# chrischoy/DeepGlobalRegistration

Measured on AMD Instinct MI355X. Metric: pair registrations/sec (FCGF x2 + 1-NN + 6-D inlier net + gate + weighted Procrustes + SE(3) refinement), higher is better.
Workload: dtype f32 results via 2 x f16 split operands (3 f16 MFMA products per MAC, f32 accumulate); k = 1 convs, kNN re-evaluation and registration in exact f32, SVD in f64

## Files before the change

deepglobalregistration_amd/_lib.py:

```python
import ctypes as C
import os
import threading

import torch

_HERE = os.path.dirname(os.path.abspath(__file__))
LIB_PATH = os.environ.get('DGR_HIP_LIB') or os.path.join(_HERE, 'lib', 'libdgr_hip.so')

DGR_OK, DGR_EINVAL, DGR_EHIP, DGR_ENOMEM, DGR_ESVD, DGR_EINTERNAL = 0, -1, -2, -3, -4, -5
STATUS_OK, STATUS_LOW_CONFIDENCE, STATUS_SVD_FAILED, STATUS_SAFEGUARD = 0, 1, 2, 3
STATUS_FLAG_ICP_SKIPPED, STATUS_MASK = 0x100, 0xff

c_i32p, c_i64p, c_f32p, c_f64p = (C.POINTER(C.c_int32), C.POINTER(C.c_int64),
                                  C.POINTER(C.c_float), C.POINTER(C.c_double))
vp = C.c_void_p


class WeightDesc(C.Structure):
    _fields_ = [('name', C.c_char_p), ('data', vp), ('numel', C.c_int64)]


class Params(C.Structure):
    _fields_ = [('clip_weight_thresh', C.c_float), ('voxel_size', C.c_float),
                ('inlier_feature_type', C.c_int), ('max_iter', C.c_int),
# ... 29 lines not shown
    'dgr_net_rerun_layer': (C.c_int, [vp, vp, C.c_int, C.c_int, c_f32p, c_f32p]),
    'dgr_maps_create': (C.c_int, [vp, vp, C.c_int64, C.c_int, C.c_int, C.POINTER(vp), vp]),
    'dgr_maps_destroy': (None, [vp]),
    'dgr_maps_get_coords': (C.c_int, [vp, C.c_int, vp, C.c_int64, c_i64p]),
    'dgr_maps_get_kernel_map': (C.c_int, [vp, C.c_int, C.c_int, vp, C.c_int64, vp, vp, C.c_int64,
                                          c_i64p, c_i64p]),
    'dgr_knn1_l2': (C.c_int, [vp, vp, C.c_int64, vp, C.c_int64, C.c_int, C.c_int, vp, vp, vp]),
    'dgr_knn1_l2_batch': (C.c_int, [vp, vp, c_i64p, vp, c_i64p, C.c_int, C.c_int, C.c_int, vp, vp, vp]),
    'dgr_knn_l2': (C.c_int, [vp, vp, C.c_int64, vp, C.c_int64, C.c_int, C.c_int, C.c_int, vp, vp, vp]),
    'dgr_knn_l2_batch': (C.c_int, [vp, vp, c_i64p, vp, c_i64p, C.c_int, C.c_int, C.c_int, C.c_int, vp, vp,
                                   vp]),
    'dgr_inlier_inputs': (C.c_int, [vp, vp, vp, C.c_int64, vp, vp, C.c_int64, vp, C.c_int, vp, vp, vp]),
    'dgr_sigmoid_clip_sum': (C.c_int, [vp, vp, C.c_int64, C.c_float, vp, c_f64p, vp]),
    'dgr_gather_rows3': (C.c_int, [vp, vp, vp, C.c_int64, vp, vp]),
    'dgr_weighted_procrustes': (C.c_int, [vp, vp, vp, vp, C.c_int64, C.c_float, c_f32p, c_f32p, vp]),
    'dgr_se3_refine': (C.c_int, [vp, vp, vp, vp, C.c_int64, C.c_float, C.c_int, C.c_int, C.c_double,
                                 c_f32p, c_f32p, c_i32p, c_f32p, c_i32p, vp]),
    'dgr_register_batch': (C.c_int, [vp, vp, vp, vp, vp, c_i64p, vp, vp, c_i64p, C.c_int,
                                     C.POINTER(Params), vp, vp, c_f32p, c_i32p, c_f32p, vp]),
    'dgr_register_pairs': (C.c_int, [vp, vp, vp, vp, vp, c_i64p, C.c_int, C.c_int, c_i32p, C.c_int,
                                     C.POINTER(Params), vp, vp, c_f32p, c_i32p, c_f32p, vp]),
    'dgr_register_batch_f64': (C.c_int, [vp, c_f64p, C.c_int64, c_i64p]),
    'dgr_register_batch_output': (C.c_int, [vp, C.c_int, vp, C.c_int64, c_i64p, vp]),
    'dgr_ctx_set_profiling': (C.c_int, [vp, C.c_int]),
    'dgr_icp_point_to_point': (C.c_int, [vp, vp, C.c_int64, vp, C.c_int64, C.c_double, c_f64p, C.c_int, C.c_double,
                                          C.c_double, c_f64p, c_f64p, vp]),
    'dgr_ransac_correspondence': (C.c_int, [vp, vp, vp, C.c_int64, C.c_double, C.c_int64, C.c_uint32, c_f64p, c_f64p, vp]),
    'dgr_ctx_stage_times': (C.c_int, [vp, c_f32p]),
    'dgr_ctx_stage_times_v2': (C.c_int, [vp, c_f32p, C.c_int, C.POINTER(C.c_int)]),
    'dgr_ctx_conv_launches': (C.c_int64, [vp]),
    'dgr_ctx_conv_launch_times': (C.c_int, [vp, c_f32p, c_f32p, C.c_int64, C.POINTER(C.c_int64)]),
    'dgr_ctx_conv_launch_kernel_us': (C.c_int, [vp, c_f32p, C.c_int64, C.POINTER(C.c_int64)]),
    'dgr_ctx_conv_launch_kinds': (C.c_int, [vp, C.c_char_p, C.c_int64, C.POINTER(C.c_int64)]),
    'dgr_radius_pairs_batch': (C.c_int, [vp, vp, c_i64p, vp, c_i64p, C.c_int, c_f64p, C.c_double, C.c_int, vp, vp,
                                         C.c_int64, c_i64p, vp]),
    'dgr_pairs_isin_batch': (C.c_int, [vp, vp, c_i64p, vp, c_i64p, C.c_int, c_i64p, vp, vp]),
    'dgr_validation_counts': (C.c_int, [vp, vp, vp, C.c_float, c_i64p, C.c_int, c_i64p, vp]),
    'dgr_score_pairs': (C.c_int, [vp, vp, c_i64p, C.c_int, c_i32p, C.c_int, c_f64p, C.c_double, c_f64p, vp]),
    'dgr_pose_graph_optimize': (C.c_int, [vp, C.c_int, c_i64p, c_i64p, c_i32p, c_f64p, c_f64p, C.POINTER(C.c_uint8), c_f64p,
                                          C.POINTER(PgParams), c_f64p, c_f64p, c_f64p, vp]),
    'dgr_voxel_mean': (C.c_int, [vp, vp, C.c_int, c_i64p, C.c_int, c_i32p, C.c_int, c_f64p, c_f64p, C.c_double, vp, vp, vp, vp,
                                 vp, c_i64p, c_i64p, vp]),
    'dgr_debug_ortho2rotation': (C.c_int, [vp, vp, C.c_int64, vp, vp, vp, vp]),
    'dgr_debug_se3_refine_from': (C.c_int, [vp, vp, vp, vp, C.c_int64, C.c_float, C.c_int, C.c_int, C.c_double,
                                            c_f64p, c_f64p, vp]),
    'dgr_debug_smooth_l1': (C.c_int, [vp, vp, vp, C.c_int64, C.c_float, vp, vp]),
    'dgr_debug_conv_layer': (C.c_int, [vp, vp, C.c_int, vp, vp, C.c_int, C.c_int64, vp, vp]),
}

_lib = None


def load():
    global _lib
    if _lib is not None:
        return _lib
    if not os.path.exists(LIB_PATH):
        raise RuntimeError(
            f'{LIB_PATH} not found: the HIP extension is not built.  Run '
            '`python -c "import __graft_entry__ as g; g.build()"` (or `make -C '
            'deepglobalregistration_amd/csrc`).  There is no CPU fallback.')
    lib = C.CDLL(LIB_PATH)
    for name, (res, args) in SIGNATURES.items():
        fn = getattr(lib, name)
        fn.restype = res
        fn.argtypes = args
# ... 74 lines not shown
```

deepglobalregistration_amd/csrc/conv.hip:

```cpp
#include <stdlib.h>

#include <map>

#include "dgr_internal.h"
#include <algorithm>
#include "hash.h"
#include "split.h"

typedef float f32x16 __attribute__((ext_vector_type(16)));
typedef float f32x4 __attribute__((ext_vector_type(4)));
typedef _Float16 f16x4 __attribute__((ext_vector_type(4)));
typedef int i32x4 __attribute__((ext_vector_type(4)));
typedef unsigned int u32x2 __attribute__((ext_vector_type(2)));
typedef unsigned int u32x4 __attribute__((ext_vector_type(4)));

struct ConvKArgs {
  const float *in;
  float *out;
  float *y;
  const float *shift;
  const float *w;
  const int32_t *pair_in, *pair_out, *tile_ptr, *rule_ptr, *n_rows_dev;
  const int4 *tile_desc;
  int in_ld, out_ld, in_relu, y_ld;
// ... 817 lines not shown
__global__ void grid_layout_kernel(DgrGridMeta *m, int pad, long long cap) {
  static_assert(GRID_MAXB == 64, "one lane per batch element");
  const int b = threadIdx.x;
  long long vol = 0;
  if (m->mx[b][0] >= m->mn[b][0]) {
    vol = 1;
    for (int d = 0; d < 3; ++d) {
      const long long e = (long long)m->mx[b][d] - m->mn[b][d] + 1 + 2 * pad;
      m->dim[b][d] = (int32_t)(e < (1ll << 30) ? e : (1ll << 30));
      vol = (vol <= cap && e <= cap) ? vol * e : cap + 1;
    }
  }
  long long incl = vol;
#pragma unroll
  for (int s = 1; s < 64; s <<= 1) {
    const long long up = __shfl_up(incl, s, 64);
    if (b >= s) incl += up;
  }
  m->base[b] = incl - vol;
  const long long total = __shfl(incl, 63, 64);
  if (b == 0) {
    m->total = total <= cap ? total : cap + 1;
    m->ok = (!m->bad && total <= cap) ? 1 : 0;
  }
}

__global__ void grid_clear_kernel(const DgrGridMeta *m, int32_t *__restrict__ cells) {
  if (!m->ok) return;
  const long long total = m->total;
  for (long long i = ((long long)blockIdx.x * blockDim.x + threadIdx.x) * 4; i < total; i += (long long)gridDim.x * blockDim.x * 4)
    *reinterpret_cast<int4 *>(cells + i) = make_int4(-1, -1, -1, -1);
}

__device__ __forceinline__ long long grid_cell(const DgrGridMeta *m, int b, int x, int y, int z, int pad) {
  const long long dx = m->dim[b][0], dy = m->dim[b][1];
  return m->base[b] + ((long long)(z - m->mn[b][2] + pad) * dy + (y - m->mn[b][1] + pad)) * dx + (x - m->mn[b][0] + pad);
}

constexpr uint32_t GRID_EMPTY = 0xffffffffu;
__global__ void grid_fill_kernel(const int32_t *__restrict__ coords, const int32_t *n_dev, const DgrGridMeta *m, int pad,
                                 int32_t *__restrict__ cells, const float *__restrict__ values, int values_ld) {
  if (!m->ok) return;
  const int64_t o = (int64_t)blockIdx.x * blockDim.x + threadIdx.x;
  if (o >= *n_dev) return;
  const int4 c = *reinterpret_cast<const int4 *>(coords + o * 4);
  cells[grid_cell(m, c.x, c.y, c.z, c.w, pad)] = values ? __builtin_bit_cast(int32_t, values[o * values_ld]) : (int32_t)o;
}

constexpr int C1_MAXK = 343;
__global__ void __launch_bounds__(256)
    conv1_grid_kernel(const int32_t *__restrict__ coords, const int32_t *n_dev, const DgrGridMeta *__restrict__ m,
                      const int32_t *__restrict__ cells, int ks, const float *__restrict__ in, int in_ld, int cin,
                      const float *__restrict__ w, const float *__restrict__ shift, float *__restrict__ out,
                      int out_ld, int32_t *pair_count, uint32_t *__restrict__ out_amax) {
  __shared__ int2 lists[256 / 64][2][C1_MAXK + 1];
  if (!m->ok) return;
  const int n = *n_dev;
  const int lane = threadIdx.x & 63, wv = threadIdx.x >> 6;
  const int half = ks >> 1, ks2 = ks * ks;
  const int ky = lane % ks, kz = lane / ks;
  const int vsel = lane >> 5, co = lane & 31;
  const unsigned long long below = (1ull << lane) - 1ull;
  const int64_t wave_id = ((int64_t)blockIdx.x * blockDim.x + threadIdx.x) >> 6;
  const int64_t n_waves = ((int64_t)gridDim.x * blockDim.x) >> 6;
  int pairs = 0;
  for (int64_t o0 = wave_id * 2; o0 < n; o0 += n_waves * 2) {
// ... 146 lines not shown
      }
      if (kz + 1 < KS) fill((kz + 1) & 1);
    }
    const int64_t o = v0 + (lane & 15);
    uint32_t mx = 0;
    if (o < n) {
#pragma unroll
      for (int jb = 0; jb < 2; ++jb) {
        f32x4 v = acc[jb];
        if (shift) v += *reinterpret_cast<const f32x4 *>(shift + 16 * jb + 4 * (lane >> 4));
        *reinterpret_cast<f32x4 *>(out + o * out_ld + 16 * jb + 4 * (lane >> 4)) = v;
        const i32x4 b = __builtin_bit_cast(i32x4, v);
        mx = max(mx, max(max((uint32_t)b.x & 0x7fffffffu, (uint32_t)b.y & 0x7fffffffu), max((uint32_t)b.z & 0x7fffffffu, (uint32_t)b.w & 0x7fffffffu)));
      }
    }
    if (out_amax) {
      mx = max(mx, (uint32_t)__shfl_xor((int)mx, 16, 64));
      mx = max(mx, (uint32_t)__shfl_xor((int)mx, 32, 64));
      if (lane < 16 && o < n) atomicMax(out_amax + o, mx);
    }
  }
  if (pair_count) {
    for (int d = 32; d > 0; d >>= 1) pairs += __shfl_down(pairs, d, 64);
    if (lane == 0 && pairs) atomicAdd(&pair_sum, pairs);
    __syncthreads();
    if (threadIdx.x == 0 && pair_sum) atomicAdd(pair_count, pair_sum);
  }
}

int dgr_conv1_probe(DgrArena &arena, const DgrCoordMap &cm, int ks, const float *in, int in_ld, int cin,
                    const float *w_tiled, const float *shift, float *out, int out_ld, int32_t *pair_count,
                    hipStream_t stream, const float *w_compact, const char **kernel_name, uint32_t *out_amax) {
  DGR_REQUIRE(cin >= 1 && cin <= 8 && ks % 2 == 1, "conv1 probe: cin=%d ks=%d", cin, ks);
  if (pair_count && ks > 7) DGR_HIP_CHECK(hipMemsetAsync(pair_count, 0, sizeof(int32_t), stream));
  const int32_t *grid_done = nullptr;
  if (ks <= 7) {
    static const long long cap = 64ll << 20;
    DgrArena::Mark mk = arena.mark();
    DgrGridMeta *meta;
    int32_t *cells;
    DGR_ALLOC(meta, arena, DgrGridMeta, 1);
    DGR_ALLOC(cells, arena, int32_t, cap + 4);
    grid_init_kernel<<<1, 64, 0, stream>>>(meta, pair_count);
    grid_bbox_kernel<<<(int)dgr_ceil_div(cm.n_cap, 256), 256, 0, stream>>>(cm.coords, cm.n_dev, meta);
    grid_layout_kernel<<<1, 64, 0, stream>>>(meta, ks >> 1, cap);
    grid_clear_kernel<<<2048, 256, 0, stream>>>(meta, cells);
    const bool mfma = cin == 1 && w_compact && (out_ld & 3) == 0 && (ks == 3 || ks == 5 || ks == 7);
    grid_fill_kernel<<<(int)dgr_ceil_div(cm.n_cap, 256), 256, 0, stream>>>(cm.coords, cm.n_dev, meta, ks >> 1, cells,
                                                                           mfma ? in : nullptr, in_ld);
    static int resident = 0;
    if (resident == 0) {
      int per_cu = 0, dev = 0, cus = 0;
      DGR_HIP_CHECK(hipOccupancyMaxActiveBlocksPerMultiprocessor(&per_cu, conv1_grid_kernel, 256, 0));
      DGR_HIP_CHECK(hipGetDevice(&dev));
      DGR_HIP_CHECK(hipDeviceGetAttribute(&cus, hipDeviceAttributeMultiprocessorCount, dev));
      resident = (per_cu < 1 ? 1 : per_cu) * (cus < 1 ? 1 : cus);
    }
    if (mfma) {
      const int wgs = (int)dgr_ceil_div(cm.n_cap, 64);
      if (ks == 7) conv1_grid_mfma<7><<<wgs, 256, 0, stream>>>(cm.coords, cm.n_dev, meta, cells, w_compact, shift, out, out_ld, pair_count, out_amax);
      else if (ks == 5) conv1_grid_mfma<5><<<wgs, 256, 0, stream>>>(cm.coords, cm.n_dev, meta, cells, w_compact, shift, out, out_ld, pair_count, out_amax);
      else conv1_grid_mfma<3><<<wgs, 256, 0, stream>>>(cm.coords, cm.n_dev, meta, cells, w_compact, shift, out, out_ld, pair_count, out_amax);
      if (kernel_name) *kernel_name = ks == 7 ? "conv1_grid_mfma<7>" : ks == 5 ? "conv1_grid_mfma<5>" : "conv1_grid_mfma<3>";
    } else {
    int64_t blocks = dgr_ceil_div(cm.n_cap, 8);
    if (blocks > resident) blocks = (int64_t)resident * std::min<int64_t>(4, blocks / resident);
    conv1_grid_kernel<<<(int)blocks, 256, 0, stream>>>(cm.coords, cm.n_dev, meta, cells, ks, in, in_ld, cin, w_tiled, shift,
                                                       out, out_ld, pair_count, out_amax);
    if (kernel_name) *kernel_name = "conv1_grid_kernel";
    }
    DGR_LAUNCH_CHECK();
    grid_done = &meta->ok;
    arena.rewind(mk);
  }
  {
    int64_t blocks = dgr_ceil_div(cm.n_cap, 4);
    if (blocks > 4096) blocks = 4096;
    conv1_probe_kernel<<<(int)blocks, 256, 0, stream>>>(cm.coords, cm.n_dev, cm.table, cm.table_mask, ks, in, in_ld, cin,
                                                        w_tiled, shift, out, out_ld, pair_count, grid_done, out_amax);
  }
  DGR_LAUNCH_CHECK();
  return DGR_OK;
}

__global__ void l2_normalize_kernel(const float *__restrict__ in, int in_ld, float *__restrict__ out,
                                    int out_ld, int c, int relu, const int32_t *n_dev) {
  const int64_t n = *n_dev;
  for (int64_t r = (int64_t)blockIdx.x * blockDim.x + threadIdx.x; r < n;
       r += (int64_t)gridDim.x * blockDim.x) {
    float s = 0.f;
    for (int j = 0; j < c; ++j) {
      float v = in[r * in_ld + j];
      if (relu) v = fmaxf(v, 0.f);
      s += v * v;
    }
    const float den = sqrtf(s) + 1e-8f;
    for (int j = 0; j < c; ++j) {
      float v = in[r * in_ld + j];
      if (relu) v = fmaxf(v, 0.f);
      out[r * out_ld + j] = v / den;
    }
  }
}

// ... 10 lines not shown
```

deepglobalregistration_amd/csrc/coordmap.hip:

```cpp
#include <algorithm>

#include "dgr_internal.h"
#include "hash.h"

constexpr int SCAN_THREADS = 256;
constexpr int SCAN_ITEMS = 8;
constexpr int SCAN_BLOCK = SCAN_THREADS * SCAN_ITEMS;

__device__ __forceinline__ int block_exclusive_scan_256(int v, int *lds , int *total) {
  const int lane = threadIdx.x & 63, wave = threadIdx.x >> 6;
  int x = v;
#pragma unroll
  for (int d = 1; d < 64; d <<= 1) {
    int y = __shfl_up(x, d, 64);
    if (lane >= d) x += y;
  }
  if (lane == 63) lds[wave] = x;
  __syncthreads();
  int base = 0, tot = 0;
#pragma unroll
  for (int w = 0; w < SCAN_THREADS / 64; ++w) {
    int s = lds[w];
    if (w < wave) base += s;
    tot += s;
  }
  __syncthreads();
  *total = tot;
  return base + x - v;
}

__global__ void __launch_bounds__(1024) scan_single_block(const int32_t *__restrict__ in, int64_t n,
                                                          int32_t *__restrict__ out, int32_t *total_out) {
  __shared__ int wsum[16];
  __shared__ int carry_s;
  const int lane = threadIdx.x & 63, wave = threadIdx.x >> 6;
  if (threadIdx.x == 0) carry_s = 0;
  __syncthreads();
  for (int64_t base = 0; base < n; base += 4096) {
    const int64_t i0 = base + (int64_t)threadIdx.x * 4;
    int v[4], s = 0;
#pragma unroll
    for (int j = 0; j < 4; ++j) { v[j] = (i0 + j < n) ? in[i0 + j] : 0; s += v[j]; }
    int x = s;
#pragma unroll
    for (int d = 1; d < 64; d <<= 1) { int y = __shfl_up(x, d, 64); if (lane >= d) x += y; }
    if (lane == 63) wsum[wave] = x;
    __syncthreads();
    int wbase = 0, tot = 0;
#pragma unroll
    for (int w = 0; w < 16; ++w) { const int t = wsum[w]; if (w < wave) wbase += t; tot += t; }
    int ex = carry_s + wbase + x - s;
#pragma unroll
    for (int j = 0; j < 4; ++j) { if (i0 + j < n) out[i0 + j] = ex; ex += v[j]; }
    __syncthreads();
    if (threadIdx.x == 0) carry_s += tot;
    __syncthreads();
  }
  if (threadIdx.x == 0 && total_out) *total_out = carry_s;
}

struct ScanJobs {
  const int32_t *in[DGR_SCAN_MAX];
  int32_t *out[DGR_SCAN_MAX], *sums[DGR_SCAN_MAX], *total[DGR_SCAN_MAX];
  long long n[DGR_SCAN_MAX];
  int nblocks[DGR_SCAN_MAX];
};

__global__ void __launch_bounds__(SCAN_THREADS) scan_block_sums_multi(ScanJobs j) {
  __shared__ int lds[4];
  const int a = blockIdx.y;
  if ((int)blockIdx.x >= j.nblocks[a]) return;
  const int32_t *in = j.in[a];
  const long long n = j.n[a];
  long long base = (long long)blockIdx.x * SCAN_BLOCK + (long long)threadIdx.x * SCAN_ITEMS;
  int s = 0;
#pragma unroll
  for (int i = 0; i < SCAN_ITEMS; ++i)
    if (base + i < n) s += in[base + i];
  int tot;
  block_exclusive_scan_256(s, lds, &tot);
  if (threadIdx.x == 0) j.sums[a][blockIdx.x] = tot;
}

__global__ void __launch_bounds__(SCAN_THREADS) scan_sums_serial_multi(ScanJobs j) {
  __shared__ int lds[4];
  const int a = blockIdx.x;
  int32_t *sums = j.sums[a];
  const int nblocks = j.nblocks[a];
  int carry = 0;
  for (int b0 = 0; b0 < nblocks; b0 += SCAN_THREADS) {
    int i = b0 + threadIdx.x;
    int v = i < nblocks ? sums[i] : 0;
    int tot;
    int ex = block_exclusive_scan_256(v, lds, &tot);
    if (i < nblocks) sums[i] = carry + ex;
    carry += tot;
  }
  if (threadIdx.x == 0 && j.total[a]) *j.total[a] = carry;
}

__global__ void __launch_bounds__(SCAN_THREADS) scan_final_multi(ScanJobs j) {
  __shared__ int lds[4];
  const int a = blockIdx.y;
  if ((int)blockIdx.x >= j.nblocks[a]) return;
  const int32_t *in = j.in[a];
  int32_t *out = j.out[a];
  const long long n = j.n[a];
  long long base = (long long)blockIdx.x * SCAN_BLOCK + (long long)threadIdx.x * SCAN_ITEMS;
  int v[SCAN_ITEMS];
  int s = 0;
#pragma unroll
  for (int i = 0; i < SCAN_ITEMS; ++i) {
    v[i] = (base + i < n) ? in[base + i] : 0;
    s += v[i];
  }
  int tot;
  int ex = block_exclusive_scan_256(s, lds, &tot) + j.sums[a][blockIdx.x];
#pragma unroll
  for (int i = 0; i < SCAN_ITEMS; ++i) {
    if (base + i < n) out[base + i] = ex;
    ex += v[i];
  }
}

int dgr_exclusive_scan_multi(DgrArena &arena, int count, const int32_t *const *in, int32_t *const *out, const int64_t *n,
                             int32_t *const *total_out, hipStream_t stream) {
  DGR_REQUIRE(count >= 1 && count <= DGR_SCAN_MAX, "scan: %d arrays", count);
  ScanJobs j;
  int maxb = 0;
  for (int a = 0; a < count; ++a) {
    DGR_REQUIRE(n[a] > 0, "scan: empty array");
    j.in[a] = in[a]; j.out[a] = out[a]; j.total[a] = total_out ? total_out[a] : nullptr; j.n[a] = n[a];
    j.nblocks[a] = (int)dgr_ceil_div(n[a], SCAN_BLOCK);
    DGR_ALLOC(j.sums[a], arena, int32_t, j.nblocks[a]);
    maxb = j.nblocks[a] > maxb ? j.nblocks[a] : maxb;
  }
  for (int a = count; a < DGR_SCAN_MAX; ++a) { j.in[a] = nullptr; j.out[a] = j.sums[a] = j.total[a] = nullptr; j.n[a] = 0; j.nblocks[a] = 0; }
  scan_block_sums_multi<<<dim3(maxb, count), SCAN_THREADS, 0, stream>>>(j);
  scan_sums_serial_multi<<<count, SCAN_THREADS, 0, stream>>>(j);
  scan_final_multi<<<dim3(maxb, count), SCAN_THREADS, 0, stream>>>(j);
  DGR_LAUNCH_CHECK();
  return DGR_OK;
}

int dgr_exclusive_scan_i32(DgrArena &arena, const int32_t *in, int32_t *out, int64_t n,
                           int32_t *total_out, hipStream_t stream) {
  if (n <= 0) {
    if (total_out) DGR_HIP_CHECK(hipMemsetAsync(total_out, 0, sizeof(int32_t), stream));
    return DGR_OK;
  }
  if (n <= (1 << 14)) {
    scan_single_block<<<1, 1024, 0, stream>>>(in, n, out, total_out);
    DGR_LAUNCH_CHECK();
    return DGR_OK;
  }
  const int32_t *ins[1] = {in};
  int32_t *outs[1] = {out}, *tots[1] = {total_out};
  const int64_t ns[1] = {n};
  return dgr_exclusive_scan_multi(arena, 1, ins, outs, ns, tots, stream);
}

template <int NC>
__global__ void unique_insert(const int32_t *__restrict__ keys, const int32_t *n_dev, int64_t n_cap,
                              int32_t *table, uint32_t mask) {
  int64_t r = (int64_t)blockIdx.x * blockDim.x + threadIdx.x;
  int64_t n = n_dev ? *n_dev : n_cap;
  if (r >= n) return;
  int32_t me[NC];
#pragma unroll
  for (int d = 0; d < NC; ++d) me[d] = keys[r * NC + d];
  uint32_t slot = dgr_hash_row<NC>(me) & mask;
  while (true) {
    int cur = __hip_atomic_load(&table[slot], __ATOMIC_RELAXED, __HIP_MEMORY_SCOPE_AGENT);
    if (cur == DGR_EMPTY) {
      int old = atomicCAS(&table[slot], DGR_EMPTY, (int)r);
      if (old == DGR_EMPTY) return;
      cur = old;
    }
    if (dgr_rows_equal<NC>(keys + (int64_t)cur * NC, me)) {
      atomicMin(&table[slot], (int)r);
      return;
// ... 33 lines not shown
  int64_t o = rank[r];
#pragma unroll
  for (int d = 0; d < NC; ++d) out_coords[o * NC + d] = keys[r * NC + d];
  if (sel_out) sel_out[o] = r;
}

__global__ void table_relabel(int32_t *table, uint32_t cap, const int32_t *__restrict__ rank) {
  uint32_t s = blockIdx.x * blockDim.x + threadIdx.x;
  if (s >= cap) return;
  int v = table[s];
  if (v >= 0) table[s] = rank[v];
}

template <int NC>
__global__ void stride_keys(const int32_t *__restrict__ coords, const int32_t *n_dev, int ts_new,
                            int32_t *__restrict__ keys) {
  int64_t r = (int64_t)blockIdx.x * blockDim.x + threadIdx.x;
  if (r >= *n_dev) return;
  const int32_t m = ~(ts_new - 1);
  keys[r * NC] = coords[r * NC];
#pragma unroll
  for (int d = 1; d < NC; ++d) keys[r * NC + d] = coords[r * NC + d] & m;
}

static inline int grid_for(int64_t n, int threads = 256) { return (int)dgr_ceil_div(n > 0 ? n : 1, threads); }

template <int NC>
static int unique_rows_t(DgrArena &arena, const int32_t *keys, const int32_t *n_dev, int64_t n_cap,
                         int32_t *first_flag, int32_t *rank, int32_t *n_unique_dev,
                         int32_t **table_out, uint32_t *mask_out, hipStream_t stream) {
  uint32_t cap = dgr_next_pow2((uint64_t)(2 * n_cap > 64 ? 2 * n_cap : 64));
  int32_t *table;
  DGR_ALLOC(table, arena, int32_t, cap);
  DGR_HIP_CHECK(hipMemsetAsync(table, 0xff, (size_t)cap * sizeof(int32_t), stream));
  unique_insert<NC><<<grid_for(n_cap), 256, 0, stream>>>(keys, n_dev, n_cap, table, cap - 1);
  unique_flag<NC><<<grid_for(n_cap), 256, 0, stream>>>(keys, n_dev, n_cap, table, cap - 1, first_flag,
                                                      nullptr);
  DGR_LAUNCH_CHECK();
  DGR_CHECK(dgr_exclusive_scan_i32(arena, first_flag, rank, n_cap, n_unique_dev, stream));
  *table_out = table;
  *mask_out = cap - 1;
  return DGR_OK;
}

int dgr_unique_rows(DgrArena &arena, const int32_t *keys, int64_t n, int nc, int32_t *first_flag,
                    int32_t *rank, int32_t *n_unique_dev, int32_t **table_out, uint32_t *mask_out,
                    hipStream_t stream) {
  if (nc == 4)
    return unique_rows_t<4>(arena, keys, nullptr, n, first_flag, rank, n_unique_dev, table_out,
                            mask_out, stream);
  if (nc == 7)
    return unique_rows_t<7>(arena, keys, nullptr, n, first_flag, rank, n_unique_dev, table_out,
                            mask_out, stream);
  dgr_set_error("unsupported coordinate width %d", nc);
  return DGR_EINVAL;
}

template <int NC>
static int build_coord_maps_t(DgrArena &arena, const int32_t *coords, int64_t N, DgrMapSet *ms,
                              hipStream_t stream) {
  DgrCoordMap &c1 = ms->cm[0];
  c1.coords = const_cast<int32_t *>(coords);
  c1.n_cap = N;
  c1.ts = 1;
  DGR_ALLOC(c1.n_dev, arena, int32_t, 1);
  int32_t n32 = (int32_t)N;
  DGR_HIP_CHECK(hipMemcpyAsync(c1.n_dev, &n32, sizeof(int32_t), hipMemcpyHostToDevice, stream));
  {
    uint32_t cap = dgr_next_pow2((uint64_t)(2 * N > 64 ? 2 * N : 64));
    DGR_ALLOC(c1.table, arena, int32_t, cap);
    c1.table_mask = cap - 1;
    DGR_HIP_CHECK(hipMemsetAsync(c1.table, 0xff, (size_t)cap * sizeof(int32_t), stream));
    unique_insert<NC><<<grid_for(N), 256, 0, stream>>>(coords, nullptr, N, c1.table, cap - 1);
    unique_flag<NC><<<grid_for(N), 256, 0, stream>>>(coords, nullptr, N, c1.table, cap - 1, nullptr,
                                                    ms->overflow);
    DGR_LAUNCH_CHECK();
  }
  for (int l = 1; l < 4; ++l) {
    DgrCoordMap &p = ms->cm[l - 1];
    DgrCoordMap &c = ms->cm[l];
    c.ts = p.ts * 2;
    c.n_cap = p.n_cap;
    int32_t *keys, *flag, *rank;
    DGR_ALLOC(keys, arena, int32_t, p.n_cap * NC);
    DGR_ALLOC(flag, arena, int32_t, p.n_cap);
    DGR_ALLOC(rank, arena, int32_t, p.n_cap);
    DGR_ALLOC(c.coords, arena, int32_t, c.n_cap * NC);
    DGR_ALLOC(c.n_dev, arena, int32_t, 1);
    stride_keys<NC><<<grid_for(p.n_cap), 256, 0, stream>>>(p.coords, p.n_dev, c.ts, keys);
    DGR_CHECK(unique_rows_t<NC>(arena, keys, p.n_dev, p.n_cap, flag, rank, c.n_dev, &c.table,
                                &c.table_mask, stream));
    unique_compact<NC><<<grid_for(p.n_cap), 256, 0, stream>>>(keys, p.n_dev, p.n_cap, flag, rank,
                                                             c.coords, nullptr);
    table_relabel<<<grid_for((int64_t)c.table_mask + 1), 256, 0, stream>>>(c.table, c.table_mask + 1,
                                                                           rank);
    DGR_LAUNCH_CHECK();
  }
  return DGR_OK;
}

__global__ void half_keys_kernel(const int32_t *__restrict__ coords7, const int32_t *n_dev,
                                 int32_t *__restrict__ keys4) {
  int64_t r = (int64_t)blockIdx.x * blockDim.x + threadIdx.x;
  if (r >= *n_dev) return;
#pragma unroll
  for (int d = 0; d < 4; ++d) keys4[r * 4 + d] = coords7[r * 7 + d];
}

__global__ void bucket_count_kernel(const int32_t *__restrict__ keys4, const int32_t *n_dev,
                                    const int32_t *__restrict__ table, uint32_t mask,
                                    const int32_t *__restrict__ bkeys, int32_t *__restrict__ row_bucket,
                                    int32_t *counts) {
  int64_t r = (int64_t)blockIdx.x * blockDim.x + threadIdx.x;
  if (r >= *n_dev) return;
  int32_t q[4] = {keys4[r * 4], keys4[r * 4 + 1], keys4[r * 4 + 2], keys4[r * 4 + 3]};
  const int b = dgr_lookup<4>(table, mask, bkeys, q);
  row_bucket[r] = b;
  atomicAdd(&counts[b], 1);
}

__global__ void bucket_members_kernel(const int32_t *__restrict__ row_bucket, const int32_t *n_dev,
                                      const int32_t *__restrict__ start, int32_t *cursor, int32_t *__restrict__ members) {
  int64_t r = (int64_t)blockIdx.x * blockDim.x + threadIdx.x;
  if (r >= *n_dev) return;
  const int b = row_bucket[r];
  members[start[b] + atomicAdd(&cursor[b], 1)] = (int32_t)r;
}

__global__ void bucket_fill_kernel(const int32_t *__restrict__ row_bucket, const int32_t *n_dev,
// ... 7 lines not shown
  const int32_t *c = coords7 + r * 7;
  int p;
  if (members) {
    int rank = 0;
    for (int e = start[b], end = start[b + 1]; e < end; ++e) rank += members[e] < (int32_t)r;
    p = start[b] + rank;
  } else {
    p = start[b] + atomicAdd(&cursor[b], 1);
  }
  if (coords_new) {
#pragma unroll
    for (int d = 0; d < 7; ++d) coords_new[(int64_t)p * 7 + d] = c[d];
    canon[p] = (int32_t)r;
    inv[r] = p;
    second[p] = make_int4(c[4], c[5], c[6], p);
  } else {
    second[p] = make_int4(c[4], c[5], c[6], (int32_t)r);
  }
}

struct RenumberJobs {
  const int32_t *inv[4];
  int32_t *table[4];
  uint32_t cap[4];
};
__global__ void renumber_table_kernel(RenumberJobs j) {
  const int l = blockIdx.y;
  const uint32_t s = blockIdx.x * blockDim.x + threadIdx.x;
  if (s >= j.cap[l]) return;
  const int v = j.table[l][s];
  if (v >= 0) j.table[l][s] = j.inv[l][v];
}

int dgr_build_half_buckets(DgrArena &arena, DgrCoordMap *cm, DgrHalfBuckets *hb, int levels, int renumber_from,
                           hipStream_t stream) {
  DGR_REQUIRE(levels >= 1 && levels <= 4 && renumber_from >= 1, "half buckets: %d levels", levels);
  int32_t *keys[4], *flag[4], *rank[4], *nb_dev[4], *row_bucket[4], *counts[4], *cursor[4];
  uint32_t cap[4];
  size_t table_words = 0, count_words = 0;
  for (int l = 0; l < levels; ++l) {
    const int64_t n = cm[l].n_cap;
    cap[l] = dgr_next_pow2((uint64_t)(2 * n > 64 ? 2 * n : 64));
    table_words += cap[l];
    count_words += 2 * (size_t)(n + 1);
  }
  int32_t *tables, *cnts;
  DGR_ALLOC(tables, arena, int32_t, table_words);
  DGR_ALLOC(cnts, arena, int32_t, count_words);
  DGR_HIP_CHECK(hipMemsetAsync(tables, 0xff, table_words * sizeof(int32_t), stream));
  DGR_HIP_CHECK(hipMemsetAsync(cnts, 0, count_words * sizeof(int32_t), stream));
  for (int l = 0; l < levels; ++l) {
    const int64_t n = cm[l].n_cap;
    hb[l].table = tables; tables += cap[l];
    hb[l].mask = cap[l] - 1;
    counts[l] = cnts; cursor[l] = cnts + (n + 1); cnts += 2 * (n + 1);
    DGR_ALLOC(keys[l], arena, int32_t, n * 4);
    DGR_ALLOC(flag[l], arena, int32_t, n);
    DGR_ALLOC(rank[l], arena, int32_t, n);
    DGR_ALLOC(nb_dev[l], arena, int32_t, 1);
    DGR_ALLOC(row_bucket[l], arena, int32_t, n);
    DGR_ALLOC(hb[l].bkeys, arena, int32_t, n * 4);
    DGR_ALLOC(hb[l].start, arena, int32_t, n + 1);
    DGR_ALLOC(hb[l].second, arena, int4, n);
  }
  for (int l = 0; l < levels; ++l) {
    const int64_t n = cm[l].n_cap;
    half_keys_kernel<<<grid_for(n), 256, 0, stream>>>(cm[l].coords, cm[l].n_dev, keys[l]);
    unique_insert<4><<<grid_for(n), 256, 0, stream>>>(keys[l], cm[l].n_dev, n, hb[l].table, hb[l].mask);
    unique_flag<4><<<grid_for(n), 256, 0, stream>>>(keys[l], cm[l].n_dev, n, hb[l].table, hb[l].mask, flag[l], nullptr);
  }
  DGR_LAUNCH_CHECK();
  {
    const int32_t *ins[4];
    int32_t *outs[4], *tots[4];
    int64_t ns[4];
    for (int l = 0; l < levels; ++l) { ins[l] = flag[l]; outs[l] = rank[l]; tots[l] = nb_dev[l]; ns[l] = cm[l].n_cap; }
    DGR_CHECK(dgr_exclusive_scan_multi(arena, levels, ins, outs, ns, tots, stream));
  }
  for (int l = 0; l < levels; ++l) {
    const int64_t n = cm[l].n_cap;
    unique_compact<4><<<grid_for(n), 256, 0, stream>>>(keys[l], cm[l].n_dev, n, flag[l], rank[l], hb[l].bkeys, nullptr);
    table_relabel<<<grid_for((int64_t)hb[l].mask + 1), 256, 0, stream>>>(hb[l].table, hb[l].mask + 1, rank[l]);
    bucket_count_kernel<<<grid_for(n), 256, 0, stream>>>(keys[l], cm[l].n_dev, hb[l].table, hb[l].mask, hb[l].bkeys, row_bucket[l],
                                                         counts[l]);
  }
  DGR_LAUNCH_CHECK();
  {
    const int32_t *ins[4];
    int32_t *outs[4], *tots[4];
    int64_t ns[4];
    for (int l = 0; l < levels; ++l) { ins[l] = counts[l]; outs[l] = hb[l].start; tots[l] = nullptr; ns[l] = cm[l].n_cap + 1; }
    DGR_CHECK(dgr_exclusive_scan_multi(arena, levels, ins, outs, ns, tots, stream));
  }
  RenumberJobs rj = {};
  int nrj = 0;
  int64_t max_cap = 0;
  for (int l = 0; l < levels; ++l) {
    const int64_t n = cm[l].n_cap;
    int32_t *coords_new = nullptr, *canon = nullptr, *inv = nullptr;
    if (l >= renumber_from) {
      DGR_ALLOC(coords_new, arena, int32_t, n * 7);
      DGR_ALLOC(canon, arena, int32_t, n);
      DGR_ALLOC(inv, arena, int32_t, n);
      rj.inv[nrj] = inv; rj.table[nrj] = cm[l].table; rj.cap[nrj] = cm[l].table_mask + 1;
      max_cap = std::max<int64_t>(max_cap, rj.cap[nrj]);
      ++nrj;
    }
    const int32_t *members = nullptr;
    if (coords_new) {
      bucket_members_kernel<<<grid_for(n), 256, 0, stream>>>(row_bucket[l], cm[l].n_dev, hb[l].start, cursor[l], rank[l]);
      members = rank[l];
    }
    bucket_fill_kernel<<<grid_for(n), 256, 0, stream>>>(row_bucket[l], cm[l].n_dev, hb[l].start, cursor[l], members,
                                                        cm[l].coords, hb[l].second, coords_new, canon, inv);
    if (coords_new) { cm[l].coords = coords_new; cm[l].canon = canon; }
    hb[l].built = true;
  }
  if (nrj) renumber_table_kernel<<<dim3((unsigned)grid_for(max_cap), nrj), 256, 0, stream>>>(rj);
  DGR_LAUNCH_CHECK();
  return DGR_OK;
}

int dgr_build_coord_maps(DgrArena &arena, const int32_t *coords, int64_t N, DgrMapSet *ms,
                         hipStream_t stream) {
  if (ms->nc == 4) return build_coord_maps_t<4>(arena, coords, N, ms, stream);
  if (ms->nc == 7) return build_coord_maps_t<7>(arena, coords, N, ms, stream);
  dgr_set_error("unsupported dimension D=%d (3 and 6 are on the DGR path)", ms->D);
  return DGR_EINVAL;
}

template <typename T>
__global__ void voxel_keys(const T *__restrict__ xyz, int64_t M, T inv_unused, T voxel, int32_t batch,
                           int32_t *__restrict__ keys) {
  int64_t r = (int64_t)blockIdx.x * blockDim.x + threadIdx.x;
  if (r >= M) return;
  keys[r * 4] = batch;
#pragma unroll
  for (int d = 0; d < 3; ++d) keys[r * 4 + 1 + d] = (int32_t)floor(xyz[r * 3 + d] / voxel);
}

template <typename T>
__global__ void voxel_gather_xyz(const T *__restrict__ xyz, const int64_t *__restrict__ sel,
                                 const int32_t *n_dev, float *__restrict__ out) {
  int64_t r = (int64_t)blockIdx.x * blockDim.x + threadIdx.x;
  if (r >= *n_dev) return;
  int64_t s = sel[r];
#pragma unroll
  for (int d = 0; d < 3; ++d) out[r * 3 + d] = (float)xyz[s * 3 + d];
}

extern "C" int dgr_voxelize(dgr_ctx *ctx, const void *xyz, int is_f64, int64_t M, double voxel_size,
                            int32_t batch_index, int64_t *sel_out, int32_t *coords_out,
                            float *xyz_out, int64_t *n_out, dgr_stream stream_) {
  DGR_REQUIRE(ctx && xyz && sel_out && coords_out && n_out, "dgr_voxelize: NULL argument");
  DGR_REQUIRE(M > 0 && M < (1ll << 30), "dgr_voxelize: M=%lld out of range", (long long)M);
  DGR_REQUIRE(voxel_size > 0, "dgr_voxelize: voxel_size must be positive");
  hipStream_t stream = (hipStream_t)stream_;
  DGR_HIP_CHECK(hipSetDevice(ctx->device));
  DGR_CHECK(ctx->arena.reset());
  DgrArena &A = ctx->arena;
  int32_t *keys, *flag, *rank, *n_dev, *table;
  uint32_t mask;
  DGR_ALLOC(keys, A, int32_t, M * 4);
  DGR_ALLOC(flag, A, int32_t, M);
  DGR_ALLOC(rank, A, int32_t, M);
  DGR_ALLOC(n_dev, A, int32_t, 1);
  if (is_f64)
    voxel_keys<double><<<grid_for(M), 256, 0, stream>>>((const double *)xyz, M, 0.0, voxel_size,
                                                       batch_index, keys);
  else
    voxel_keys<float><<<grid_for(M), 256, 0, stream>>>((const float *)xyz, M, 0.f, (float)voxel_size,
                                                      batch_index, keys);
  DGR_CHECK(unique_rows_t<4>(A, keys, nullptr, M, flag, rank, n_dev, &table, &mask, stream));
  unique_compact<4><<<grid_for(M), 256, 0, stream>>>(keys, nullptr, M, flag, rank, coords_out, sel_out);
  if (xyz_out) {
    if (is_f64)
      voxel_gather_xyz<double><<<grid_for(M), 256, 0, stream>>>((const double *)xyz, sel_out, n_dev,
                                                               xyz_out);
    else
      voxel_gather_xyz<float><<<grid_for(M), 256, 0, stream>>>((const float *)xyz, sel_out, n_dev,
                                                              xyz_out);
  }
  DGR_LAUNCH_CHECK();
  int32_t n32 = 0;
  DGR_HIP_CHECK(hipMemcpyAsync(&n32, n_dev, sizeof(int32_t), hipMemcpyDeviceToHost, stream));
  DGR_HIP_CHECK(hipStreamSynchronize(stream));
  *n_out = n32;
  return DGR_OK;
}
```

deepglobalregistration_amd/csrc/ctx.hip:

```cpp
#include <stdarg.h>
#include <time.h>
#include <string.h>

#include "dgr_internal.h"

static thread_local char g_err[1024] = "";

void dgr_set_error(const char *fmt, ...) {
  va_list ap;
  va_start(ap, fmt);
  vsnprintf(g_err, sizeof(g_err), fmt, ap);
  va_end(ap);
}

extern "C" const char *dgr_last_error(void) { return g_err; }
extern "C" const char *dgr_version(void) { return "dgr_hip 0.4 (gfx950)"; }

static constexpr size_t kAlign = 256;
static constexpr size_t kMinChunk = (size_t)256 << 20;

void *DgrArena::alloc(size_t bytes) {
  bytes = (bytes + kAlign - 1) / kAlign * kAlign;
  if (bytes == 0) bytes = kAlign;
  while (cur < chunks.size()) {
// ... 203 lines not shown

extern "C" int dgr_ctx_stage_times_v2(dgr_ctx *ctx, float *times_ms, int capacity, int *n) {
  DGR_REQUIRE(ctx != nullptr && times_ms != nullptr && capacity >= 0, "bad argument");
  static_assert(sizeof(ctx->stage_ms) == DGR_NUM_STAGE_TIMES * sizeof(float), "stage list and header disagree");
  const int m = capacity < DGR_NUM_STAGE_TIMES ? capacity : DGR_NUM_STAGE_TIMES;
  memcpy(times_ms, ctx->stage_ms, (size_t)m * sizeof(float));
  if (n) *n = m;
  return DGR_OK;
}

extern "C" int64_t dgr_ctx_conv_launches(dgr_ctx *ctx) { return ctx ? ctx->conv_launches : 0; }

extern "C" int dgr_ctx_conv_launch_times(dgr_ctx *ctx, float *times_ms, float *gemm_ms, int64_t capacity, int64_t *n) {
  DGR_REQUIRE(ctx != nullptr && times_ms != nullptr && n != nullptr, "bad argument");
  int64_t m = (int64_t)ctx->conv_span_ms.size();
  if (m > capacity) m = capacity;
  for (int64_t i = 0; i < m; ++i) {
    times_ms[i] = ctx->conv_span_ms[i];
    if (gemm_ms) gemm_ms[i] = i < (int64_t)ctx->gemm_span_ms.size() ? ctx->gemm_span_ms[i] : 0.f;
  }
  *n = m;
  return DGR_OK;
}

extern "C" int dgr_ctx_conv_launch_kernel_us(dgr_ctx *ctx, float *us, int64_t capacity, int64_t *n) {
  DGR_REQUIRE(ctx != nullptr && us != nullptr && n != nullptr, "bad argument");
  int64_t m = (int64_t)ctx->conv_clk_us.size();
  if (m > capacity) m = capacity;
  for (int64_t i = 0; i < m; ++i) us[i] = ctx->conv_clk_us[i];
  *n = m;
  return DGR_OK;
}

extern "C" int dgr_ctx_conv_launch_kinds(dgr_ctx *ctx, char *buf, int64_t capacity, int64_t *n) {
  DGR_REQUIRE(ctx != nullptr && buf != nullptr && n != nullptr && capacity > 0, "bad argument");
  std::string all;
  int64_t m = 0;
  for (const char *k : ctx->conv_kinds) {
    if ((int64_t)(all.size() + strlen(k) + 2) > capacity) break;
    all += k;
    all += '\n';
    ++m;
  }
  memcpy(buf, all.c_str(), all.size() + 1);
  *n = m;
  return DGR_OK;
}
```

deepglobalregistration_amd/csrc/dgr_internal.h:

```cpp
#pragma once
#include <hip/hip_runtime.h>
#include <stdint.h>
#include <stdio.h>
#include <stdlib.h>
#include <string>
#include <vector>

#include "../../include/dgr_hip.h"

void dgr_set_error(const char *fmt, ...);

#define DGR_HIP_CHECK(expr)                                                                  \
  do {                                                                                       \
    hipError_t _e = (expr);                                                                  \
    if (_e != hipSuccess) {                                                                  \
      dgr_set_error("%s:%d: %s failed: %s", __FILE__, __LINE__, #expr, hipGetErrorString(_e)); \
      return DGR_EHIP;                                                                       \
    }                                                                                        \
  } while (0)

#define DGR_CHECK(expr)          \
  do {                           \
    int _r = (expr);             \
    if (_r != DGR_OK) return _r; \
  } while (0)

#define DGR_REQUIRE(cond, ...)     \
  do {                             \
    if (!(cond)) {                 \
      dgr_set_error(__VA_ARGS__);  \
      return DGR_EINVAL;           \
    }                              \
  } while (0)

#define DGR_LAUNCH_CHECK() DGR_HIP_CHECK(hipGetLastError())

inline bool dgr_exact_f32() {
  static const bool on = getenv("DGR_EXACT_F32") != nullptr;
  return on;
}

struct DgrArena {
  struct Chunk {
    char *base;
    size_t size;
  };
  std::vector<Chunk> chunks;
  size_t cur = 0;
  size_t offset = 0;
  size_t high_water = 0, used_total = 0;
  uint64_t generation = 0;

  struct Mark {
    size_t cur, offset, used_total;
  };
  Mark mark() const { return {cur, offset, used_total}; }
  void rewind(const Mark &m) { cur = m.cur; offset = m.offset; used_total = m.used_total; }
  void *alloc(size_t bytes);
  int reset();
  void release();
  size_t reserved() const;
  template <typename T>
  T *get(size_t n) {
    return static_cast<T *>(alloc(n * sizeof(T)));
  }
};

#define DGR_ALLOC(ptr, arena, T, n)                       \
// ... 151 lines not shown
};

struct DgrEventPool {
  std::vector<hipEvent_t> ev;
  size_t used = 0;
  hipEvent_t next();
  void release();
};

struct dgr_ctx {
  int device = 0;
  int num_cus = 256;
  DgrArena arena;
  bool profiling = false;
  float stage_ms[9] = {0, 0, 0, 0, 0, 0, 0, 0, 0};
  int64_t conv_launches = 0;
  DgrBatchOutputs last;
  std::vector<double> last_T64;
  DgrEventPool events;
  std::vector<std::pair<hipEvent_t, hipEvent_t>> conv_spans, gemm_spans, map3_spans, map6_spans;
  std::vector<float> conv_span_ms, gemm_span_ms;
  std::vector<unsigned long long *> conv_clks;
  std::vector<float> conv_clk_us;
  std::vector<const char *> conv_kinds;
  int32_t *flag_dev = nullptr;
  hipEvent_t wait_ev = nullptr;
  long last_wait_ns = 0;
  double batch_ns_per_row = 0;
  double pairs_ns_per_row = 0;
  unsigned char *pin = nullptr;
  size_t pin_bytes = 0;
  hipStream_t part_stream = nullptr;
  int all_cus = 256;
};

int dgr_ctx_pinned(dgr_ctx *ctx, size_t bytes, unsigned char **out);
int dgr_flag_error(int32_t flag);

int dgr_ctx_wait(dgr_ctx *ctx, hipStream_t stream, long predicted_ns = 0);

int dgr_resunet_forward_impl(dgr_ctx *ctx, dgr_net *net, const int32_t *coords, const float *feats,
                             int64_t N, float *out, hipStream_t stream);
int dgr_ctx_collect_profile(dgr_ctx *ctx);
void dgr_ctx_begin_profile(dgr_ctx *ctx);

int dgr_knn1_batch_impl(dgr_ctx *ctx, const float *F0, const int64_t *off0, const float *F1, const int64_t *off1,
                        int npairs, int C, int squared, int64_t *idx_out, float *dist_out, hipStream_t stream);
int dgr_knn1_impl(dgr_ctx *ctx, const float *F0, int64_t N0, const float *F1, int64_t N1, int C,
                  int squared, int64_t *idx_out, float *dist_out, hipStream_t stream);
int dgr_inlier_inputs_impl(const int32_t *coords0, const float *xyz0, int64_t N0,
                           const int32_t *coords1, const float *xyz1, const int64_t *idx1,
                           int feature_type, int32_t *coords6, float *feats, hipStream_t stream);
int dgr_icp_impl(dgr_ctx *ctx, const float *src, int64_t N0, const float *dst, int64_t N1, double max_dist,
                 const double *T_init, int max_iter, double rel_fitness, double rel_rmse, double *T_out,
                 double *stats_out, hipStream_t stream);
int dgr_ransac_impl(dgr_ctx *ctx, const float *X, const float *Y, int64_t N, double max_dist, int64_t num_hypotheses,
                    uint32_t seed, double *T_out, double *stats_out, hipStream_t stream);
struct DgrIcpJob {
  const float *src = nullptr, *dst = nullptr;
  int64_t N0 = 0, N1 = 0;
  double max_dist = 0;
  int nblocks = 0;
  void *st = nullptr;
  double *P = nullptr, *sorted = nullptr, *partial = nullptr;
  int32_t ncell = 0;
  double host_state[64];
// ... 25 lines not shown
```

deepglobalregistration_amd/csrc/kmap.hip:

```cpp
#include <string.h>

#include <algorithm>

#include "dgr_internal.h"
#include "hash.h"

constexpr int KM_THREADS = 256;

template <int D>
__device__ __forceinline__ void offset_of(int k, int ks, int ts, int32_t *delta) {
  const int half = ks >> 1;
#pragma unroll
  for (int d = 0; d < D; ++d) {
    delta[d] = ((k % ks) - half) * ts;
    k /= ks;
  }
}

template <int D>
__device__ __forceinline__ int probe(const int32_t *__restrict__ out_coords, int64_t o,
                                     const int32_t *delta, const int32_t *__restrict__ in_coords,
                                     const int32_t *__restrict__ in_table, uint32_t in_mask) {
  constexpr int NC = D + 1;
  int32_t q[NC];
// ... 442 lines not shown
  if (need_in_csr) {
    DGR_ALLOC(km->in_ptr, arena, int32_t, n_in_cap + 1);
    DGR_ALLOC(km->in_pos, arena, int32_t, km->pair_cap);
  }
  return DGR_OK;
}

static void finalize_job(FinalizeJobs &fj, int m, const int32_t *base, const int32_t *total, int K, int RB, DgrKernelMap *km) {
  fj.base[m] = base; fj.total[m] = total; fj.K[m] = K; fj.RB[m] = RB;
  fj.rule_ptr[m] = km->rule_ptr; fj.tile_ptr[m] = km->tile_ptr;
  fj.desc[m] = km->tile_desc; fj.tile_cap[m] = km->tile_cap;
}

static int build_kernel_map3(DgrArena &arena, const DgrCoordMap &in, const DgrCoordMap &out, int ks, int max_pairs_per_row,
                             bool need_in_csr, bool want_pair_out, bool want_pair_k, DgrKernelMap *km,
                             int32_t *overflow, hipStream_t stream) {
  constexpr int D = 3;
  const int K = ks * ks * ks;
  const int64_t n_cap = out.n_cap, n_in_cap = in.n_cap;
  const int RB = (int)dgr_ceil_div(n_cap, KM_THREADS);
  DGR_CHECK(alloc_kernel_map(arena, K, n_cap, n_in_cap, max_pairs_per_row, need_in_csr, want_pair_out, want_pair_k, km));
  const int KW = (K + 31) / 32;
  DgrArena::Mark mk = arena.mark();
  int32_t *counts, *base, *total;
  DGR_ALLOC(counts, arena, int32_t, (int64_t)K * RB);
  DGR_ALLOC(base, arena, int32_t, (int64_t)K * RB);
  DGR_ALLOC(total, arena, int32_t, 1);
  uint32_t *mask_out, *mask_in = nullptr;
  int32_t *cnt_out, *cnt_in = nullptr;
  {
    const size_t w_out = (size_t)(n_cap + 1) * KW, w_in = need_in_csr ? (size_t)(n_in_cap + 1) * KW : 0;
    DGR_ALLOC(mask_out, arena, uint32_t, w_out + w_in);
    if (need_in_csr) mask_in = mask_out + w_out;
    DGR_HIP_CHECK(hipMemsetAsync(mask_out, 0, (w_out + w_in) * sizeof(uint32_t), stream));
  }
  DGR_ALLOC(cnt_out, arena, int32_t, n_cap + 1);
  if (need_in_csr) DGR_ALLOC(cnt_in, arena, int32_t, n_in_cap + 1);
  int32_t *hits;
  DGR_ALLOC(hits, arena, int32_t, (int64_t)K * n_cap);
  kmap_search<D><<<dim3(RB, K), KM_THREADS, 0, stream>>>(out.coords, out.n_dev, in.coords, in.table, in.table_mask, ks,
                                                         in.ts, RB, n_cap, hits, counts, KW, mask_out, mask_in);
  DGR_LAUNCH_CHECK();
  mask_count_kernel<<<(int)dgr_ceil_div(n_cap + 1, 256), 256, 0, stream>>>(mask_out, KW, out.n_dev, n_cap + 1, cnt_out);
  if (need_in_csr)
    mask_count_kernel<<<(int)dgr_ceil_div(n_in_cap + 1, 256), 256, 0, stream>>>(mask_in, KW, in.n_dev, n_in_cap + 1, cnt_in);
  {
    const int32_t *ins[3] = {cnt_out, counts, cnt_in};
    int32_t *outs[3] = {km->out_ptr, base, km->in_ptr}, *tots[3] = {nullptr, total, nullptr};
    const int64_t ns[3] = {n_cap + 1, (int64_t)K * RB, n_in_cap + 1};
    DGR_CHECK(dgr_exclusive_scan_multi(arena, need_in_csr ? 3 : 2, ins, outs, ns, tots, stream));
  }
  FinalizeJobs fj = {};
  finalize_job(fj, 0, base, total, K, RB, km);
  kmap_finalize<<<1, 1024, 0, stream>>>(fj);
  tile_desc_kernel<<<dim3((unsigned)dgr_ceil_div(km->tile_cap, 256), 1), 256, 0, stream>>>(fj);
  kmap_fill<<<dim3(RB, (K + KM_KGROUP - 1) / KM_KGROUP), KM_THREADS, 0, stream>>>(
      out.n_dev, RB, K, n_cap, hits, counts, base, km->pair_in, km->pair_out, km->pair_cap, overflow, KW, mask_out,
      km->out_ptr, km->out_pos, mask_in, km->in_ptr, km->in_pos, km->pair_k);
  DGR_LAUNCH_CHECK();
  arena.rewind(mk);
  km->built = true;
  return DGR_OK;
}

struct Kmap6Job {
  const DgrCoordMap *in, *out;
  const DgrHalfBuckets *hb;
  const DgrHalfBuckets *hb_out;
  bool need_in_csr, want_pair_out, want_pair_k;
  DgrKernelMap *km;
};
static int build_kernel_maps6(DgrArena &arena, const Kmap6Job *jobs, int nj, int max_pairs_per_row, int32_t *overflow,
                              hipStream_t stream) {
  constexpr int K = 729, KW = (K + 31) / 32;
  DGR_REQUIRE(nj >= 1 && nj <= KM_MAXJOBS, "6-D kernel maps: %d jobs", nj);
  struct Tr {
    int RB, symmetric;
    int64_t n_cap, n_in_cap, hit_waves;
    int32_t *counts, *base, *total, *cnt_out, *cnt_in;
    uint32_t *mask_out, *mask_in;
    int4 *cell;
    HitList hl;
    unsigned short *wpre_out, *wpre_in;
  } t[KM_MAXJOBS];
  for (int m = 0; m < nj; ++m) {
    const Kmap6Job &J = jobs[m];
    t[m].n_cap = J.out->n_cap; t[m].n_in_cap = J.in->n_cap;
    DGR_REQUIRE(t[m].n_cap < (1ll << 27) && t[m].n_in_cap < (1ll << 27), "6-D kernel maps: more than 2^27 rows");
    DGR_CHECK(alloc_kernel_map(arena, K, t[m].n_cap, t[m].n_in_cap, max_pairs_per_row, J.need_in_csr, J.want_pair_out,
                               J.want_pair_k, J.km));
  }
  DgrArena::Mark mk = arena.mark();
  {
    size_t words = 0;
    for (int m = 0; m < nj; ++m)
      words += (size_t)(t[m].n_cap + 1) * KW + (jobs[m].need_in_csr ? (size_t)(t[m].n_in_cap + 1) * KW : 0) + (size_t)(t[m].n_cap + 1);
    uint32_t *pool;
    DGR_ALLOC(pool, arena, uint32_t, words);
    DGR_HIP_CHECK(hipMemsetAsync(pool, 0, words * sizeof(uint32_t), stream));
    for (int m = 0; m < nj; ++m) {
      t[m].mask_out = pool; pool += (size_t)(t[m].n_cap + 1) * KW;
      t[m].mask_in = nullptr;
      if (jobs[m].need_in_csr) { t[m].mask_in = pool; pool += (size_t)(t[m].n_in_cap + 1) * KW; }
      t[m].cnt_out = reinterpret_cast<int32_t *>(pool); pool += (size_t)(t[m].n_cap + 1);
    }
  }
  for (int m = 0; m < nj; ++m) {
    const Kmap6Job &J = jobs[m];
    Tr &r = t[m];
    r.RB = (int)dgr_ceil_div(r.n_cap, KM_THREADS);
    r.symmetric = (J.in->coords == J.out->coords && !J.need_in_csr) ? 1 : 0;
    DGR_REQUIRE(J.hb && J.hb->built && J.hb_out && J.hb_out->built, "6-D kernel map: first-half buckets missing");
    DGR_ALLOC(r.counts, arena, int32_t, (int64_t)K * r.RB);
    DGR_ALLOC(r.base, arena, int32_t, (int64_t)K * r.RB);
    DGR_ALLOC(r.total, arena, int32_t, 1);
    r.cnt_in = nullptr;
    if (J.need_in_csr) DGR_ALLOC(r.cnt_in, arena, int32_t, r.n_in_cap + 1);
    DGR_ALLOC(r.cell, arena, int4, (int64_t)r.RB * (KM_THREADS / 64) * K);
    const int64_t search_blocks = dgr_ceil_div(r.n_cap * (r.symmetric ? 14 : 27), KM_THREADS);
    r.hit_waves = search_blocks * (KM_THREADS / 64);
    r.hl.region = (J.in->ts >= 8 && r.symmetric) ? 2 * KM_REGION : KM_REGION / 2;
    DGR_REQUIRE(r.hit_waves < (1ll << 31), "6-D kernel map: too many search waves");
    DGR_ALLOC(r.hl.recs, arena, unsigned long long, r.hit_waves * r.hl.region);
    DGR_ALLOC(r.hl.wave_count, arena, int32_t, r.hit_waves);
    DGR_ALLOC(r.wpre_out, arena, unsigned short, (r.n_cap + 1) * KW);
    r.wpre_in = nullptr;
    if (J.need_in_csr) DGR_ALLOC(r.wpre_in, arena, unsigned short, (r.n_in_cap + 1) * KW);
  }
  static_assert(KM_JOBS6 >= KM_MAXJOBS, "multi-job launch tables");
  {
    Bits6Jobs bj = {};
    Colmask6Jobs cj = {};
    int max_sb = 0, max_rb = 0;
    for (int m = 0; m < nj; ++m) {
      const Kmap6Job &J = jobs[m];
      Tr &r = t[m];
      bj.pa[m] = PrunedArgs{J.out->coords, J.out->n_dev, J.hb_out->second, r.n_cap, *J.hb, J.in->ts, r.symmetric};
      bj.mask_out[m] = r.mask_out; bj.mask_in[m] = r.mask_in; bj.hl[m] = r.hl;
      bj.blocks[m] = (int)(r.hit_waves / (KM_THREADS / 64));
      max_sb = std::max(max_sb, bj.blocks[m]);
      cj.mask_out[m] = r.mask_out; cj.n_out_dev[m] = J.out->n_dev; cj.RB[m] = r.RB; cj.cell[m] = r.cell;
      cj.counts[m] = r.counts; cj.row_cnt[m] = r.cnt_out; cj.wpre[m] = r.wpre_out;
      max_rb = std::max(max_rb, r.RB);
    }
    kmap_bits_pruned6<<<dim3((unsigned)max_sb, (unsigned)nj), KM_THREADS, 0, stream>>>(bj, KW);
    kmap_colmask<<<dim3((unsigned)max_rb, (unsigned)nj), KM_THREADS, 0, stream>>>(cj, K, KW);
    {
      MaskCountJobs mj = {};
      int nm = 0;
      long long max_rows = 0;
      for (int m = 0; m < nj; ++m)
        if (jobs[m].need_in_csr) {
          mj.mask[nm] = t[m].mask_in; mj.n_dev[nm] = jobs[m].in->n_dev; mj.n_cap[nm] = t[m].n_in_cap + 1;
          mj.cnt[nm] = t[m].cnt_in; mj.wpre[nm] = t[m].wpre_in;
          max_rows = std::max(max_rows, mj.n_cap[nm]);
          ++nm;
        }
      static_assert(KM_MC_JOBS >= KM_MAXJOBS, "mask-count job table");
      if (nm) mask_count_multi<KW><<<dim3((unsigned)dgr_ceil_div(max_rows, 256), (unsigned)nm), 256, 0, stream>>>(mj);
    }
  }
  DGR_LAUNCH_CHECK();
  {
    const int32_t *ins[DGR_SCAN_MAX];
    int32_t *outs[DGR_SCAN_MAX], *tots[DGR_SCAN_MAX];
    int64_t ns[DGR_SCAN_MAX];
    int c = 0;
    for (int m = 0; m < nj; ++m) {
      ins[c] = t[m].cnt_out; outs[c] = jobs[m].km->out_ptr; tots[c] = nullptr; ns[c++] = t[m].n_cap + 1;
      ins[c] = t[m].counts; outs[c] = t[m].base; tots[c] = t[m].total; ns[c++] = (int64_t)K * t[m].RB;
      if (jobs[m].need_in_csr) { ins[c] = t[m].cnt_in; outs[c] = jobs[m].km->in_ptr; tots[c] = nullptr; ns[c++] = t[m].n_in_cap + 1; }
    }
    DGR_CHECK(dgr_exclusive_scan_multi(arena, c, ins, outs, ns, tots, stream));
  }
  FinalizeJobs fj = {};
  int64_t max_tiles = 0;
  for (int m = 0; m < nj; ++m) {
    finalize_job(fj, m, t[m].base, t[m].total, K, t[m].RB, jobs[m].km);
    max_tiles = std::max<int64_t>(max_tiles, jobs[m].km->tile_cap);
  }
  kmap_finalize<<<nj, 1024, 0, stream>>>(fj);
  tile_desc_kernel<<<dim3((unsigned)dgr_ceil_div(max_tiles, 256), nj), 256, 0, stream>>>(fj);
  {
    Place6Jobs pj = {};
    int max_pb = 0;
    for (int m = 0; m < nj; ++m) {
      const Kmap6Job &J = jobs[m];
      Tr &r = t[m];
      DgrKernelMap *km = J.km;
      pj.p[m] = PlaceArgs{K, KW, r.RB, r.mask_out, km->out_ptr, r.cell, r.base, km->pair_in, km->pair_out, km->pair_k, km->out_pos,
                          km->pair_cap, overflow, r.mask_in, km->in_ptr, km->in_pos, r.wpre_out, r.wpre_in};
      pj.replay[m] = PrunedArgs{J.out->coords, J.out->n_dev, J.hb_out->second, r.n_cap, *J.hb, J.in->ts, r.symmetric};
      pj.h[m] = r.hl;
      pj.n_waves[m] = (int)r.hit_waves;
      pj.blocks[m] = (int)std::min<int64_t>(dgr_ceil_div(r.hit_waves, KM_THREADS / 64), 16384);
      max_pb = std::max(max_pb, pj.blocks[m]);
      km->built = true;
    }
    kmap_place_hits<<<dim3((unsigned)max_pb, (unsigned)nj), KM_THREADS, 0, stream>>>(pj);
  }
  DGR_LAUNCH_CHECK();
  arena.rewind(mk);
  return DGR_OK;
}

constexpr int NBR_JOBS = 10;
struct NbrJobs {
  const int32_t *out_coords[NBR_JOBS], *n_out_dev[NBR_JOBS], *in_coords[NBR_JOBS], *in_table[NBR_JOBS];
  uint32_t in_mask[NBR_JOBS];
  int ts[NBR_JOBS];
  long long n_pad[NBR_JOBS];
  int32_t *nbr[NBR_JOBS];
};
__global__ void __launch_bounds__(KM_THREADS) nbr_search3(NbrJobs J) {
  const int jm = blockIdx.z;
  const int64_t n_pad = J.n_pad[jm];
  const int64_t o = (int64_t)blockIdx.x * KM_THREADS + threadIdx.x;
  if (o >= n_pad) return;
  int32_t *__restrict__ nbr = J.nbr[jm];
  const int kz = blockIdx.y;
  if (o >= *J.n_out_dev[jm]) {
#pragma unroll
    for (int u = 0; u < 9; ++u) nbr[(int64_t)(9 * kz + u) * n_pad + o] = -1;
    return;
  }
  const int sts = J.ts[jm];
  const int4 c = *reinterpret_cast<const int4 *>(J.out_coords[jm] + o * 4);
  int32_t q[9][4];
#pragma unroll
  for (int u = 0; u < 9; ++u) {
    q[u][0] = c.x;
    q[u][1] = c.y + ((u % 3) - 1) * sts;
    q[u][2] = c.z + ((u / 3) - 1) * sts;
    q[u][3] = c.w + (kz - 1) * sts;
// ... 112 lines not shown
  for (int64_t o = (int64_t)blockIdx.x * blockDim.x + threadIdx.x; o < n; o += (int64_t)gridDim.x * blockDim.x)
    c += nbr[(int64_t)k * n_pad + o] >= 0;
  for (int d = 32; d > 0; d >>= 1) c += __shfl_down(c, d, 64);
  if ((threadIdx.x & 63) == 0 && c) atomicAdd(&counts[k], (unsigned long long)c);
}

int dgr_nbr_counts(const DgrNbrTable &t, const int32_t *n_out_dev, int64_t counts[27]) {
  unsigned long long *dev;
  DGR_HIP_CHECK(hipMalloc((void **)&dev, 27 * sizeof(unsigned long long)));
  DGR_HIP_CHECK(hipMemset(dev, 0, 27 * sizeof(unsigned long long)));
  nbr_count_kernel<<<dim3(64, 27), 256>>>(t.nbr, t.n_pad, n_out_dev, dev);
  unsigned long long host[27];
  hipError_t e = hipMemcpy(host, dev, sizeof(host), hipMemcpyDeviceToHost);
  (void)hipFree(dev);
  DGR_HIP_CHECK(e);
  for (int k = 0; k < 27; ++k) counts[k] = (int64_t)host[k];
  return DGR_OK;
}

int dgr_build_coord_maps(DgrArena &arena, const int32_t *coords, int64_t N, DgrMapSet *ms,
                         hipStream_t stream);
int dgr_build_half_buckets(DgrArena &arena, DgrCoordMap *cm, DgrHalfBuckets *hb, int levels, int renumber_from, hipStream_t stream);

int dgr_build_maps(DgrArena &arena, const int32_t *coords, int64_t N, int D, int conv1_ks,
                   DgrMapSet *ms, hipStream_t stream, bool skip_conv1_map, bool lean, bool nbr_tables) {
  DGR_REQUIRE(D == 3 || D == 6, "D=%d not supported (the DGR path uses D=3 and D=6)", D);
  DGR_REQUIRE(conv1_ks % 2 == 1 && conv1_ks >= 1, "conv1 kernel size must be odd");
  DGR_REQUIRE(N > 0 && N < (1ll << 30), "N=%lld out of range", (long long)N);
  ms->D = D;
  ms->nc = D + 1;
  ms->conv1_ks = conv1_ks;
  if (!ms->overflow) {
    DGR_ALLOC(ms->overflow, arena, int32_t, 1);
    DGR_HIP_CHECK(hipMemsetAsync(ms->overflow, 0, sizeof(int32_t), stream));
  }
  DGR_CHECK(dgr_build_coord_maps(arena, coords, N, ms, stream));
  if (nbr_tables) {
    DGR_REQUIRE(D == 3, "neighbour tables are a D = 3 structure");
    ms->use_nbr = true;
    NbrJobs nbj = {};
    int n_nbj = 0;
    int32_t *cls;
    DGR_ALLOC(cls, arena, int32_t, 3 * 8);
    for (int l = 0; l < 4; ++l) DGR_CHECK(build_nbr_table(arena, ms->cm[l], ms->cm[l], ms->cm[l].ts, +1, &ms->nsame[l], &nbj, &n_nbj));
    for (int l = 0; l < 3; ++l) {
      DGR_CHECK(build_nbr_table(arena, ms->cm[l], ms->cm[l + 1], ms->cm[l].ts, +1, &ms->ndown[l], &nbj, &n_nbj));
      DGR_CHECK(build_nbr_table(arena, ms->cm[l + 1], ms->cm[l], ms->cm[l].ts, -1, &ms->nup[l], &nbj, &n_nbj, cls + 8 * l));
    }
    DGR_CHECK(nbr_tables_launch(nbj, n_nbj, stream));
    {
      ClsJobs cj = {};
      int max_nb = 0;
      for (int l = 0; l < 3; ++l) {
        cj.coords[l] = ms->cm[l].coords; cj.n_dev[l] = ms->cm[l].n_dev; cj.ts[l] = ms->cm[l].ts;
        cj.nb[l] = (int)dgr_ceil_div(ms->cm[l].n_cap, KM_THREADS);
        DGR_ALLOC(cj.blk_cnt[l], arena, int32_t, (int64_t)cj.nb[l] * 8);
        cj.perm[l] = ms->nup[l].perm; cj.cls_count[l] = ms->nup[l].cls_count; cj.cls_cap[l] = ms->nup[l].cls_cap;
        max_nb = std::max(max_nb, cj.nb[l]);
      }
      cls_count_kernel<<<dim3((unsigned)max_nb, 3), KM_THREADS, 0, stream>>>(cj);
      cls_fill_kernel<<<dim3((unsigned)max_nb, 3), KM_THREADS, 0, stream>>>(cj);
      DGR_LAUNCH_CHECK();
    }
    if (lean) {
      if (conv1_ks != 3 && !skip_conv1_map)
        DGR_CHECK(build_kernel_map3(arena, ms->cm[0], ms->cm[0], conv1_ks, 1024, false, false, true, &ms->conv1, ms->overflow,
                                    stream));
      return DGR_OK;
    }
  }
  const int cap_row = (D == 3) ? 1024 : 160;
  if (D == 6) {
    DGR_REQUIRE(conv1_ks == 3, "6-D kernel maps support kernel size 3 only (got %d)", conv1_ks);
    DGR_CHECK(dgr_build_half_buckets(arena, ms->cm, ms->hb, 4, 1, stream));
    Kmap6Job jobs[7];
    for (int l = 0; l < 4; ++l) jobs[l] = {&ms->cm[l], &ms->cm[l], &ms->hb[l], &ms->hb[l], false, !lean, !lean || l == 0, &ms->same[l]};
    for (int l = 0; l < 3; ++l) jobs[4 + l] = {&ms->cm[l], &ms->cm[l + 1], &ms->hb[l], &ms->hb[l + 1], true, true, !lean, &ms->down[l]};
    DGR_CHECK(build_kernel_maps6(arena, jobs, 7, cap_row, ms->overflow, stream));
    ms->conv1 = ms->same[0];
    return DGR_OK;
  }
  auto build = [&](const DgrCoordMap &in, const DgrCoordMap &out, int ks, bool rev, bool want_k, DgrKernelMap *km) -> int {
    const bool want_out = !lean || rev, want_pk = !lean || want_k;
    return build_kernel_map3(arena, in, out, ks, cap_row, rev, want_out, want_pk, km, ms->overflow, stream);
  };
  for (int l = 0; l < 4; ++l) DGR_CHECK(build(ms->cm[l], ms->cm[l], 3, false, l == 0, &ms->same[l]));
  if (conv1_ks == 3)
    ms->conv1 = ms->same[0];
  else if (!skip_conv1_map)
    DGR_CHECK(build(ms->cm[0], ms->cm[0], conv1_ks, false, true, &ms->conv1));
  for (int l = 0; l < 3; ++l) DGR_CHECK(build(ms->cm[l], ms->cm[l + 1], 3, true, false, &ms->down[l]));
  return DGR_OK;
}

struct dgr_maps {
  dgr_ctx *ctx;
  DgrArena arena;
  DgrMapSet ms;
  int32_t *coords_copy = nullptr;
  hipStream_t stream;
};

extern "C" int dgr_maps_create(dgr_ctx *ctx, const int32_t *coords, int64_t N, int D,
                               int conv1_kernel_size, dgr_maps **out, dgr_stream stream_) {
  DGR_REQUIRE(ctx && coords && out, "dgr_maps_create: NULL argument");
  hipStream_t stream = (hipStream_t)stream_;
  DGR_HIP_CHECK(hipSetDevice(ctx->device));
  dgr_maps *m = new dgr_maps();
  m->ctx = ctx;
  m->stream = stream;
  int rc = DGR_OK;
  do {
    m->coords_copy = m->arena.get<int32_t>((size_t)N * (D + 1));
    if (!m->coords_copy) { rc = DGR_ENOMEM; break; }
    if (hipMemcpyAsync(m->coords_copy, coords, (size_t)N * (D + 1) * sizeof(int32_t),
                       hipMemcpyDeviceToDevice, stream) != hipSuccess) { rc = DGR_EHIP; break; }
    rc = dgr_build_maps(m->arena, m->coords_copy, N, D, conv1_kernel_size, &m->ms, stream, false, false, D == 3);
    if (rc != DGR_OK) break;
    int32_t flag = 0;
    if (hipMemcpyAsync(&flag, m->ms.overflow, sizeof(int32_t), hipMemcpyDeviceToHost, stream) != hipSuccess ||
        hipStreamSynchronize(stream) != hipSuccess) { rc = DGR_EHIP; dgr_set_error("maps sync failed"); break; }
    if (flag == 1) { dgr_set_error("duplicate coordinates in the sparse tensor input"); rc = DGR_EINVAL; break; }
    if (flag == 2) { dgr_set_error("kernel-map capacity exceeded"); rc = DGR_ENOMEM; break; }
  } while (0);
  if (rc != DGR_OK) {
    m->arena.release();
    delete m;
    return rc;
  }
  *out = m;
  return DGR_OK;
}

extern "C" void dgr_maps_destroy(dgr_maps *m) {
  if (!m) return;
  (void)hipDeviceSynchronize();
  m->arena.release();
  delete m;
// ... 110 lines not shown
```

deepglobalregistration_amd/csrc/knn.hip:

```cpp
#include "knn_prefilter.h"

template <int C, int QPT>
__global__ void __launch_bounds__(KNN_THREADS)
    knn1_kernel(const float *__restrict__ F0, const float *__restrict__ F1, KnnBatch B, int splits,
                u64 *__restrict__ best, const int32_t *run_flag, const int32_t *__restrict__ qlist,
                const int32_t *qcount, int64_t q_begin) {
  __shared__ __attribute__((aligned(16))) float tile[KNN_TB * C];
  const KnnPair d = B.p[blockIdx.z];
  if (run_flag && run_flag[blockIdx.z] == 0) return;
  F0 += d.q0 * C;
  F1 += d.r0 * C;
  best += d.q0;
  const int64_t N0 = d.n0, N1 = d.n1;
  if (qlist) qlist += d.q0 - q_begin;
  const int64_t n_q = qlist ? (int64_t)qcount[blockIdx.z] : N0;
  if ((int64_t)blockIdx.x * KNN_THREADS * QPT >= n_q) return;
  const int64_t q0 = ((int64_t)blockIdx.x * KNN_THREADS + threadIdx.x) * QPT;
  const int rows_per_split = (int)(((N1 + splits - 1) / splits + KNN_TB - 1) / KNN_TB) * KNN_TB;
  const int64_t j_begin = (int64_t)blockIdx.y * rows_per_split;
  const int64_t j_end = min(N1, j_begin + rows_per_split);
  if (j_begin >= j_end) return;
  float q[QPT][C];
  int64_t qrow[QPT];
#pragma unroll
// ... 139 lines not shown
    }
#pragma unroll
    for (int s2 = 32; s2 > 0; s2 >>= 1) {
      const u64 o = __shfl_xor(key, s2, 64);
      key = o < key ? o : key;
    }
    if ((threadIdx.x & 63) == 0) wkey[threadIdx.x >> 6] = key;
    __syncthreads();
    if (threadIdx.x == 0) {
      u64 k3 = wkey[0];
      for (int w = 1; w < 4; ++w) k3 = wkey[w] < k3 ? wkey[w] : k3;
      if (k3 != KNN_KEY_NONE) atomicMin(best + q, k3);
    }
    __syncthreads();
  }
}

__global__ void knn_long_list_flags(const int32_t *__restrict__ qcount, int np, int32_t *__restrict__ flags) {
  if ((int)threadIdx.x < np) flags[threadIdx.x] = qcount[threadIdx.x] > KNN_SCAN_MAX;
}

static int knn_prefiltered(dgr_ctx *ctx, const float *F0, const float *F1, KnnBatch B, u64 *best, hipStream_t stream) {
  KnnPlan P;
  DGR_CHECK(knn_prefilter_setup<false>(ctx, F0, F1, B, KNN_SLOTS, stream, &P));
  DGR_CHECK((knn_mfma_launch<false, false>(ctx, B, P, KNN_SUB, KNN_SLOTS, stream)));
  DGR_CHECK((knn_mfma_launch<true, false>(ctx, B, P, 1, KNN_SLOTS, stream)));
  knn_exact_kernel<<<(int)dgr_ceil_div(P.span, 256), 256, 0, stream>>>(F0, F1, P.cand, P.cand_cnt, P.q_begin,
                                                                      P.q_begin + P.span, best);
  DGR_LAUNCH_CHECK();
  DGR_CHECK(knn_list_overflows(B, P, KNN_SLOTS, stream));
  dim3 grid(KNN_SCAN_SPLITS, B.np);
  knn_query_scan_kernel<<<grid, 256, 0, stream>>>(F0, F1, B, P.q_begin, P.qlist, P.qcount, best);
  knn_long_list_flags<<<1, 64, 0, stream>>>(P.qcount, B.np, P.flags);
  DGR_LAUNCH_CHECK();
  DGR_CHECK(knn_launch<32>(ctx, F0, F1, B, best, P.flags, stream, P.qlist, P.qcount, P.q_begin));
  return knn_launch<32>(ctx, F0, F1, B, best, P.fallback, stream);
}

int dgr_knn1_batch_impl(dgr_ctx *ctx, const float *F0, const int64_t *off0, const float *F1, const int64_t *off1,
                        int npairs, int C, int squared, int64_t *idx_out, float *dist_out, hipStream_t stream) {
  return knn_for_each_table(ctx, off0, off1, npairs, 1, true, stream, [&](const KnnBatch &B, u64 *best) -> int {
    DGR_CHECK(knn_dispatch(
        B, C,
        [&](auto width, const KnnBatch &pairs) {
          return knn_launch<decltype(width)::value>(ctx, F0, F1, pairs, best, nullptr, stream);
        },
        [&](const KnnBatch &pairs) { return knn_prefiltered(ctx, F0, F1, pairs, best, stream); }));
    dim3 grid((unsigned)dgr_ceil_div(knn_n0_max(B), 256), B.np);
    knn1_finish<<<grid, 256, 0, stream>>>(best, B, squared, idx_out, dist_out);
    DGR_LAUNCH_CHECK();
    return DGR_OK;
  });
}

int dgr_knn1_impl(dgr_ctx *ctx, const float *F0, int64_t N0, const float *F1, int64_t N1, int C,
                  int squared, int64_t *idx_out, float *dist_out, hipStream_t stream) {
  const int64_t off0[2] = {0, N0}, off1[2] = {0, N1};
  return dgr_knn1_batch_impl(ctx, F0, off0, F1, off1, 1, C, squared, idx_out, dist_out, stream);
}

extern "C" int dgr_knn1_l2(dgr_ctx *ctx, const float *F0, int64_t N0, const float *F1, int64_t N1, int C,
                           int squared, int64_t *idx_out, float *dist_out, dgr_stream stream) {
  const int64_t off0[2] = {0, N0}, off1[2] = {0, N1};
  DGR_CHECK(knn_enter("dgr_knn1_l2", ctx, F0, F1, idx_out, off0, off1, 1));
  return dgr_knn1_impl(ctx, F0, N0, F1, N1, C, squared, idx_out, dist_out, (hipStream_t)stream);
}

// ... 7 lines not shown
```

deepglobalregistration_amd/csrc/knn_common.h:

```cpp
#pragma once
#include <type_traits>
#include "dgr_internal.h"

constexpr int KNN_THREADS = 256;
constexpr int KNN_TB = 64;
constexpr int KNN_MAXP = 32;
constexpr int KNN_MIN_REFS = 1024;

struct KnnPair {
  int64_t q0, r0;
  int32_t n0, n1;
  int32_t qb0, rt0;
};
struct KnnBatch {
  KnnPair p[KNN_MAXP];
  int np;
};

typedef unsigned long long u64;
constexpr u64 KNN_KEY_NONE = ~0ull;
__device__ __forceinline__ u64 knn_key(float d2, int64_t row) {
  return ((u64)__float_as_uint(d2) << 32) | (unsigned int)row;
}

// ... 34 lines not shown
    *q_begin = std::min(*q_begin, B.p[p].q0);
    q_end = std::max(q_end, B.p[p].q0 + B.p[p].n0);
  }
  return q_end - *q_begin;
}

inline dim3 knn_brute_grid(const dgr_ctx *ctx, const KnnBatch &B, int qpt, int64_t max_splits) {
  int64_t n1_max = 0, qblocks_all = 0;
  for (int p = 0; p < B.np; ++p) {
    n1_max = std::max<int64_t>(n1_max, B.p[p].n1);
    qblocks_all += dgr_ceil_div(B.p[p].n0, (int64_t)KNN_THREADS * qpt);
  }
  int64_t splits = dgr_ceil_div((int64_t)ctx->num_cus * 4, qblocks_all);
  splits = std::max<int64_t>(1, std::min(splits, std::min(max_splits, dgr_ceil_div(n1_max, KNN_TB))));
  return dim3((unsigned)dgr_ceil_div(knn_n0_max(B), (int64_t)KNN_THREADS * qpt), (unsigned)splits, B.np);
}

inline int knn_enter(const char *entry, dgr_ctx *ctx, const void *F0, const void *F1, const void *idx_out,
                     const int64_t *off0, const int64_t *off1, int npairs) {
  DGR_REQUIRE(ctx && F0 && F1 && off0 && off1 && idx_out, "%s: NULL argument", entry);
  DGR_REQUIRE(npairs >= 1, "%s: npairs=%d", entry, npairs);
  DGR_HIP_CHECK(hipSetDevice(ctx->device));
  return ctx->arena.reset();
}

template <class Fn>
inline int knn_for_each_table(dgr_ctx *ctx, const int64_t *off0, const int64_t *off1, int npairs, int k, bool clear,
                              hipStream_t stream, Fn &&fn) {
  const int64_t n0 = off0[npairs];
  DGR_REQUIRE(off0[0] == 0 && off1[0] == 0, "find_knn: the row offsets start at 0");
  DGR_REQUIRE(off1[npairs] < (1ll << 31) && n0 < (1ll << 31), "find_knn: N0 / N1 too large");
  u64 *keys;
  DGR_ALLOC(keys, ctx->arena, u64, n0 * k);
  if (clear) DGR_HIP_CHECK(hipMemsetAsync(keys, 0xff, (size_t)(n0 * k) * sizeof(u64), stream));
  for (int p0 = 0; p0 < npairs; p0 += KNN_MAXP) {
    KnnBatch B;
    B.np = std::min(KNN_MAXP, npairs - p0);
    for (int p = 0; p < B.np; ++p) {
      KnnPair &d = B.p[p];
      d.q0 = off0[p0 + p]; d.r0 = off1[p0 + p];
      d.n0 = (int32_t)(off0[p0 + p + 1] - off0[p0 + p]); d.n1 = (int32_t)(off1[p0 + p + 1] - off1[p0 + p]);
      d.qb0 = d.rt0 = 0;
      DGR_REQUIRE(d.n0 > 0 && d.n1 > 0, "find_knn: pair %d has an empty feature matrix (N0=%d, N1=%d)", p0 + p, d.n0,
                  d.n1);
    }
    const DgrArena::Mark mk = ctx->arena.mark();
    DGR_CHECK(fn(B, keys));
    ctx->arena.rewind(mk);
  }
  return DGR_OK;
}

inline bool knn_force_brute() {
  static const bool brute = getenv("DGR_KNN_BRUTE") != nullptr;
  return brute;
}
template <class Brute, class Prefiltered>
inline int knn_dispatch(const KnnBatch &B, int C, Brute &&brute, Prefiltered &&prefiltered) {
  switch (C) {
    case 16: return brute(std::integral_constant<int, 16>{}, B);
    case 64: return brute(std::integral_constant<int, 64>{}, B);
    case 32: {
      KnnBatch big, small;
      big.np = small.np = 0;
      for (int p = 0; p < B.np; ++p) {
        if (knn_force_brute() || B.p[p].n1 < KNN_MIN_REFS) small.p[small.np++] = B.p[p];
        else big.p[big.np++] = B.p[p];
// ... 11 lines not shown
```

deepglobalregistration_amd/csrc/knn_prefilter.h:

```cpp
#pragma once
#include "knn_common.h"

typedef __attribute__((ext_vector_type(8))) short bf16x8;
typedef __attribute__((ext_vector_type(16))) float f32x16_t;
constexpr float KNN_TAU_C = 8e-5f;
constexpr int KNN_ST = 4;
constexpr int KNN_SLOTS = 32;
#ifndef DGR_KNN_SUB
#define DGR_KNN_SUB 2
#endif
constexpr int KNN_SUB = DGR_KNN_SUB;

__device__ __forceinline__ unsigned short knn_f2bf(float x) {
  uint32_t u = __float_as_uint(x);
  if ((u & 0x7f800000u) == 0x7f800000u) return (unsigned short)((u >> 16) | ((u & 0xffffu) ? 0x40u : 0u));
  u += 0x7fffu + ((u >> 16) & 1u);
  return (unsigned short)(u >> 16);
}
__device__ __forceinline__ float knn_bf2f(unsigned short h) { return __uint_as_float((uint32_t)h << 16); }
__device__ __forceinline__ uint32_t knn_ord(float f) {
  const uint32_t u = __float_as_uint(f);
  return u ^ ((u >> 31) ? 0xffffffffu : 0x80000000u);
}
__device__ __forceinline__ float knn_unord(uint32_t k) {
// ... 224 lines not shown
  KnnPlan &P = *plan;
  DgrArena &arena = ctx->arena;
  int n_qb = 0, n_rt = 0;
  P.qb_max = P.rt_max = P.qgroups_all = 0;
  for (int p = 0; p < B.np; ++p) {
    KnnPair &d = B.p[p];
    d.qb0 = n_qb;
    d.rt0 = n_rt;
    const int qb = (d.n0 + 31) / 32, rt = (d.n1 + 31) / 32;
    n_qb += qb;
    n_rt += rt;
    P.qb_max = std::max(P.qb_max, qb);
    P.rt_max = std::max(P.rt_max, rt);
    P.qgroups_all += (int)dgr_ceil_div(qb, 16);
  }
  P.n0_max = knn_n0_max(B);
  P.span = knn_query_span(B, &P.q_begin);
  const int64_t n_mt = (TOPK ? 32 : 1) * P.span;
  DGR_ALLOC(P.Qp, arena, bf16x8, (int64_t)n_qb * 256);
  DGR_ALLOC(P.Rp, arena, bf16x8, (int64_t)n_rt * 256);
  DGR_ALLOC(P.na, arena, float, (int64_t)n_qb * 32);
  DGR_ALLOC(P.nb, arena, float, (int64_t)n_rt * 32);
  DGR_ALLOC(P.mt, arena, uint32_t, n_mt);
  P.thr = nullptr;
  if (TOPK) DGR_ALLOC(P.thr, arena, float, P.span);
  DGR_ALLOC(P.qlist, arena, int32_t, P.span);
  DGR_ALLOC(P.cand_cnt, arena, int32_t, P.span + 4 * KNN_MAXP);
  DGR_ALLOC(P.cand, arena, int32_t, P.span * slots);
  int32_t *pair_words = P.cand_cnt + P.span;
  P.nb_max = reinterpret_cast<uint32_t *>(pair_words);
  P.fallback = pair_words + KNN_MAXP;
  P.qcount = pair_words + 2 * KNN_MAXP;
  P.flags = pair_words + 3 * KNN_MAXP;
  DGR_HIP_CHECK(hipMemsetAsync(P.cand_cnt, 0, (size_t)(P.span + 4 * KNN_MAXP) * sizeof(int32_t), stream));
  DGR_HIP_CHECK(hipMemsetAsync(P.mt, 0xff, (size_t)n_mt * sizeof(uint32_t), stream));
  dim3 grid((unsigned)dgr_ceil_div((int64_t)std::max(P.qb_max, P.rt_max) * 32 * 4, 256), 2 * B.np);
  knn_pack_kernel<TOPK><<<grid, 256, 0, stream>>>(F0, F1, B, P.Qp, P.Rp, P.na, P.nb, P.nb_max, P.fallback);
  DGR_LAUNCH_CHECK();
  return DGR_OK;
}

template <bool PASS2, bool TOPK>
inline int knn_mfma_launch(dgr_ctx *ctx, const KnnBatch &B, const KnnPlan &P, int sub, int slots, hipStream_t stream) {
  const auto kernel = knn_mfma_kernel<PASS2, TOPK>;
  static int per_cu = 0;
  if (per_cu == 0) {
    int n = 0;
    DGR_HIP_CHECK(hipOccupancyMaxActiveBlocksPerMultiprocessor(&n, kernel, 256, 0));
    per_cu = n < 1 ? 1 : n;
  }
  const int capacity = ctx->num_cus * per_cu;
  const int stages = (int)dgr_ceil_div(P.rt_max, KNN_ST);
  int splits = 1;
  double best_fill = 0.;
  for (int sp = 1; sp <= std::min(16, std::max(1, stages / sub)); ++sp) {
    const int64_t blocks = (int64_t)P.qgroups_all * sp;
    const double fill = (double)blocks / (double)(dgr_ceil_div(blocks, (int64_t)capacity) * capacity);
    if (fill >= best_fill) { best_fill = fill; splits = sp; }
  }
  dim3 grid((unsigned)dgr_ceil_div(P.qb_max, 16), splits, B.np);
  kernel<<<grid, 256, 0, stream>>>(P.Qp, P.Rp, P.nb, B, splits, sub, P.q_begin, P.span, P.mt, P.na, P.nb_max, P.thr,
                                   P.cand, P.cand_cnt, slots);
  DGR_LAUNCH_CHECK();
  return DGR_OK;
}

int knn_list_overflows(const KnnBatch &B, const KnnPlan &P, int slots, hipStream_t stream);
```

deepglobalregistration_amd/csrc/net.hip:

```cpp
#include <math.h>
#include <stdlib.h>
#include <string.h>

#include <algorithm>
#include <map>
#include <memory>
#include <string>

#include "dgr_internal.h"

static const int CH[5] = {0, 32, 64, 128, 256};
static const int TR[5] = {0, 64, 64, 64, 128};
static constexpr float BN_EPS = 1e-5f;

struct DgrLayer {
  std::string name;
  int K, cin, cout, cin_pad, cout_pad;
  float *w = nullptr;
  float *w16 = nullptr;
  void *w16b = nullptr;
  void *w16d = nullptr;
  int64_t w16b_piece = 0;
  float *wc = nullptr;
  float *wq = nullptr;
// ... 140 lines not shown
                          *v = find_desc(descs, nd, p + "running_var");
    DGR_REQUIRE(g && b && m && v, "state_dict is missing batch-norm tensors '%s*'", p.c_str());
    DGR_REQUIRE(g->numel == cout && b->numel == cout && m->numel == cout && v->numel == cout,
                "batch-norm '%s' has the wrong width", p.c_str());
    const float *gd = host_of(g), *bd2 = host_of(b), *md = host_of(m), *vd = host_of(v);
    DGR_REQUIRE(gd && bd2 && md && vd, "batch-norm '%s': device tensors could not be read", p.c_str());
    for (int c = 0; c < cout; ++c) {
      float s = gd[c] / sqrtf(vd[c] + BN_EPS);
      scale[c] = s;
      shift[c] = bd2[c] - md[c] * s;
    }
    has_shift = true;
  }
  if (bias) {
    const dgr_weight_desc *bd = find_desc(descs, nd, name + ".bias");
    DGR_REQUIRE(bd && bd->numel == cout, "state_dict is missing '%s.bias' [1,%d]", name.c_str(), cout);
    const float *bh = host_of(bd);
    DGR_REQUIRE(bh, "'%s.bias': device tensor could not be read", name.c_str());
    for (int c = 0; c < cout; ++c) shift[c] += bh[c];
    has_shift = true;
  }
  DgrWeights &W = *net->W;
  hipStream_t s = P.s;
  const float *src = kd->data;
  if (!P.dev) {
    const size_t n = (size_t)kd->numel;
    if (n > P.staging_n) {
      DGR_HIP_CHECK(hipStreamSynchronize(s));
      DGR_HIP_CHECK(hipFree(P.staging));
      P.staging = nullptr;
      DGR_HIP_CHECK(hipMalloc((void **)&P.staging, n * sizeof(float)));
      P.staging_n = n;
    }
    DGR_HIP_CHECK(hipMemcpyAsync(P.staging, kd->data, n * sizeof(float), hipMemcpyHostToDevice, s));
    src = P.staging;
  }
  const float *sc = P.sc;
  DGR_HIP_CHECK(hipMemcpyAsync(P.sc, scale.data(), (size_t)cout * sizeof(float), hipMemcpyHostToDevice, s));
  if (has_shift) {
    DGR_CHECK(W.alloc(&L.shift, cout));
    DGR_HIP_CHECK(hipMemcpyAsync(L.shift, shift.data(), (size_t)cout * sizeof(float), hipMemcpyHostToDevice, s));
  }
  const int64_t nw = (int64_t)K * cin * cout;
  DGR_HIP_CHECK(hipMemsetAsync(P.mxb, 0, sizeof(uint32_t), s));
  dgr_absmax_scaled_kernel<<<(int)std::min<int64_t>((nw + 255) / 256, 4096), 256, 0, s>>>(src, sc, nw, cout, P.mxb);
  DGR_LAUNCH_CHECK();
  uint32_t bits = 0;
  DGR_HIP_CHECK(hipMemcpyAsync(&bits, P.mxb, sizeof(bits), hipMemcpyDeviceToHost, s));
  DGR_HIP_CHECK(hipStreamSynchronize(s));
  float mx;
  memcpy(&mx, &bits, 4);
  int ex = 0;
  if (mx > 0.f && std::isfinite(mx)) (void)frexpf(mx, &ex);
  ex = std::min(std::max(ex, -100), 100);
  const float w_scale = ldexpf(1.f, 15 - ex);
  L.w_unscale = ldexpf(1.f, ex - 15);
  const bool use_wide = K > 1 && !dgr_exact_f32() && dgr_conv_wide_supported(L.cin_pad, cin, cout) && !(net->D == 3 && K == 27);
  if (use_wide) {
    const int S16 = cin / 16, NB32 = cout / 32;
    L.wb_piece = (int64_t)K * S16 * NB32 * 64;
    const int64_t ne = L.wb_piece * 8;
    uint16_t *dst;
    DGR_CHECK(W.alloc(&dst, (size_t)2 * ne));
    L.wb = dst;
    DGR_CHECK(dgr_fill(s, ne, [=] __device__(int64_t o) {
      const int e = (int)(o & 7), lane = (int)((o >> 3) & 63);
      const int64_t r = o >> 9;
      const int nb = (int)(r % NB32), s2 = (int)((r / NB32) % S16), k = (int)(r / ((int64_t)NB32 * S16));
      const int col = 32 * nb + (lane & 31), row = 16 * s2 + 8 * (lane >> 5) + e;
      const float xs = __fmul_rn(__fmul_rn(src[((size_t)k * cin + row) * cout + col], sc[col]), w_scale);
      dst[o] = dgr_f16_bits_dev(xs);
      dst[ne + o] = dgr_f16_bits_dev(xs - dgr_f16_val_dev(xs));
    }));
    W.param_bytes += (size_t)2 * ne * sizeof(uint16_t);
  } else {
    const int S = L.cin_pad / 8, NBLK = L.cout_pad / 32;
    const int64_t ne = (int64_t)K * S * NBLK * 256;
    DGR_CHECK(W.alloc(&L.w, ne));
    float *const dst = L.w;
    DGR_CHECK(dgr_fill(s, ne, [=] __device__(int64_t o) {
      const int c = (int)(o & 3), lane = (int)((o >> 2) & 63);
// ... 273 lines not shown
        o.in_dsplit = in.dsplit;
        o.out_dsplit = out.dsplit;
        if (out.dsplit_only) o.out = nullptr;
      }
      const char *kname = "sparse_conv_os";
      DGR_CHECK(dgr_conv_os_launch(o, stream, &kname));
      if (prof) {
        DGR_HIP_CHECK(hipEventRecord(e1, stream));
        ctx->conv_spans.push_back({e0, e1});
        ctx->gemm_spans.push_back({e0, e1});
        ctx->conv_kinds.push_back(kname);
      }
      LayerRun &r = net->runs[li];
      r = LayerRun();
      r.os = true;
      r.os_launch = o;
      r.nbr = *t;
      r.os_launch.nbr = &r.nbr;
      r.n_in = cin_map.n_dev; r.n_out = cout_map.n_dev; r.K = L.K;
      r.n_out_cap = cout_map.n_cap;
      return DGR_OK;
    }
    const bool small_cin = km && !swapped && !res && L.cin <= 8 && L.cout == 32 && L.cin_pad == 8;
    const char *kname = (L.cin == 6 && L.wq) ? "conv_cin6_quad_kernel" : L.cin == 1 ? "conv_small_cin_row_kernel" : "conv_small_cin_kernel";
    unsigned long long *clk = nullptr;
    const bool wide = L.wb && km;
    if (small_cin)
      DGR_CHECK(dgr_conv_small_cin(in.ptr, in.ld, in.relu, L.cin, L.w, L.wq, L.shift, *km, cout_map.n_dev, cout_map.n_cap,
                                   out.ptr, out.ld, stream));
    else if (wide) {
      DGR_REQUIRE(in.split.planes, "layer %s: the wide-layer kernel needs its input as split rows", L.name.c_str());
      if (prof) {
        DGR_ALLOC(a.clk, ctx->arena, unsigned long long, 2);
        DGR_HIP_CHECK(hipMemsetAsync(a.clk, 0xff, sizeof(unsigned long long), stream));
        DGR_HIP_CHECK(hipMemsetAsync(a.clk + 1, 0, sizeof(unsigned long long), stream));
        clk = a.clk;
      }
      DGR_CHECK(dgr_conv_wide_launch(a, in.split, L.wb, L.wb_piece, L.w_unscale, ctx->num_cus, stream, &kname));
    } else
      DGR_CHECK(dgr_conv_launch(a, ctx->num_cus, stream, &kname));
    if (prof) DGR_HIP_CHECK(hipEventRecord(em, stream));
    DGR_REQUIRE(!out.split.planes || (km && !small_cin), "layer %s: only a reduction can write split rows", L.name.c_str());
    if (km && !small_cin)
      DGR_CHECK(dgr_reduce_rows(ybuf, L.cout, swapped ? km->in_ptr : km->out_ptr, swapped ? km->in_pos : km->out_pos,
                                cout_map.n_dev, cout_map.n_cap, out.split_only ? nullptr : out.ptr, out.ld, L.shift, res ? res->ptr : nullptr,
                                res ? res->ld : 0, res ? res->relu : 0, stream, out.split.planes ? &out.split : nullptr,
                                out.relu));
    if (prof) {
      DGR_HIP_CHECK(hipEventRecord(e1, stream));
      ctx->conv_spans.push_back({e0, e1});
      ctx->gemm_spans.push_back({e0, em});
      ctx->conv_kinds.push_back(kname);
      ctx->conv_clks.resize(ctx->conv_spans.size(), nullptr);
      ctx->conv_clks.back() = clk;
    }
    LayerRun &r = net->runs[li];
    a.clk = nullptr;
    r.launch = a;
    r.split_in = wide ? in.split : DgrSplitRows();
    r.split_out = out.split;
    r.out_relu = out.relu;
    r.split_only = out.split_only;
    r.has_reduce = km != nullptr;
    r.small_cin = small_cin;
    if (km) r.km = *km;
    if (km) {
      r.red_ptr = swapped ? km->in_ptr : km->out_ptr;
      r.red_pos = swapped ? km->in_pos : km->out_pos;
// ... 52 lines not shown
  const Tensor X{const_cast<float *>(feats), net->cin, 0};
  Tensor T1{t1, 32, 0}, Y1{y1, 32, 1}, S1{cat1 + 64, 96, 1};
  Tensor T2{t2, 64, 0}, Y2{y2, 64, 1};
  Tensor S2{cat2 + 64, 128, 1};
  Tensor T4{t4, 128, 0}, Y4{y4, 128, 1}, S4{cat4 + 128, 256, 1};
  Tensor T8{t8, 256, 0}, Y8{y8, 256, 1}, S8{s8, 256, 1};
  Tensor U4{u4, 128, 0}, V4{v4, 128, 1};
  Tensor U2{u2, 64, 0}, V2{v2, 64, 1};
  Tensor U1{u1, 64, 0}, V1{v1, 64, 1};
  Tensor S4T{cat4, 256, 1};
  {
    struct { Tensor *t; int consumer, channels; int64_t rows; bool middle; } sp[] = {
        {&T2, 4, 64, n2, false}, {&Y2, 5, 64, n2, true},
        {&S2, 6, 64, n2, false}, {&T4, 7, 128, n4, false}, {&Y4, 8, 128, n4, true}, {&S4, 9, 128, n4, false},
        {&T8, 10, 256, n8, false}, {&Y8, 11, 256, n8, true}, {&S8, 12, 256, n8, false}, {&U4, 13, 128, n4, false},
        {&V4, 14, 128, n4, true}, {&U2, 16, 64, n2, false}, {&V2, 17, 64, n2, true}, {&U1, 19, 64, n1, false},
        {&V1, 20, 64, n1, true}};
    for (auto &e : sp) {
      if (!net->W->layers[e.consumer].wb) continue;
      e.t->split.channels = e.channels;
      e.t->split_only = e.middle;
      DGR_ALLOC(e.t->split.planes, A, unsigned char, (size_t)e.rows * 4 * e.channels);
      DGR_ALLOC(e.t->split.scale, A, float, e.rows);
    }
  }
  Tensor S2T{cat2, 128, 1};
  const Tensor S1T{cat1, 96, 1};
  const Tensor H{h, 64, 1}, FIN{fin, net->cout, 0};
  Tensor CAT4{cat4, 256, 1}, CAT2{cat2, 128, 1};
  if (use_nbr) {
    const int64_t words = 5 * n1 + 6 * n2 + 6 * n4 + 3 * n8;
    uint32_t *pool;
    DGR_ALLOC(pool, A, uint32_t, words);
    DGR_HIP_CHECK(hipMemsetAsync(pool, 0, (size_t)words * sizeof(uint32_t), stream));
    auto take = [&](int64_t n) { uint32_t *p = pool; pool += n; return p; };
    for (Tensor *t : {&T1, &Y1, &S1, &U1, &V1}) t->amax = take(n1);
    for (Tensor *t : {&T2, &Y2, &S2, &CAT2, &U2, &V2}) t->amax = take(n2);
    for (Tensor *t : {&T4, &Y4, &S4, &CAT4, &U4, &V4}) t->amax = take(n4);
    for (Tensor *t : {&T8, &Y8, &S8}) t->amax = take(n8);
    S2.amax2 = CAT2.amax; S2T.amax2 = CAT2.amax;
    S4.amax2 = CAT4.amax; S4T.amax2 = CAT4.amax;
  }

  if (use_nbr && !getenv("DGR_NO_DSPLIT")) {
    static const bool os_lists = getenv("DGR_OS_LISTS") != nullptr;
    auto dense_layer = [&](int l, int64_t rows) {
      const DgrLayer &L = net->W->layers[l];
      return L.w16b && L.w16d && !dgr_exact_f32() && !os_lists && dgr_conv_dense_supported(L.cin, L.cin_pad, L.cout) &&
             rows * (int64_t)L.cin * 4 < (1ll << 31);
    };
    struct { Tensor *t; int producer; int64_t rows; } mid[] = {{&Y1, 1, n1}, {&Y2, 4, n2}, {&V2, 16, n2}, {&V1, 19, n1}};
    for (auto &e : mid)
      if (dense_layer(e.producer, e.rows) && dense_layer(e.producer + 1, e.rows) && e.t->ld == net->W->layers[e.producer].cout) {
        e.t->dsplit = reinterpret_cast<unsigned char *>(e.t->ptr);
        e.t->dsplit_only = true;
      }
  }

  int li = 0;
  if (conv1_fused) {
    const DgrLayer &L0 = net->W->layers[0];
    int32_t *pc;
    DGR_ALLOC(pc, A, int32_t, 1);
    hipEvent_t e0 = nullptr, e1 = nullptr;
    if (f.prof) {
      e0 = ctx->events.next(); e1 = ctx->events.next();
      DGR_HIP_CHECK(hipEventRecord(e0, stream));
// ... 89 lines not shown
    DGR_HIP_CHECK(hipEventElapsedTime(&t, sp.first, sp.second));
    ctx->conv_span_ms.push_back(t);
  }
  for (auto &sp : ctx->gemm_spans) {
    float t = 0.f;
    DGR_HIP_CHECK(hipEventElapsedTime(&t, sp.first, sp.second));
    ctx->gemm_span_ms.push_back(t);
  }
  ctx->conv_clk_us.assign(ctx->conv_spans.size(), 0.f);
  for (size_t i = 0; i < ctx->conv_clks.size() && i < ctx->conv_clk_us.size(); ++i)
    if (ctx->conv_clks[i]) {
      unsigned long long c[2] = {0, 0};
      DGR_HIP_CHECK(hipMemcpy(c, ctx->conv_clks[i], sizeof(c), hipMemcpyDeviceToHost));
      if (c[1] > c[0]) ctx->conv_clk_us[i] = (float)((double)(c[1] - c[0]) * 0.01);
    }
  return DGR_OK;
}

int dgr_flag_error(int32_t flag) {
  if (flag == 1) {
    dgr_set_error("duplicate coordinates in the sparse tensor input");
    return DGR_EINVAL;
  }
  if (flag == 2) {
    dgr_set_error("kernel-map capacity exceeded (more than the reserved pairs per output row)");
    return DGR_ENOMEM;
  }
  return DGR_OK;
}

static int check_flag(dgr_ctx *ctx, const int32_t *flag_dev, hipStream_t stream) {
  unsigned char *pin;
  DGR_CHECK(dgr_ctx_pinned(ctx, 64, &pin));
  DGR_HIP_CHECK(hipMemcpyAsync(pin, flag_dev, sizeof(int32_t), hipMemcpyDeviceToHost, stream));
  DGR_CHECK(dgr_ctx_wait(ctx, stream));
  return dgr_flag_error(*reinterpret_cast<volatile int32_t *>(pin));
}

int dgr_ctx_new_flag(dgr_ctx *ctx, hipStream_t stream) {
  DGR_ALLOC(ctx->flag_dev, ctx->arena, int32_t, 1);
  DGR_HIP_CHECK(hipMemsetAsync(ctx->flag_dev, 0, sizeof(int32_t), stream));
  return DGR_OK;
}

int dgr_ctx_check_flag(dgr_ctx *ctx, hipStream_t stream) {
  if (!ctx->flag_dev) return DGR_OK;
  return check_flag(ctx, ctx->flag_dev, stream);
}

void dgr_net_invalidate_runs(dgr_net *net) { net->run_generation = ~0ull; }
int dgr_net_out_channels(const dgr_net *net) { return net->cout; }
int dgr_net_in_channels(const dgr_net *net) { return net->cin; }
int dgr_net_dim(const dgr_net *net) { return net->D; }
const dgr_ctx *dgr_net_ctx(const dgr_net *net) { return net->ctx; }

extern "C" int dgr_resunet_forward(dgr_ctx *ctx, dgr_net *net, const int32_t *coords, const float *feats,
                                   int64_t N, float *out, dgr_stream stream_) {
  DGR_REQUIRE(ctx && net && coords && feats && out, "dgr_resunet_forward: NULL argument");
  DGR_REQUIRE(net->ctx == ctx, "dgr_resunet_forward: the net object belongs to another context (one dgr_net per context: "
                               "dgr_net_share gives a second context its own over the same weights)");
  DGR_REQUIRE(N > 0, "dgr_resunet_forward: empty sparse tensor (N=%lld)", (long long)N);
  hipStream_t stream = (hipStream_t)stream_;
  DGR_HIP_CHECK(hipSetDevice(ctx->device));
  DGR_CHECK(ctx->arena.reset());
  DGR_CHECK(dgr_ctx_new_flag(ctx, stream));
  dgr_ctx_begin_profile(ctx);
  DGR_CHECK(dgr_resunet_forward_impl(ctx, net, coords, feats, N, out, stream));
  DGR_CHECK(dgr_ctx_check_flag(ctx, stream));
  if (ctx->profiling) {
    memset(ctx->stage_ms, 0, sizeof(ctx->stage_ms));
    DGR_CHECK(dgr_ctx_collect_profile(ctx));
  }
  return DGR_OK;
}

extern "C" int dgr_debug_conv_layer(dgr_ctx *ctx, dgr_net *net, int layer, const int32_t *coords, const float *in,
                                    int in_relu, int64_t N, float *out, dgr_stream stream_) {
  DGR_REQUIRE(ctx && net && coords && in && out && N > 0, "dgr_debug_conv_layer: bad argument");
  DGR_REQUIRE(layer >= 0 && layer < (int)net->W->layers.size(), "layer %d out of range", layer);
  const DgrLayer &L = net->W->layers[layer];
  int k3 = 1;
  for (int d = 0; d < net->D; ++d) k3 *= 3;
  DGR_REQUIRE(L.K == k3 && L.cin >= 32, "dgr_debug_conv_layer: layer %s is not a 3^D conv with >= 32 input channels", L.name.c_str());
  hipStream_t stream = (hipStream_t)stream_;
  DGR_HIP_CHECK(hipSetDevice(ctx->device));
  DGR_CHECK(ctx->arena.reset());
  DGR_CHECK(dgr_ctx_new_flag(ctx, stream));
  dgr_ctx_begin_profile(ctx);
  DgrArena &A = ctx->arena;
  Fwd f;
  f.ctx = ctx; f.net = net; f.stream = stream; f.prof = false;
  f.ms.overflow = ctx->flag_dev;
  DGR_CHECK(dgr_build_maps(A, coords, N, net->D, 3, &f.ms, stream, false, true, net->D == 3));
  const int64_t n_cap = f.ms.cm[0].n_cap;
// ... 123 lines not shown
```

deepglobalregistration_amd/csrc/pipeline.hip:

```cpp
#include <string.h>

#include "dgr_internal.h"

int dgr_registration_launch_ctx(dgr_ctx *ctx, const float *xyz0, const float *xyz1, const int64_t *idx1,
                                const float *lw, int is_logit, float clip, const int64_t *off0_dev,
                                const int64_t *off0_host, int npairs, int64_t total_rows, float q, int max_iter, int max_break,
                                double ratio, int skip_refine, int gate, float eps, float *weights_out,
                                DgrRegResult *results_dev, hipStream_t stream);
int dgr_ctx_new_flag(dgr_ctx *ctx, hipStream_t stream);
int dgr_ctx_check_flag(dgr_ctx *ctx, hipStream_t stream);
int dgr_net_out_channels(const dgr_net *net);
void dgr_net_invalidate_runs(dgr_net *net);
int dgr_net_in_channels(const dgr_net *net);
int dgr_net_dim(const dgr_net *net);
const dgr_ctx *dgr_net_ctx(const dgr_net *net);

__global__ void inlier_inputs_kernel(const int32_t *__restrict__ coords0, const float *__restrict__ xyz0,
                                     int64_t N0, const int32_t *__restrict__ coords1,
                                     const float *__restrict__ xyz1, const int64_t *__restrict__ idx1,
                                     int feature_type, int32_t *__restrict__ coords6,
                                     float *__restrict__ feats) {
  const int64_t i = (int64_t)blockIdx.x * blockDim.x + threadIdx.x;
  if (i >= N0) return;
  const int64_t j = idx1[i];
// ... 31 lines not shown
              "inlier_feature_type must be 'ones' (0) or 'coords' (1); 'feats' is inconsistent with the "
              "network input width in the reference (deep_global_registration.py:119)");
  DGR_REQUIRE(N0 > 0 && N1 > 0, "dgr_inlier_inputs: empty input");
  DGR_HIP_CHECK(hipSetDevice(ctx->device));
  return dgr_inlier_inputs_impl(coords0, xyz0, N0, coords1, xyz1, idx1, feature_type, coords6_out, feats_out,
                                (hipStream_t)stream);
}

__global__ void sigmoid_clip_sum_kernel(const float *__restrict__ logit, int64_t N, float clip,
                                        float *__restrict__ w_out, double *__restrict__ sum) {
  __shared__ double part[4];
  double s = 0.0;
  for (int64_t i = (int64_t)blockIdx.x * blockDim.x + threadIdx.x; i < N; i += (int64_t)gridDim.x * blockDim.x) {
    float w = 1.f / (1.f + expf(-logit[i]));
    if (clip > 0.f && w < clip) w = 0.f;
    w_out[i] = w;
    s += (double)w;
  }
  for (int d = 32; d > 0; d >>= 1) s += __shfl_down(s, d, 64);
  if ((threadIdx.x & 63) == 0) part[threadIdx.x >> 6] = s;
  __syncthreads();
  if (threadIdx.x == 0) atomicAdd(sum, part[0] + part[1] + part[2] + part[3]);
}

extern "C" int dgr_sigmoid_clip_sum(dgr_ctx *ctx, const float *logit, int64_t N, float clip,
                                    float *weights_out, double *wsum, dgr_stream stream_) {
  DGR_REQUIRE(ctx && logit && weights_out && wsum, "dgr_sigmoid_clip_sum: NULL argument");
  DGR_REQUIRE(N > 0, "dgr_sigmoid_clip_sum: empty input");
  hipStream_t stream = (hipStream_t)stream_;
  DGR_HIP_CHECK(hipSetDevice(ctx->device));
  DGR_CHECK(ctx->arena.reset());
  double *sum;
  DGR_ALLOC(sum, ctx->arena, double, 1);
  DGR_HIP_CHECK(hipMemsetAsync(sum, 0, sizeof(double), stream));
  int blocks = (int)dgr_ceil_div(N, 256);
  if (blocks > 1024) blocks = 1024;
  sigmoid_clip_sum_kernel<<<blocks, 256, 0, stream>>>(logit, N, clip, weights_out, sum);
  DGR_LAUNCH_CHECK();
  DGR_HIP_CHECK(hipMemcpyAsync(wsum, sum, sizeof(double), hipMemcpyDeviceToHost, stream));
  DGR_HIP_CHECK(hipStreamSynchronize(stream));
  return DGR_OK;
}

__global__ void gather_rows3_kernel(const float *__restrict__ src, const int64_t *__restrict__ idx, int64_t N,
                                    float *__restrict__ dst) {
  const int64_t i = (int64_t)blockIdx.x * blockDim.x + threadIdx.x;
  if (i >= N) return;
  const int64_t j = idx[i];
  dst[i * 3] = src[j * 3]; dst[i * 3 + 1] = src[j * 3 + 1]; dst[i * 3 + 2] = src[j * 3 + 2];
}

extern "C" int dgr_gather_rows3(dgr_ctx *ctx, const float *src, const int64_t *idx, int64_t N, float *dst,
                                dgr_stream stream) {
  DGR_REQUIRE(ctx && src && idx && dst && N > 0, "dgr_gather_rows3: bad argument");
  DGR_HIP_CHECK(hipSetDevice(ctx->device));
  gather_rows3_kernel<<<(int)dgr_ceil_div(N, 256), 256, 0, (hipStream_t)stream>>>(src, idx, N, dst);
  DGR_LAUNCH_CHECK();
  return DGR_OK;
}

__global__ void fill_kernel(float *p, int64_t n, float v) {
  for (int64_t i = (int64_t)blockIdx.x * blockDim.x + threadIdx.x; i < n; i += (int64_t)gridDim.x * blockDim.x) p[i] = v;
}

__global__ void override_idx_kernel(int64_t *idx, const int64_t *__restrict__ ovr, int64_t n) {
  const int64_t i = (int64_t)blockIdx.x * blockDim.x + threadIdx.x;
  if (i < n && ovr[i] >= 0) idx[i] = ovr[i];
}

__global__ void concat_coords_kernel(const int32_t *__restrict__ c0, int64_t n0, const int32_t *__restrict__ c1,
                                     int64_t n1, int32_t *__restrict__ out) {
  const int64_t i = (int64_t)blockIdx.x * blockDim.x + threadIdx.x;
  if (i >= n0 + n1) return;
  const int32_t *src = i < n0 ? c0 + i * 4 : c1 + (i - n0) * 4;
  out[i * 4] = src[0] * 2 + (i < n0 ? 0 : 1);
  out[i * 4 + 1] = src[1]; out[i * 4 + 2] = src[2]; out[i * 4 + 3] = src[3];
}

struct StageTimer {
  dgr_ctx *ctx;
  hipStream_t stream;
  hipEvent_t e[9][2];
  bool on;
  int rec(int stage, int which) {
    if (!on) return DGR_OK;
    e[stage][which] = ctx->events.next();
    if (!e[stage][which]) return DGR_EHIP;
    DGR_HIP_CHECK(hipEventRecord(e[stage][which], stream));
    return DGR_OK;
  }
};

struct BatchBuffers {
  int64_t *idx1, *off0_dev;
  int32_t *coords6;
  float *feats6, *logit, *weights;
  DgrRegResult *res_dev;
};

static int alloc_batch_buffers(DgrArena &A, int64_t n0, int npairs, const int64_t *off0, hipStream_t stream,
                               BatchBuffers *B) {
  DGR_ALLOC(B->idx1, A, int64_t, n0);
  DGR_ALLOC(B->coords6, A, int32_t, n0 * 7);
  DGR_ALLOC(B->feats6, A, float, n0 * 6);
  DGR_ALLOC(B->logit, A, float, n0);
  DGR_ALLOC(B->weights, A, float, n0);
  DGR_ALLOC(B->off0_dev, A, int64_t, npairs + 1);
  DGR_ALLOC(B->res_dev, A, DgrRegResult, npairs);
  DGR_HIP_CHECK(hipMemcpyAsync(B->off0_dev, off0, (size_t)(npairs + 1) * sizeof(int64_t), hipMemcpyHostToDevice, stream));
  return DGR_OK;
}

static int register_from_features(dgr_ctx *ctx, dgr_net *inlier, const int32_t *coords0, const float *xyz0,
                                  const int64_t *off0, const int32_t *coords1, const float *xyz1, const int64_t *off1,
                                  const float *F0, const float *F1, int C, int npairs, const dgr_params *prm,
                                  const int64_t *override_idx1, const float *forced_logit, const BatchBuffers &B,
                                  StageTimer &tm, double *ns_per_row, float *T_out, int32_t *status_out,
                                  float *stats_out, hipStream_t stream);

extern "C" int dgr_register_batch(dgr_ctx *ctx, dgr_net *fcgf, dgr_net *inlier, const int32_t *coords0,
                                  const float *xyz0, const int64_t *off0, const int32_t *coords1,
                                  const float *xyz1, const int64_t *off1, int npairs, const dgr_params *prm,
                                  const int64_t *override_idx1, const float *forced_logit, float *T_out,
                                  int32_t *status_out,
                                  float *stats_out, dgr_stream stream_) {
  DGR_REQUIRE(ctx && fcgf && inlier && coords0 && xyz0 && off0 && coords1 && xyz1 && off1 && prm && T_out &&
                  status_out,
              "dgr_register_batch: NULL argument");
  DGR_REQUIRE(npairs >= 1 && npairs <= 65535, "dgr_register_batch: npairs=%d out of range", npairs);
  DGR_REQUIRE(dgr_net_dim(fcgf) == 3 && dgr_net_dim(inlier) == 6 && dgr_net_in_channels(fcgf) == 1,
              "dgr_register_batch: expects the 3-D FCGF net (1 input channel) and the 6-D inlier net");
  const int ftype = prm->inlier_feature_type;
  DGR_REQUIRE((ftype == 0 && dgr_net_in_channels(inlier) == 1) || (ftype == 1 && dgr_net_in_channels(inlier) == 6),
              "inlier_feature_type %d does not match the inlier network input width %d", ftype,
              dgr_net_in_channels(inlier));
  for (int p = 0; p < npairs; ++p)
    DGR_REQUIRE(off0[p + 1] > off0[p] && off1[p + 1] > off1[p], "pair %d is empty", p);
  DGR_REQUIRE(dgr_net_ctx(fcgf) == ctx && dgr_net_ctx(inlier) == ctx,
              "dgr_register_batch: a net object belongs to another context (one dgr_net per context: dgr_net_share)");
  hipStream_t stream = (hipStream_t)stream_;
  DGR_HIP_CHECK(hipSetDevice(ctx->device));
  ctx->last_T64.clear();
  DGR_CHECK(ctx->arena.reset());
  dgr_ctx_begin_profile(ctx);
  DGR_CHECK(dgr_ctx_new_flag(ctx, stream));
  DgrArena &A = ctx->arena;
  const int64_t n0 = off0[npairs], n1 = off1[npairs];
  const int C = dgr_net_out_channels(fcgf);
  StageTimer tm{ctx, stream, {}, ctx->profiling};

  float *F0, *F1, *ones;
  BatchBuffers B;
  DGR_ALLOC(F0, A, float, (n0 + n1) * C);
  F1 = F0 + n0 * C;
  DGR_ALLOC(ones, A, float, n0 + n1);
  DGR_CHECK(alloc_batch_buffers(A, n0, npairs, off0, stream, &B));
  fill_kernel<<<256, 256, 0, stream>>>(ones, n0 + n1, 1.f);

  DGR_CHECK(tm.rec(0, 0));
  {
    DgrArena::Mark mk = A.mark();
    int32_t *coords01;
    DGR_ALLOC(coords01, A, int32_t, (n0 + n1) * 4);
    concat_coords_kernel<<<(int)dgr_ceil_div(n0 + n1, 256), 256, 0, stream>>>(coords0, n0, coords1, n1, coords01);
    DGR_CHECK(dgr_resunet_forward_impl(ctx, fcgf, coords01, ones, n0 + n1, F0, stream));
    A.rewind(mk);
    dgr_net_invalidate_runs(fcgf);
  }
  DGR_CHECK(tm.rec(0, 1));
  return register_from_features(ctx, inlier, coords0, xyz0, off0, coords1, xyz1, off1, F0, F1, C, npairs, prm,
                                override_idx1, forced_logit, B, tm, &ctx->batch_ns_per_row, T_out, status_out, stats_out,
                                stream);
}

static int register_from_features(dgr_ctx *ctx, dgr_net *inlier, const int32_t *coords0, const float *xyz0,
                                  const int64_t *off0, const int32_t *coords1, const float *xyz1, const int64_t *off1,
                                  const float *F0, const float *F1, int C, int npairs, const dgr_params *prm,
                                  const int64_t *override_idx1, const float *forced_logit, const BatchBuffers &B,
                                  StageTimer &tm, double *ns_per_row, float *T_out, int32_t *status_out,
                                  float *stats_out, hipStream_t stream) {
  DgrArena &A = ctx->arena;
  const int64_t n0 = off0[npairs], n1 = off1[npairs];
  const int ftype = prm->inlier_feature_type;
  int64_t *const idx1 = B.idx1, *const off0_dev = B.off0_dev;
  int32_t *const coords6 = B.coords6;
  float *const feats6 = B.feats6, *const logit = B.logit, *const weights = B.weights;
  DgrRegResult *const res_dev = B.res_dev;
  DGR_CHECK(tm.rec(1, 0));
  DGR_CHECK(dgr_knn1_batch_impl(ctx, F0, off0, F1, off1, npairs, C, 0, idx1, nullptr, stream));
  if (override_idx1)
    override_idx_kernel<<<(int)dgr_ceil_div(n0, 256), 256, 0, stream>>>(idx1, override_idx1, n0);
  DGR_CHECK(tm.rec(1, 1));
  DGR_CHECK(tm.rec(2, 0));
  DGR_CHECK(dgr_inlier_inputs_impl(coords0, xyz0, n0, coords1, xyz1, idx1, ftype, coords6, feats6, stream));
  DGR_CHECK(tm.rec(2, 1));
  DGR_CHECK(tm.rec(3, 0));
  {
    DgrArena::Mark mk = A.mark();
    DGR_CHECK(dgr_resunet_forward_impl(ctx, inlier, coords6, feats6, n0, logit, stream));
    A.rewind(mk);
    dgr_net_invalidate_runs(inlier);
  }
  DGR_CHECK(tm.rec(3, 1));
  DGR_CHECK(tm.rec(4, 0));
  const float eps = 1.1920928955078125e-07f;
  DGR_CHECK(dgr_registration_launch_ctx(ctx, xyz0, xyz1, idx1, forced_logit ? forced_logit : logit, 1,
                                        prm->clip_weight_thresh, off0_dev, off0, npairs, n0, 2.f * prm->voxel_size,
                                        prm->max_iter, prm->max_break_count, prm->break_threshold_ratio,
                                        prm->skip_refinement, 1, eps, weights, res_dev, stream));
  DGR_CHECK(tm.rec(4, 1));

  unsigned char *pin;
  DGR_CHECK(dgr_ctx_pinned(ctx, 64 + (size_t)npairs * sizeof(DgrRegResult), &pin));
  const DgrRegResult *res = reinterpret_cast<const DgrRegResult *>(pin + 64);
  DGR_HIP_CHECK(hipMemcpyAsync(pin + 64, res_dev, (size_t)npairs * sizeof(DgrRegResult), hipMemcpyDeviceToHost, stream));
  DGR_HIP_CHECK(hipMemcpyAsync(pin, ctx->flag_dev, sizeof(int32_t), hipMemcpyDeviceToHost, stream));
  DGR_CHECK(dgr_ctx_wait(ctx, stream, (long)(*ns_per_row * (double)(n0 + n1))));
  *ns_per_row = (double)ctx->last_wait_ns / (double)(n0 + n1);
  DGR_CHECK(dgr_flag_error(*reinterpret_cast<volatile int32_t *>(pin)));
  for (int p = 0; p < npairs; ++p)
    if (res[p].status == DGR_STATUS_EXCHANGE_TIMEOUT) {
      dgr_set_error("registration of pair %d: the workgroups sharing the pair lost each other (exchange timed out)", p);
      return DGR_EINTERNAL;
    }
  for (int p = 0; p < npairs; ++p) {
    float *T = T_out + p * 16;
    const DgrRegResult &r = res[p];
    for (int i = 0; i < 16; ++i) T[i] = (i % 5 == 0) ? 1.f : 0.f;
    if (r.status == DGR_STATUS_OK) {
      for (int i = 0; i < 3; ++i) {
        for (int j = 0; j < 3; ++j) T[i * 4 + j] = r.R[i * 3 + j];
        T[i * 4 + 3] = r.t[i];
      }
    }
    status_out[p] = r.status;
    if (stats_out) {
      stats_out[p * 4 + 0] = (float)r.iterations;
      stats_out[p * 4 + 1] = r.loss;
      stats_out[p * 4 + 2] = (float)r.break_count;
      stats_out[p * 4 + 3] = r.wsum;
    }
  }
  ctx->last_T64.assign((size_t)npairs * 16, 0.0);
  for (int i = 0; i < npairs * 16; ++i) ctx->last_T64[i] = (double)T_out[i];
  ctx->last.ptr[0] = idx1;    ctx->last.numel[0] = n0;
  ctx->last.ptr[1] = logit;   ctx->last.numel[1] = n0;
  ctx->last.ptr[2] = weights; ctx->last.numel[2] = n0;
  ctx->last.ptr[3] = F0;      ctx->last.numel[3] = n0 * C;
  ctx->last.ptr[4] = F1;      ctx->last.numel[4] = n1 * C;
  ctx->last.generation = ctx->arena.generation;
  DGR_CHECK(tm.rec(8, 0));
  if (prm->safeguard || prm->use_icp) {
    const DgrArena::Mark mk = A.mark();
    std::vector<double *> rs(npairs, nullptr);
    std::vector<double> Th((size_t)npairs * 16), rsh((size_t)npairs * DGR_RANSAC_RESULT_DOUBLES);
    std::vector<DgrIcpJob> jobs(prm->use_icp ? npairs : 0);
    auto tail = [&]() -> int {
      if (prm->safeguard)
        for (int p = 0; p < npairs; ++p) {
          if (res[p].status != DGR_STATUS_LOW_CONFIDENCE) continue;
          const int64_t m0 = off0[p + 1] - off0[p];
          float *Y;
          DGR_ALLOC(Y, A, float, m0 * 3);
          gather_rows3_kernel<<<(int)dgr_ceil_div(m0, 256), 256, 0, stream>>>(xyz1, idx1 + off0[p], m0, Y);
          DGR_CHECK(dgr_ransac_begin(ctx, xyz0 + off0[p] * 3, Y, m0, 2.0 * prm->voxel_size,
                                     prm->ransac_hypotheses > 0 ? prm->ransac_hypotheses : 4000000, prm->ransac_seed, &rs[p],
                                     stream));
          DGR_HIP_CHECK(hipMemcpyAsync(&rsh[(size_t)p * DGR_RANSAC_RESULT_DOUBLES], rs[p],
                                       DGR_RANSAC_RESULT_DOUBLES * sizeof(double), hipMemcpyDeviceToHost, stream));
          status_out[p] = DGR_STATUS_SAFEGUARD;
        }
      if (prm->use_icp) {
        double *Tinit;
        DGR_ALLOC(Tinit, A, double, (int64_t)npairs * 16);
        for (int i = 0; i < npairs * 16; ++i) Th[i] = T_out[i];
        DGR_HIP_CHECK(hipMemcpyAsync(Tinit, Th.data(), Th.size() * sizeof(double), hipMemcpyHostToDevice, stream));
        for (int p = 0; p < npairs; ++p)
          DGR_CHECK(dgr_icp_begin(ctx, xyz0 + off0[p] * 3, off0[p + 1] - off0[p], xyz1 + off1[p] * 3, off1[p + 1] - off1[p],
                                  2.0 * prm->voxel_size, rs[p] ? rs[p] : Tinit + (int64_t)p * 16, &jobs[p], stream));
      }
      DGR_HIP_CHECK(hipStreamSynchronize(stream));
      for (int p = 0; p < npairs; ++p)
        if (rs[p])
          for (int i = 0; i < 16; ++i) {
            ctx->last_T64[(size_t)p * 16 + i] = rsh[(size_t)p * DGR_RANSAC_RESULT_DOUBLES + i];
            T_out[p * 16 + i] = (float)rsh[(size_t)p * DGR_RANSAC_RESULT_DOUBLES + i];
          }
      if (prm->use_icp) {
        std::vector<char> ran(npairs, 0);
        for (int p = 0; p < npairs; ++p) {
          if (jobs[p].ncell < 1 || jobs[p].ncell > (4 << 20)) {
            status_out[p] |= DGR_STATUS_FLAG_ICP_SKIPPED;
            continue;
          }
          DGR_CHECK(dgr_icp_run(ctx, &jobs[p], 30, 1e-6, 1e-6, stream));
          ran[p] = 1;
        }
        DGR_HIP_CHECK(hipStreamSynchronize(stream));
        for (int p = 0; p < npairs; ++p) {
          if (!ran[p]) continue;
          double Td[16];
          dgr_icp_finish(&jobs[p], Td, nullptr);
          for (int i = 0; i < 16; ++i) {
            ctx->last_T64[(size_t)p * 16 + i] = Td[i];
            T_out[p * 16 + i] = (float)Td[i];
          }
        }
      }
      return DGR_OK;
// ... 67 lines not shown
                                  const int32_t *pair_ids, int npairs, const dgr_params *prm,
                                  const int64_t *override_idx1, const float *forced_logit, float *T_out,
                                  int32_t *status_out, float *stats_out, dgr_stream stream_) {
  DGR_REQUIRE(ctx && inlier && bank_coords && bank_xyz && bank_F && bank_off && pair_ids && prm && T_out && status_out,
              "dgr_register_pairs: NULL argument");
  DGR_REQUIRE(npairs >= 1 && npairs <= 65535, "dgr_register_pairs: npairs=%d out of range", npairs);
  DGR_REQUIRE(nfrag >= 1, "dgr_register_pairs: nfrag=%d", nfrag);
  DGR_REQUIRE(C == 16 || C == 32 || C == 64, "dgr_register_pairs: feature width %d not supported (16, 32, 64)", C);
  DGR_REQUIRE(((uintptr_t)bank_coords & 15) == 0 && ((uintptr_t)bank_F & 15) == 0,
              "dgr_register_pairs: bank_coords and bank_F must be 16-byte aligned");
  DGR_REQUIRE(dgr_net_dim(inlier) == 6, "dgr_register_pairs: expects the 6-D inlier net");
  const int ftype = prm->inlier_feature_type;
  DGR_REQUIRE((ftype == 0 && dgr_net_in_channels(inlier) == 1) || (ftype == 1 && dgr_net_in_channels(inlier) == 6),
              "inlier_feature_type %d does not match the inlier network input width %d", ftype,
              dgr_net_in_channels(inlier));
  DGR_REQUIRE(dgr_net_ctx(inlier) == ctx,
              "dgr_register_pairs: the net object belongs to another context (one dgr_net per context: dgr_net_share)");
  DGR_REQUIRE(bank_off[0] >= 0, "dgr_register_pairs: bank_off[0] = %lld", (long long)bank_off[0]);
  for (int f = 0; f < nfrag; ++f)
    DGR_REQUIRE(bank_off[f + 1] > bank_off[f], "fragment %d of the bank is empty", f);
  std::vector<BankSegment> segs((size_t)2 * npairs);
  std::vector<int64_t> off0(npairs + 1, 0), off1(npairs + 1, 0);
  for (int s = 0; s < 2; ++s) {
    std::vector<int64_t> &off = s ? off1 : off0;
    for (int p = 0; p < npairs; ++p) {
      const int32_t f = pair_ids[2 * p + s];
      DGR_REQUIRE(f >= 0 && f < nfrag, "pair %d: fragment id %d outside [0, %d)", p, f, nfrag);
      off[p + 1] = off[p] + (bank_off[f + 1] - bank_off[f]);
      segs[(size_t)s * npairs + p] = {bank_off[f], off[p], bank_off[f + 1] - bank_off[f], p, s};
    }
  }
  const int64_t n0 = off0[npairs], n1 = off1[npairs];
  for (int p = 0; p < npairs; ++p) segs[(size_t)npairs + p].dst += n0;
  hipStream_t stream = (hipStream_t)stream_;
  DGR_HIP_CHECK(hipSetDevice(ctx->device));
  ctx->last_T64.clear();
  DGR_CHECK(ctx->arena.reset());
  dgr_ctx_begin_profile(ctx);
  DGR_CHECK(dgr_ctx_new_flag(ctx, stream));
  DgrArena &A = ctx->arena;
  StageTimer tm{ctx, stream, {}, ctx->profiling};

  int32_t *coords;
  float *xyz, *F0;
  BankSegment *segs_dev;
  BatchBuffers B;
  DGR_ALLOC(F0, A, float, (n0 + n1) * C);
  DGR_ALLOC(coords, A, int32_t, (n0 + n1) * 4);
  DGR_ALLOC(xyz, A, float, (n0 + n1) * 3);
  DGR_ALLOC(segs_dev, A, BankSegment, segs.size());
  auto run = [&]() -> int {
    DGR_CHECK(alloc_batch_buffers(A, n0, npairs, off0.data(), stream, &B));
    DGR_CHECK(tm.rec(0, 0));
    DGR_HIP_CHECK(hipMemcpyAsync(segs_dev, segs.data(), segs.size() * sizeof(BankSegment), hipMemcpyHostToDevice, stream));
    bank_gather_kernel<<<(int)dgr_ceil_div(n0 + n1, BANK_GATHER_ROWS), BANK_GATHER_ROWS, 0, stream>>>(
        reinterpret_cast<const int4 *>(bank_coords), bank_xyz, reinterpret_cast<const float4 *>(bank_F), segs_dev,
        2 * npairs, n0 + n1, C == 16 ? 2 : C == 32 ? 3 : 4, reinterpret_cast<int4 *>(coords), xyz,
        reinterpret_cast<float4 *>(F0));
    DGR_LAUNCH_CHECK();
    DGR_CHECK(tm.rec(0, 1));
    return register_from_features(ctx, inlier, coords, xyz, off0.data(), coords + n0 * 4, xyz + n0 * 3, off1.data(), F0,
                                  F0 + n0 * C, C, npairs, prm, override_idx1, forced_logit, B, tm, &ctx->pairs_ns_per_row,
                                  T_out, status_out, stats_out, stream);
  };
  const int rc = run();
  if (rc != DGR_OK) (void)hipStreamSynchronize(stream);
  return rc;
}

extern "C" int dgr_register_batch_f64(dgr_ctx *ctx, double *T_out, int64_t capacity_pairs, int64_t *npairs) {
  DGR_REQUIRE(ctx && npairs, "dgr_register_batch_f64: NULL argument");
  const int64_t n = (int64_t)(ctx->last_T64.size() / 16);
  DGR_REQUIRE(n > 0, "no dgr_register_batch has run on this ctx");
  *npairs = n;
  if (T_out) {
    DGR_REQUIRE(capacity_pairs >= n, "destination buffer too small");
    memcpy(T_out, ctx->last_T64.data(), (size_t)n * 16 * sizeof(double));
  }
  return DGR_OK;
}

extern "C" int dgr_register_batch_output(dgr_ctx *ctx, int which, void *dst_dev, int64_t capacity_bytes,
                                         int64_t *numel, dgr_stream stream) {
  DGR_REQUIRE(ctx && numel && which >= 0 && which < 5, "dgr_register_batch_output: bad argument");
  DGR_REQUIRE(ctx->last.ptr[which] != nullptr, "no dgr_register_batch has run on this ctx");
  DGR_REQUIRE(ctx->last.generation == ctx->arena.generation,
              "the outputs of the last dgr_register_batch are gone: a later call on this context reused its workspace "
              "(fetch them before the next library call)");
  *numel = ctx->last.numel[which];
  if (dst_dev) {
    const int64_t bytes = ctx->last.numel[which] * (which == 0 ? 8 : 4);
    DGR_REQUIRE(capacity_bytes >= bytes, "destination buffer too small");
    DGR_HIP_CHECK(hipMemcpyAsync(dst_dev, ctx->last.ptr[which], (size_t)bytes, hipMemcpyDeviceToDevice,
                                 (hipStream_t)stream));
  }
  return DGR_OK;
}
```

deepglobalregistration_amd/csrc/reg.hip:

```cpp
#include "dgr_internal.h"
#include "svd3.h"

#ifndef DGR_REG_THREADS
#define DGR_REG_THREADS 256
#endif
constexpr int REG_THREADS = DGR_REG_THREADS;
constexpr int REG_WAVES = REG_THREADS / 64;

constexpr int REG_CLMAX = 8;
constexpr int REG_XG = 64;
constexpr int REG_SPIN_LIMIT = 4000000;
#ifndef DGR_REG_CLUSTER_MAX
#define DGR_REG_CLUSTER_MAX REG_CLMAX
#endif
__host__ __device__ inline int reg_cluster_size(int n) {
  const int cl = n >= 16384 ? 8 : n >= 8192 ? 4 : n >= 4096 ? 2 : 1;
  return cl < DGR_REG_CLUSTER_MAX ? cl : DGR_REG_CLUSTER_MAX;
}

struct RegArgs {
  unsigned long long *xbuf;
  int pair_base;
  const float *xyz0, *xyz1;
  const int64_t *idx1;
// ... 453 lines not shown
  }
  if (it >= a.max_iter) it = a.max_iter - 1;
  if (tid == 0 && cj == 0) {
    Ortho o;
    ortho_forward(prm, o);
    res->R[0] = o.x[0]; res->R[1] = o.y[0]; res->R[2] = o.z[0];
    res->R[3] = o.x[1]; res->R[4] = o.y[1]; res->R[5] = o.z[1];
    res->R[6] = o.x[2]; res->R[7] = o.y[2]; res->R[8] = o.z[2];
    res->t[0] = prm[6]; res->t[1] = prm[7]; res->t[2] = prm[8];
    res->iterations = it;
    res->break_count = breaks;
    res->loss = loss;
#ifdef DGR_REG_TIMING
    printf("reg timing: m=%d iters=%d cycles/iter: points %lld reduce %lld update %lld\n", m, it + 1,
           tsum[0] / (it + 1), tsum[1] / (it + 1), tsum[2] / (it + 1));
#endif
  }
}

constexpr int REG_MAX_SPINNERS = 64;
static int launch_registration(dgr_ctx *ctx, const float *xyz0, const float *xyz1, const int64_t *idx1,
                               const float *lw, int is_logit, float clip, const int64_t *off0_dev, const int64_t *off0_host,
                               int npairs, int64_t total_rows, float q, int max_iter, int max_break,
                               double ratio, int skip_refine, int gate, float eps, float *weights_out,
                               DgrRegResult *results_dev, hipStream_t stream, const double *state_in = nullptr,
                               double *state_out = nullptr) {
  RegArgs a;
  a.xyz0 = xyz0; a.xyz1 = xyz1; a.idx1 = idx1; a.lw = lw; a.off0 = off0_dev;
  a.weights_out = weights_out; a.res = results_dev;
  const int64_t crows = total_rows + (int64_t)npairs * REG_CLMAX * REG_THREADS;
  DGR_ALLOC(a.cA, ctx->arena, float4, crows);
  DGR_ALLOC(a.cB, ctx->arena, float4, crows);
  DGR_ALLOC(a.xbuf, ctx->arena, unsigned long long, (int64_t)npairs * 2 * REG_CLMAX * REG_XG);
  DGR_HIP_CHECK(hipMemsetAsync(a.xbuf, 0, (size_t)npairs * 2 * REG_CLMAX * REG_XG * sizeof(unsigned long long), stream));
  a.clip = clip; a.q = q; a.eps = eps;
  a.is_logit = is_logit; a.gate = gate; a.skip_refine = skip_refine;
  a.max_iter = max_iter; a.max_break = max_break; a.ratio = ratio;
  a.state_in = state_in; a.state_out = state_out;
  for (int p0 = 0; p0 < npairs;) {
    int p1 = p0, spinners = 0;
    while (p1 < npairs && p1 - p0 < 4096) {
      const int cl = off0_host ? reg_cluster_size((int)(off0_host[p1 + 1] - off0_host[p1])) : REG_CLMAX;
      const int add = cl > 1 ? cl : 0;
      if (p1 > p0 && spinners + add > REG_MAX_SPINNERS) break;
      spinners += add;
      ++p1;
    }
    a.pair_base = p0;
    registration_kernel<<<(p1 - p0) * REG_CLMAX, REG_THREADS, 0, stream>>>(a);
    DGR_LAUNCH_CHECK();
    p0 = p1;
  }
  return DGR_OK;
}

int dgr_registration_launch_ctx(dgr_ctx *ctx, const float *xyz0, const float *xyz1, const int64_t *idx1,
                                const float *lw, int is_logit, float clip, const int64_t *off0_dev,
                                const int64_t *off0_host, int npairs, int64_t total_rows, float q, int max_iter, int max_break,
                                double ratio, int skip_refine, int gate, float eps, float *weights_out,
                                DgrRegResult *results_dev, hipStream_t stream) {
  return launch_registration(ctx, xyz0, xyz1, idx1, lw, is_logit, clip, off0_dev, off0_host, npairs, total_rows, q,
                             max_iter, max_break, ratio, skip_refine, gate, eps, weights_out, results_dev,
                             stream);
}

static int run_single(dgr_ctx *ctx, const float *X, const float *Y, const float *w, int64_t N, float q,
                      int max_iter, int max_break, double ratio, int skip_refine, float eps,
                      DgrRegResult *host_res, hipStream_t stream, const double *state_in_host = nullptr,
                      double *state_out_host = nullptr) {
  DGR_REQUIRE(ctx && X && Y && w, "registration: NULL argument");
  DGR_REQUIRE(N > 0 && N < (1ll << 31), "registration: N=%lld out of range", (long long)N);
  DGR_REQUIRE(skip_refine || max_iter >= 1, "GlobalRegistration: max_iter must be >= 1");
  DGR_HIP_CHECK(hipSetDevice(ctx->device));
  DGR_CHECK(ctx->arena.reset());
  int64_t *off;
  DgrRegResult *res;
  DGR_ALLOC(off, ctx->arena, int64_t, 2);
  DGR_ALLOC(res, ctx->arena, DgrRegResult, 1);
  const int64_t h_off[2] = {0, N};
  DGR_HIP_CHECK(hipMemcpyAsync(off, h_off, sizeof(h_off), hipMemcpyHostToDevice, stream));
  double *st_in = nullptr, *st_out = nullptr;
  if (state_in_host) {
    DGR_ALLOC(st_in, ctx->arena, double, 30);
    DGR_HIP_CHECK(hipMemcpyAsync(st_in, state_in_host, 30 * sizeof(double), hipMemcpyHostToDevice, stream));
  }
  if (state_out_host) {
    DGR_ALLOC(st_out, ctx->arena, double, 30);
    DGR_HIP_CHECK(hipMemsetAsync(st_out, 0, 30 * sizeof(double), stream));
  }
  DGR_CHECK(launch_registration(ctx, X, Y, nullptr, w, 0, 0.f, off, h_off, 1, N, q, max_iter, max_break, ratio,
                                skip_refine, 0, eps, nullptr, res, stream, st_in, st_out));
  DGR_HIP_CHECK(hipMemcpyAsync(host_res, res, sizeof(DgrRegResult), hipMemcpyDeviceToHost, stream));
  if (state_out_host) DGR_HIP_CHECK(hipMemcpyAsync(state_out_host, st_out, 30 * sizeof(double), hipMemcpyDeviceToHost, stream));
  DGR_HIP_CHECK(hipStreamSynchronize(stream));
  if (host_res->status == DGR_STATUS_EXCHANGE_TIMEOUT) {
    dgr_set_error("registration: the workgroups sharing a pair lost each other (exchange timed out)");
    return DGR_EINTERNAL;
  }
  if (host_res->status == DGR_STATUS_SVD_FAILED) {
    dgr_set_error("weighted Procrustes: non-finite covariance, SVD failed");
    return DGR_ESVD;
  }
  return DGR_OK;
}

extern "C" int dgr_weighted_procrustes(dgr_ctx *ctx, const float *X, const float *Y, const float *w,
                                       int64_t N, float eps, float *R9, float *t3, dgr_stream stream) {
  DGR_REQUIRE(R9 && t3, "dgr_weighted_procrustes: NULL output");
  DgrRegResult r;
  DGR_CHECK(run_single(ctx, X, Y, w, N, 1.f, 1, 1, 0.0, 1, eps, &r, (hipStream_t)stream));
  for (int i = 0; i < 9; ++i) R9[i] = r.R[i];
  for (int i = 0; i < 3; ++i) t3[i] = r.t[i];
  return DGR_OK;
}

extern "C" int dgr_se3_refine(dgr_ctx *ctx, const float *X, const float *Y, const float *w, int64_t N,
                              float quantization_size, int max_iter, int max_break_count,
                              double break_threshold_ratio, float *R9, float *t3, int32_t *iterations,
                              float *loss, int32_t *break_count, dgr_stream stream) {
  DGR_REQUIRE(R9 && t3, "dgr_se3_refine: NULL output");
  DgrRegResult r;
  const float eps = 1.1920928955078125e-07f;
  DGR_CHECK(run_single(ctx, X, Y, w, N, quantization_size, max_iter, max_break_count, break_threshold_ratio, 0,
                       eps, &r, (hipStream_t)stream));
  for (int i = 0; i < 9; ++i) R9[i] = r.R[i];
  for (int i = 0; i < 3; ++i) t3[i] = r.t[i];
// ... 69 lines not shown
```

deepglobalregistration_amd/ops.py:

```python
import ctypes as C

import numpy as np
import torch

from . import _lib
from ._lib import check, get_ctx, ptr, stream_ptr, vp

F32_EPS = float(np.finfo(np.float32).eps)


def _dev(t):
    if not (torch.is_tensor(t) and t.is_cuda):
        raise ValueError('expected a CUDA(ROCm) tensor')
    return t.device


def _as(t, dtype, device):
    if not torch.is_tensor(t):
        t = torch.as_tensor(np.asarray(t))
    return t.to(device=device, dtype=dtype).contiguous()


def voxelize(xyz, voxel_size, batch_index=0, device='cuda'):
    lib = _lib.load()
# ... 838 lines not shown
    n = C.c_int(0)
    check(_lib.load().dgr_ctx_stage_times_v2(get_ctx(device), t, 16, C.byref(n)))
    names = ['fcgf', 'knn', 'inlier_inputs', 'inlier_net', 'registration', 'maps_3d', 'maps_6d', 'conv_kernels', 'o3d_steps']
    out = dict(zip(names, [float(v) for v in t[:n.value]]))
    out['conv_launches'] = int(_lib.load().dgr_ctx_conv_launches(get_ctx(device)))
    return out


def conv_launch_times(device):
    cap = 4096
    t, g = (C.c_float * cap)(), (C.c_float * cap)()
    n = C.c_int64(0)
    check(_lib.load().dgr_ctx_conv_launch_times(get_ctx(device), t, g, cap, C.byref(n)))
    return [float(t[i]) for i in range(n.value)], [float(g[i]) for i in range(n.value)]


def conv_launch_kernel_us(device):
    cap = 4096
    t = (C.c_float * cap)()
    n = C.c_int64(0)
    check(_lib.load().dgr_ctx_conv_launch_kernel_us(get_ctx(device), t, cap, C.byref(n)))
    return [float(t[i]) for i in range(n.value)]


def conv_launch_kinds(device):
    cap = 1 << 16
    buf = C.create_string_buffer(cap)
    n = C.c_int64(0)
    check(_lib.load().dgr_ctx_conv_launch_kinds(get_ctx(device), buf, cap, C.byref(n)))
    names = buf.value.decode().split('\n')
    return names[:n.value]


def debug_ortho2rotation(p6, grad_R=None):
    dev = _dev(p6)
    p6 = _as(p6, torch.float32, dev).reshape(-1, 6)
    n = p6.shape[0]
    R = torch.empty((n, 3, 3), dtype=torch.float32, device=dev)
    g = dp = None
    if grad_R is not None:
        g = _as(grad_R, torch.float32, dev).reshape(n, 9)
        dp = torch.empty((n, 6), dtype=torch.float32, device=dev)
    check(_lib.load().dgr_debug_ortho2rotation(get_ctx(dev), ptr(p6), n, ptr(g), ptr(R), ptr(dp), stream_ptr(dev.index)))
    return (R, dp) if grad_R is not None else R


def debug_smooth_l1(X, Y, quantization_size):
    dev = _dev(X)
    X, Y = _as(X, torch.float32, dev), _as(Y, torch.float32, dev)
    out = torch.empty(X.shape[0], dtype=torch.float32, device=dev)
    check(_lib.load().dgr_debug_smooth_l1(get_ctx(dev), ptr(X), ptr(Y), X.shape[0], float(quantization_size), ptr(out),
                                          stream_ptr(dev.index)))
    return out
```

include/dgr_hip.h:

```cpp
#ifndef DGR_HIP_H
#define DGR_HIP_H

#include <stdint.h>

#ifdef __cplusplus
extern "C" {
#endif

typedef struct dgr_ctx dgr_ctx;
typedef struct dgr_net dgr_net;
typedef struct dgr_maps dgr_maps;
typedef void *dgr_stream;

enum {
  DGR_OK = 0,
  DGR_EINVAL = -1,
  DGR_EHIP = -2,
  DGR_ENOMEM = -3,
  DGR_ESVD = -4,
  DGR_EINTERNAL = -5
};

enum { DGR_STATUS_OK = 0, DGR_STATUS_LOW_CONFIDENCE = 1, DGR_STATUS_SVD_FAILED = 2,
       DGR_STATUS_SAFEGUARD = 3 ,
// ... 94 lines not shown
  int max_iter;
  int max_break_count;
  double break_threshold_ratio;
  int skip_refinement;
  int safeguard;
  int64_t ransac_hypotheses;
  uint32_t ransac_seed;
  int use_icp;
} dgr_params;

int dgr_register_batch(dgr_ctx *ctx, dgr_net *fcgf, dgr_net *inlier, const int32_t *coords0,
                       const float *xyz0, const int64_t *off0, const int32_t *coords1,
                       const float *xyz1, const int64_t *off1, int npairs, const dgr_params *params,
                       const int64_t *override_idx1, const float *forced_logit, float *T_out,
                       int32_t *status_out,
                       float *stats_out, dgr_stream stream);
int dgr_register_pairs(dgr_ctx *ctx, dgr_net *inlier, const int32_t *bank_coords, const float *bank_xyz,
                       const float *bank_F, const int64_t *bank_off, int nfrag, int C, const int32_t *pair_ids,
                       int npairs, const dgr_params *params, const int64_t *override_idx1,
                       const float *forced_logit, float *T_out, int32_t *status_out, float *stats_out,
                       dgr_stream stream);
int dgr_register_batch_output(dgr_ctx *ctx, int which, void *dst_dev, int64_t capacity_bytes,
                              int64_t *numel, dgr_stream stream);
int dgr_register_batch_f64(dgr_ctx *ctx, double *T_out, int64_t capacity_pairs, int64_t *npairs);

int dgr_ctx_set_profiling(dgr_ctx *ctx, int enable);
#define DGR_NUM_STAGE_TIMES 9
int dgr_ctx_stage_times_v2(dgr_ctx *ctx, float *times_ms, int capacity, int *n);
int dgr_ctx_stage_times(dgr_ctx *ctx, float *times_ms);
int64_t dgr_ctx_conv_launches(dgr_ctx *ctx);
int dgr_ctx_conv_launch_times(dgr_ctx *ctx, float *times_ms, float *gemm_ms, int64_t capacity, int64_t *n);
int dgr_ctx_conv_launch_kernel_us(dgr_ctx *ctx, float *us, int64_t capacity, int64_t *n);
int dgr_ctx_conv_launch_kinds(dgr_ctx *ctx, char *buf, int64_t capacity, int64_t *n);

int dgr_radius_pairs_batch(dgr_ctx *ctx, const float *xyz0, const int64_t *off0, const float *xyz1,
                           const int64_t *off1, int npairs, const double *T, double radius, int K,
                           int32_t *counts_out, int64_t *pairs_out, int64_t capacity, int64_t *total_out,
                           dgr_stream stream);
int dgr_pairs_isin_batch(dgr_ctx *ctx, const int64_t *pos, const int64_t *pos_off, const int64_t *pred,
                         const int64_t *pred_off, int npairs, const int64_t *M_per_pair, uint8_t *out,
                         dgr_stream stream);
int dgr_validation_counts(dgr_ctx *ctx, const uint8_t *label, const float *weights, float threshold,
                          const int64_t *off, int npairs, int64_t *counts_out, dgr_stream stream);

#define DGR_SCORE_WIDTH 11
int dgr_score_pairs(dgr_ctx *ctx, const float *bank_xyz, const int64_t *bank_off, int nfrag, const int32_t *pair_ids,
                    int npairs, const double *T, double radius, double *sums_out, dgr_stream stream);

#define DGR_PG_MAX_NODES 128
typedef struct {
  double mu;
  int reference_node;
  int max_iter;
  double rel_tol;
} dgr_pg_params;
int dgr_pose_graph_optimize(dgr_ctx *ctx, int ngraphs, const int64_t *node_off, const int64_t *edge_off,
                            const int32_t *edge_ids, const double *edge_T, const double *edge_info,
                            const uint8_t *edge_uncertain, const double *pose_init, const dgr_pg_params *params,
                            double *pose_out, double *line_out, double *stats_out, dgr_stream stream);

#define DGR_VM_FRAC_BITS 40
int dgr_voxel_mean(dgr_ctx *ctx, const void *xyz, int is_f64, const int64_t *off, int nfrag, const int32_t *frag_ids,
                   int nsel, const double *T, const double *origin, double voxel_size, int64_t *first_out,
                   int32_t *coords_out, int32_t *count_out, int64_t *fsum_out, double *mean_out, int64_t *n_out,
                   int64_t *dropped_out, dgr_stream stream);

// ... 17 lines not shown
```

Measured before the change: 395.1.

## Fuse coordinate-map and grid-setup kernels to cut launch count

Reduces kernel launches across the coordinate-map and grid setup. It fuses grid layout with grid clearing, builds all four stride levels of coordinate hash tables in batched grid.y launches, and uses a single-workgroup or two-pass scan for small arrays. It also adds a launch counter wrapper for memsets and memcpys, with an env switch that restores the old unfused path. The cost is redundant per-block layout computation and a quadratic in-block prefix over block sums in the raw scan.

New measurement: 390.5. 0.988x the previous value.

```diff
diff --git a/deepglobalregistration_amd/_lib.py b/deepglobalregistration_amd/_lib.py
--- a/deepglobalregistration_amd/_lib.py
+++ b/deepglobalregistration_amd/_lib.py
@@ -85,6 +85,7 @@
     'dgr_ctx_conv_launch_times': (C.c_int, [vp, c_f32p, c_f32p, C.c_int64, C.POINTER(C.c_int64)]),
     'dgr_ctx_conv_launch_kernel_us': (C.c_int, [vp, c_f32p, C.c_int64, C.POINTER(C.c_int64)]),
     'dgr_ctx_conv_launch_kinds': (C.c_int, [vp, C.c_char_p, C.c_int64, C.POINTER(C.c_int64)]),
+    'dgr_ctx_launches': (C.c_int64, [vp]),
     'dgr_radius_pairs_batch': (C.c_int, [vp, vp, c_i64p, vp, c_i64p, C.c_int, c_f64p, C.c_double, C.c_int, vp, vp,
                                          C.c_int64, c_i64p, vp]),
     'dgr_pairs_isin_batch': (C.c_int, [vp, vp, c_i64p, vp, c_i64p, C.c_int, c_i64p, vp, vp]),
diff --git a/deepglobalregistration_amd/csrc/conv.hip b/deepglobalregistration_amd/csrc/conv.hip
--- a/deepglobalregistration_amd/csrc/conv.hip
+++ b/deepglobalregistration_amd/csrc/conv.hip
@@ -873,6 +873,44 @@
     *reinterpret_cast<int4 *>(cells + i) = make_int4(-1, -1, -1, -1);
 }
 
+__global__ void __launch_bounds__(256)
+    grid_layout_clear_kernel(DgrGridMeta *m, int pad, long long cap, int32_t *__restrict__ cells) {
+  static_assert(GRID_MAXB == 64, "one lane per batch element");
+  __shared__ long long total_s;
+  __shared__ int ok_s;
+  if (threadIdx.x < 64) {
+    const int b = threadIdx.x;
+    const bool write = blockIdx.x == 0;
+    long long vol = 0;
+    if (m->mx[b][0] >= m->mn[b][0]) {
+      vol = 1;
+      for (int d = 0; d < 3; ++d) {
+        const long long e = (long long)m->mx[b][d] - m->mn[b][d] + 1 + 2 * pad;
+        if (write) m->dim[b][d] = (int32_t)(e < (1ll << 30) ? e : (1ll << 30));
+        vol = (vol <= cap && e <= cap) ? vol * e : cap + 1;
+      }
+    }
+    long long incl = vol;
+#pragma unroll
+    for (int s = 1; s < 64; s <<= 1) {
+      const long long up = __shfl_up(incl, s, 64);
+      if (b >= s) incl += up;
+    }
+    if (write) m->base[b] = incl - vol;
+    const long long total = __shfl(incl, 63, 64);
+    if (b == 0) {
+      total_s = total <= cap ? total : cap + 1;
+      ok_s = (!m->bad && total <= cap) ? 1 : 0;
+      if (write) { m->total = total_s; m->ok = ok_s; }
+    }
+  }
+  __syncthreads();
+  if (!ok_s) return;
+  const long long total = total_s;
+  for (long long i = ((long long)blockIdx.x * blockDim.x + threadIdx.x) * 4; i < total; i += (long long)gridDim.x * blockDim.x * 4)
+    *reinterpret_cast<int4 *>(cells + i) = make_int4(-1, -1, -1, -1);
+}
+
 __device__ __forceinline__ long long grid_cell(const DgrGridMeta *m, int b, int x, int y, int z, int pad) {
   const long long dx = m->dim[b][0], dy = m->dim[b][1];
   return m->base[b] + ((long long)(z - m->mn[b][2] + pad) * dy + (y - m->mn[b][1] + pad)) * dx + (x - m->mn[b][0] + pad);
@@ -1085,7 +1123,7 @@
                     const float *w_tiled, const float *shift, float *out, int out_ld, int32_t *pair_count,
                     hipStream_t stream, const float *w_compact, const char **kernel_name, uint32_t *out_amax) {
   DGR_REQUIRE(cin >= 1 && cin <= 8 && ks % 2 == 1, "conv1 probe: cin=%d ks=%d", cin, ks);
-  if (pair_count && ks > 7) DGR_HIP_CHECK(hipMemsetAsync(pair_count, 0, sizeof(int32_t), stream));
+  if (pair_count && ks > 7) DGR_HIP_CHECK(dgr_memset_async(pair_count, 0, sizeof(int32_t), stream));
   const int32_t *grid_done = nullptr;
   if (ks <= 7) {
     static const long long cap = 64ll << 20;
@@ -1096,8 +1134,13 @@
     DGR_ALLOC(cells, arena, int32_t, cap + 4);
     grid_init_kernel<<<1, 64, 0, stream>>>(meta, pair_count);
     grid_bbox_kernel<<<(int)dgr_ceil_div(cm.n_cap, 256), 256, 0, stream>>>(cm.coords, cm.n_dev, meta);
-    grid_layout_kernel<<<1, 64, 0, stream>>>(meta, ks >> 1, cap);
-    grid_clear_kernel<<<2048, 256, 0, stream>>>(meta, cells);
+    const bool layout_apart = dgr_maps_unfused();
+    if (layout_apart) {
+      grid_layout_kernel<<<1, 64, 0, stream>>>(meta, ks >> 1, cap);
+      grid_clear_kernel<<<2048, 256, 0, stream>>>(meta, cells);
+    } else {
+      grid_layout_clear_kernel<<<2048, 256, 0, stream>>>(meta, ks >> 1, cap, cells);
+    }
     const bool mfma = cin == 1 && w_compact && (out_ld & 3) == 0 && (ks == 3 || ks == 5 || ks == 7);
     grid_fill_kernel<<<(int)dgr_ceil_div(cm.n_cap, 256), 256, 0, stream>>>(cm.coords, cm.n_dev, meta, ks >> 1, cells,
                                                                            mfma ? in : nullptr, in_ld);
@@ -1122,7 +1165,7 @@
                                                        out, out_ld, pair_count, out_amax);
     if (kernel_name) *kernel_name = "conv1_grid_kernel";
     }
-    DGR_LAUNCH_CHECK();
+    DGR_LAUNCH_CHECK(layout_apart ? 6 : 5);
     grid_done = &meta->ok;
     arena.rewind(mk);
   }
diff --git a/deepglobalregistration_amd/csrc/coordmap.hip b/deepglobalregistration_amd/csrc/coordmap.hip
--- a/deepglobalregistration_amd/csrc/coordmap.hip
+++ b/deepglobalregistration_amd/csrc/coordmap.hip
@@ -29,8 +29,8 @@
   return base + x - v;
 }
 
-__global__ void __launch_bounds__(1024) scan_single_block(const int32_t *__restrict__ in, int64_t n,
-                                                          int32_t *__restrict__ out, int32_t *total_out) {
+__device__ __forceinline__ void scan_one_workgroup(const int32_t *__restrict__ in, int64_t n, int32_t *__restrict__ out,
+                                                   int32_t *total_out) {
   __shared__ int wsum[16];
   __shared__ int carry_s;
   const int lane = threadIdx.x & 63, wave = threadIdx.x >> 6;
@@ -57,6 +57,11 @@
     __syncthreads();
   }
   if (threadIdx.x == 0 && total_out) *total_out = carry_s;
+}
+
+__global__ void __launch_bounds__(1024) scan_single_block(const int32_t *__restrict__ in, int64_t n,
+                                                          int32_t *__restrict__ out, int32_t *total_out) {
+  scan_one_workgroup(in, n, out, total_out);
 }
 
 struct ScanJobs {
@@ -99,6 +104,7 @@
   if (threadIdx.x == 0 && j.total[a]) *j.total[a] = carry;
 }
 
+template <bool RAW>
 __global__ void __launch_bounds__(SCAN_THREADS) scan_final_multi(ScanJobs j) {
   __shared__ int lds[4];
   const int a = blockIdx.y;
@@ -106,6 +112,14 @@
   const int32_t *in = j.in[a];
   int32_t *out = j.out[a];
   const long long n = j.n[a];
+  int before;
+  if (RAW) {
+    int part = 0;
+    for (int i = threadIdx.x; i < (int)blockIdx.x; i += SCAN_THREADS) part += j.sums[a][i];
+    block_exclusive_scan_256(part, lds, &before);
+  } else {
+    before = j.sums[a][blockIdx.x];
+  }
   long long base = (long long)blockIdx.x * SCAN_BLOCK + (long long)threadIdx.x * SCAN_ITEMS;
   int v[SCAN_ITEMS];
   int s = 0;
@@ -115,12 +129,18 @@
     s += v[i];
   }
   int tot;
-  int ex = block_exclusive_scan_256(s, lds, &tot) + j.sums[a][blockIdx.x];
+  int ex = block_exclusive_scan_256(s, lds, &tot) + before;
 #pragma unroll
   for (int i = 0; i < SCAN_ITEMS; ++i) {
     if (base + i < n) out[base + i] = ex;
     ex += v[i];
   }
+  if (RAW && (int)blockIdx.x == j.nblocks[a] - 1 && threadIdx.x == 0 && j.total[a]) *j.total[a] = before + tot;
+}
+
+__global__ void __launch_bounds__(1024) scan_single_block_multi(ScanJobs j) {
+  const int a = blockIdx.x;
+  scan_one_workgroup(j.in[a], j.n[a], j.out[a], j.total[a]);
 }
 
 int dgr_exclusive_scan_multi(DgrArena &arena, int count, const int32_t *const *in, int32_t *const *out, const int64_t *n,
@@ -128,6 +148,19 @@
   DGR_REQUIRE(count >= 1 && count <= DGR_SCAN_MAX, "scan: %d arrays", count);
   ScanJobs j;
   int maxb = 0;
+  int64_t max_n = 0;
+  for (int a = 0; a < count; ++a) max_n = std::max(max_n, n[a]);
+  if (max_n <= (1 << 14) && !dgr_maps_unfused()) {
+    for (int a = 0; a < DGR_SCAN_MAX; ++a) {
+      const bool on = a < count;
+      DGR_REQUIRE(!on || n[a] > 0, "scan: empty array");
+      j.in[a] = on ? in[a] : nullptr; j.out[a] = on ? out[a] : nullptr; j.sums[a] = nullptr;
+      j.total[a] = on && total_out ? total_out[a] : nullptr; j.n[a] = on ? n[a] : 0; j.nblocks[a] = 0;
+    }
+    scan_single_block_multi<<<count, 1024, 0, stream>>>(j);
+    DGR_LAUNCH_CHECK();
+    return DGR_OK;
+  }
   for (int a = 0; a < count; ++a) {
     DGR_REQUIRE(n[a] > 0, "scan: empty array");
     j.in[a] = in[a]; j.out[a] = out[a]; j.total[a] = total_out ? total_out[a] : nullptr; j.n[a] = n[a];
@@ -137,16 +170,21 @@
   }
   for (int a = count; a < DGR_SCAN_MAX; ++a) { j.in[a] = nullptr; j.out[a] = j.sums[a] = j.total[a] = nullptr; j.n[a] = 0; j.nblocks[a] = 0; }
   scan_block_sums_multi<<<dim3(maxb, count), SCAN_THREADS, 0, stream>>>(j);
+  if (maxb <= 2048 && !dgr_maps_unfused()) {
+    scan_final_multi<true><<<dim3(maxb, count), SCAN_THREADS, 0, stream>>>(j);
+    DGR_LAUNCH_CHECK(2);
+    return DGR_OK;
+  }
   scan_sums_serial_multi<<<count, SCAN_THREADS, 0, stream>>>(j);
-  scan_final_multi<<<dim3(maxb, count), SCAN_THREADS, 0, stream>>>(j);
-  DGR_LAUNCH_CHECK();
+  scan_final_multi<false><<<dim3(maxb, count), SCAN_THREADS, 0, stream>>>(j);
+  DGR_LAUNCH_CHECK(3);
   return DGR_OK;
 }
 
 int dgr_exclusive_scan_i32(DgrArena &arena, const int32_t *in, int32_t *out, int64_t n,
                            int32_t *total_out, hipStream_t stream) {
   if (n <= 0) {
-    if (total_out) DGR_HIP_CHECK(hipMemsetAsync(total_out, 0, sizeof(int32_t), stream));
+    if (total_out) DGR_HIP_CHECK(dgr_memset_async(total_out, 0, sizeof(int32_t), stream));
     return DGR_OK;
   }
   if (n <= (1 << 14)) {
@@ -246,11 +284,11 @@
   uint32_t cap = dgr_next_pow2((uint64_t)(2 * n_cap > 64 ? 2 * n_cap : 64));
   int32_t *table;
   DGR_ALLOC(table, arena, int32_t, cap);
-  DGR_HIP_CHECK(hipMemsetAsync(table, 0xff, (size_t)cap * sizeof(int32_t), stream));
+  DGR_HIP_CHECK(dgr_memset_async(table, 0xff, (size_t)cap * sizeof(int32_t), stream));
   unique_insert<NC><<<grid_for(n_cap), 256, 0, stream>>>(keys, n_dev, n_cap, table, cap - 1);
   unique_flag<NC><<<grid_for(n_cap), 256, 0, stream>>>(keys, n_dev, n_cap, table, cap - 1, first_flag,
                                                       nullptr);
-  DGR_LAUNCH_CHECK();
+  DGR_LAUNCH_CHECK(2);
   DGR_CHECK(dgr_exclusive_scan_i32(arena, first_flag, rank, n_cap, n_unique_dev, stream));
   *table_out = table;
   *mask_out = cap - 1;
@@ -270,25 +308,164 @@
   return DGR_EINVAL;
 }
 
+template <int NK, int STRIDE>
+__device__ __forceinline__ void masked_key(const int32_t *__restrict__ rows, int64_t r, int32_t m, int32_t *me) {
+  me[0] = rows[r * STRIDE];
+#pragma unroll
+  for (int d = 1; d < NK; ++d) me[d] = rows[r * STRIDE + d] & m;
+}
+
+template <int NK, int STRIDE>
+__device__ __forceinline__ bool masked_key_equal(const int32_t *__restrict__ rows, int64_t r, int32_t m, const int32_t *me) {
+  bool eq = rows[r * STRIDE] == me[0];
+#pragma unroll
+  for (int d = 1; d < NK; ++d) eq &= ((rows[r * STRIDE + d] & m) == me[d]);
+  return eq;
+}
+
+template <int NK, int STRIDE>
+__device__ __forceinline__ void masked_insert(const int32_t *__restrict__ rows, int64_t r, int32_t m, int32_t *table,
+                                              uint32_t mask) {
+  int32_t me[NK];
+  masked_key<NK, STRIDE>(rows, r, m, me);
+  uint32_t slot = dgr_hash_row<NK>(me) & mask;
+  while (true) {
+    int cur = __hip_atomic_load(&table[slot], __ATOMIC_RELAXED, __HIP_MEMORY_SCOPE_AGENT);
+    if (cur == DGR_EMPTY) {
+      int old = atomicCAS(&table[slot], DGR_EMPTY, (int)r);
+      if (old == DGR_EMPTY) return;
+      cur = old;
+    }
+    if (masked_key_equal<NK, STRIDE>(rows, cur, m, me)) {
+      atomicMin(&table[slot], (int)r);
+      return;
+    }
+    slot = (slot + 1) & mask;
+  }
+}
+
+template <int NK, int STRIDE>
+__device__ __forceinline__ int masked_first_row(const int32_t *__restrict__ rows, int64_t r, int32_t m,
+                                                const int32_t *__restrict__ table, uint32_t mask) {
+  int32_t me[NK];
+  masked_key<NK, STRIDE>(rows, r, m, me);
+  uint32_t slot = dgr_hash_row<NK>(me) & mask;
+  while (true) {
+    const int v = table[slot];
+    if (v == DGR_EMPTY) return -1;
+    if (masked_key_equal<NK, STRIDE>(rows, v, m, me)) return v;
+    slot = (slot + 1) & mask;
+  }
+}
+
+struct LevelJobs {
+  const int32_t *coords;
+  int64_t n;
+  int32_t *tables;
+  uint32_t cap;
+  int32_t *flag, *rank;
+  int32_t *out_coords[4];
+  int32_t *n_dev;
+  int32_t *dup_flag;
+};
+
+template <int NC>
+__global__ void levels_insert(LevelJobs j) {
+  const int l = blockIdx.y;
+  const int64_t r = (int64_t)blockIdx.x * blockDim.x + threadIdx.x;
+  if (l == 0 && r == 0) j.n_dev[0] = (int32_t)j.n;
+  if (r >= j.n) return;
+  masked_insert<NC, NC>(j.coords, r, ~((1 << l) - 1), j.tables + (size_t)l * j.cap, j.cap - 1);
+}
+
+template <int NC>
+__global__ void levels_flag(LevelJobs j) {
+  const int l = blockIdx.y;
+  const int64_t r = (int64_t)blockIdx.x * blockDim.x + threadIdx.x;
+  if (r >= j.n) return;
+  const int first = masked_first_row<NC, NC>(j.coords, r, ~((1 << l) - 1), j.tables + (size_t)l * j.cap, j.cap - 1) == (int)r;
+  if (l == 0) {
+    if (!first) *j.dup_flag = 1;
+  } else {
+    j.flag[(int64_t)(l - 1) * j.n + r] = first;
+  }
+}
+
+template <int NC>
+__global__ void levels_compact_relabel(LevelJobs j) {
+  const int l = blockIdx.y + 1;
+  const int64_t i = (int64_t)blockIdx.x * blockDim.x + threadIdx.x;
+  const int32_t *flag = j.flag + (int64_t)(l - 1) * j.n, *rank = j.rank + (int64_t)(l - 1) * j.n;
+  if (i < j.n && flag[i]) {
+    int32_t me[NC];
+    masked_key<NC, NC>(j.coords, i, ~((1 << l) - 1), me);
+    const int64_t o = rank[i];
+#pragma unroll
+    for (int d = 0; d < NC; ++d) j.out_coords[l][o * NC + d] = me[d];
+  }
+  if (i < (int64_t)j.cap) {
+    int32_t *table = j.tables + (size_t)l * j.cap;
+    const int v = table[i];
+    if (v >= 0) table[i] = rank[v];
+  }
+}
+
+template <int NC>
+static int build_coord_maps_levels(DgrArena &arena, const int32_t *coords, int64_t N, DgrMapSet *ms, hipStream_t stream) {
+  const uint32_t cap = dgr_next_pow2((uint64_t)(2 * N > 64 ? 2 * N : 64));
+  LevelJobs j = {};
+  j.coords = coords; j.n = N; j.cap = cap; j.dup_flag = ms->overflow;
+  DGR_ALLOC(j.n_dev, arena, int32_t, 4);
+  DGR_ALLOC(j.tables, arena, int32_t, 4 * (size_t)cap);
+  DGR_ALLOC(j.flag, arena, int32_t, 3 * N);
+  DGR_ALLOC(j.rank, arena, int32_t, 3 * N);
+  for (int l = 0; l < 4; ++l) {
+    DgrCoordMap &c = ms->cm[l];
+    c.ts = 1 << l;
+    c.n_cap = N;
+    c.n_dev = j.n_dev + l;
+    c.table = j.tables + (size_t)l * cap;
+    c.table_mask = cap - 1;
+    if (l == 0) c.coords = const_cast<int32_t *>(coords);
+    else DGR_ALLOC(c.coords, arena, int32_t, N * NC);
+    j.out_coords[l] = c.coords;
+  }
+  DGR_HIP_CHECK(dgr_memset_async(j.tables, 0xff, 4 * (size_t)cap * sizeof(int32_t), stream));
+  const unsigned gx = (unsigned)dgr_ceil_div(N, 256);
+  levels_insert<NC><<<dim3(gx, 4), 256, 0, stream>>>(j);
+  levels_flag<NC><<<dim3(gx, 4), 256, 0, stream>>>(j);
+  DGR_LAUNCH_CHECK(2);
+  {
+    const int32_t *ins[3] = {j.flag, j.flag + N, j.flag + 2 * N};
+    int32_t *outs[3] = {j.rank, j.rank + N, j.rank + 2 * N}, *tots[3] = {j.n_dev + 1, j.n_dev + 2, j.n_dev + 3};
+    const int64_t ns[3] = {N, N, N};
+    DGR_CHECK(dgr_exclusive_scan_multi(arena, 3, ins, outs, ns, tots, stream));
+  }
+  levels_compact_relabel<NC><<<dim3((unsigned)dgr_ceil_div((int64_t)cap, 256), 3), 256, 0, stream>>>(j);
+  DGR_LAUNCH_CHECK();
+  return DGR_OK;
+}
+
 template <int NC>
 static int build_coord_maps_t(DgrArena &arena, const int32_t *coords, int64_t N, DgrMapSet *ms,
                               hipStream_t stream) {
+  if (!dgr_maps_unfused()) return build_coord_maps_levels<NC>(arena, coords, N, ms, stream);
   DgrCoordMap &c1 = ms->cm[0];
   c1.coords = const_cast<int32_t *>(coords);
   c1.n_cap = N;
   c1.ts = 1;
   DGR_ALLOC(c1.n_dev, arena, int32_t, 1);
   int32_t n32 = (int32_t)N;
-  DGR_HIP_CHECK(hipMemcpyAsync(c1.n_dev, &n32, sizeof(int32_t), hipMemcpyHostToDevice, stream));
+  DGR_HIP_CHECK(dgr_memcpy_async(c1.n_dev, &n32, sizeof(int32_t), hipMemcpyHostToDevice, stream));
   {
     uint32_t cap = dgr_next_pow2((uint64_t)(2 * N > 64 ? 2 * N : 64));
     DGR_ALLOC(c1.table, arena, int32_t, cap);
     c1.table_mask = cap - 1;
-    DGR_HIP_CHECK(hipMemsetAsync(c1.table, 0xff, (size_t)cap * sizeof(int32_t), stream));
+    DGR_HIP_CHECK(dgr_memset_async(c1.table, 0xff, (size_t)cap * sizeof(int32_t), stream));
     unique_insert<NC><<<grid_for(N), 256, 0, stream>>>(coords, nullptr, N, c1.table, cap - 1);
     unique_flag<NC><<<grid_for(N), 256, 0, stream>>>(coords, nullptr, N, c1.table, cap - 1, nullptr,
                                                     ms->overflow);
-    DGR_LAUNCH_CHECK();
+    DGR_LAUNCH_CHECK(2);
   }
   for (int l = 1; l < 4; ++l) {
     DgrCoordMap &p = ms->cm[l - 1];
@@ -308,7 +485,7 @@
                                                              c.coords, nullptr);
     table_relabel<<<grid_for((int64_t)c.table_mask + 1), 256, 0, stream>>>(c.table, c.table_mask + 1,
                                                                            rank);
-    DGR_LAUNCH_CHECK();
+    DGR_LAUNCH_CHECK(3);
   }
   return DGR_OK;
 }
@@ -382,9 +559,168 @@
   if (v >= 0) j.table[l][s] = j.inv[l][v];
 }
 
+struct HbJobs {
+  const int32_t *coords[4];
+  const int32_t *n_dev[4];
+  int64_t n_cap[4];
+  int32_t *table[4];
+  uint32_t mask[4];
+  int32_t *flag[4], *rank[4], *bkeys[4], *row_bucket[4], *counts[4], *cursor[4], *start[4];
+  int32_t *members[4];
+  int4 *second[4];
+  int32_t *coords_new[4], *canon[4], *inv[4];
+  int32_t *cm_table[4];
+  uint32_t cm_cap[4];
+};
+
+__global__ void hb_insert_kernel(HbJobs j) {
+  const int l = blockIdx.y;
+  const int64_t r = (int64_t)blockIdx.x * blockDim.x + threadIdx.x;
+  if (r >= j.n_cap[l] || r >= *j.n_dev[l]) return;
+  masked_insert<4, 7>(j.coords[l], r, -1, j.table[l], j.mask[l]);
+}
+
+__global__ void hb_flag_kernel(HbJobs j) {
+  const int l = blockIdx.y;
+  const int64_t r = (int64_t)blockIdx.x * blockDim.x + threadIdx.x;
+  if (r >= j.n_cap[l]) return;
+  j.flag[l][r] = r < *j.n_dev[l] ? (masked_first_row<4, 7>(j.coords[l], r, -1, j.table[l], j.mask[l]) == (int)r) : 0;
+}
+
+__global__ void hb_count_kernel(HbJobs j) {
+  const int l = blockIdx.y;
+  const int64_t r = (int64_t)blockIdx.x * blockDim.x + threadIdx.x;
+  if (r >= j.n_cap[l] || r >= *j.n_dev[l]) return;
+  const int first = masked_first_row<4, 7>(j.coords[l], r, -1, j.table[l], j.mask[l]);
+  const int b = j.rank[l][first];
+  j.row_bucket[l][r] = b;
+  atomicAdd(&j.counts[l][b], 1);
+  if (first == (int)r) {
+#pragma unroll
+    for (int d = 0; d < 4; ++d) j.bkeys[l][(int64_t)b * 4 + d] = j.coords[l][r * 7 + d];
+  }
+}
+
+__global__ void hb_members_kernel(HbJobs j, int first_level) {
+  const int l = first_level + blockIdx.y;
+  const int64_t r = (int64_t)blockIdx.x * blockDim.x + threadIdx.x;
+  if (r >= j.n_cap[l] || r >= *j.n_dev[l]) return;
+  const int b = j.row_bucket[l][r];
+  j.members[l][j.start[l][b] + atomicAdd(&j.cursor[l][b], 1)] = (int32_t)r;
+}
+
+__global__ void hb_fill_kernel(HbJobs j) {
+  const int l = blockIdx.y;
+  const int64_t r = (int64_t)blockIdx.x * blockDim.x + threadIdx.x;
+  if (r >= j.n_cap[l] || r >= *j.n_dev[l]) return;
+  const int32_t *start = j.start[l], *members = j.members[l];
+  const int b = j.row_bucket[l][r];
+  const int32_t *c = j.coords[l] + r * 7;
+  int p;
+  if (members) {
+    int rank = 0;
+    for (int e = start[b], end = start[b + 1]; e < end; ++e) rank += members[e] < (int32_t)r;
+    p = start[b] + rank;
+  } else {
+    p = start[b] + atomicAdd(&j.cursor[l][b], 1);
+  }
+  if (j.coords_new[l]) {
+#pragma unroll
+    for (int d = 0; d < 7; ++d) j.coords_new[l][(int64_t)p * 7 + d] = c[d];
+    j.canon[l][p] = (int32_t)r;
+    j.inv[l][r] = p;
+    j.second[l][p] = make_int4(c[4], c[5], c[6], p);
+  } else {
+    j.second[l][p] = make_int4(c[4], c[5], c[6], (int32_t)r);
+  }
+}
+
+__global__ void hb_tables_kernel(HbJobs j) {
+  const int l = blockIdx.y;
+  const uint32_t s = blockIdx.x * blockDim.x + threadIdx.x;
+  if (s <= j.mask[l]) {
+    const int v = j.table[l][s];
+    if (v >= 0) j.table[l][s] = j.rank[l][v];
+  }
+  if (j.cm_table[l] && s < j.cm_cap[l]) {
+    const int v = j.cm_table[l][s];
+    if (v >= 0) j.cm_table[l][s] = j.inv[l][v];
+  }
+}
+
+static int build_half_buckets_levels(DgrArena &arena, DgrCoordMap *cm, DgrHalfBuckets *hb, int levels, int renumber_from,
+                                     hipStream_t stream) {
+  HbJobs j = {};
+  int32_t *nb_dev[4];
+  size_t table_words = 0, count_words = 0;
+  int64_t max_n = 0, max_slots = 0;
+  for (int l = 0; l < levels; ++l) {
+    const int64_t n = cm[l].n_cap;
+    j.mask[l] = dgr_next_pow2((uint64_t)(2 * n > 64 ? 2 * n : 64)) - 1;
+    table_words += (size_t)j.mask[l] + 1;
+    count_words += 2 * (size_t)(n + 1);
+    max_n = std::max(max_n, n);
+    max_slots = std::max<int64_t>(max_slots, (int64_t)j.mask[l] + 1);
+  }
+  int32_t *tables, *cnts;
+  DGR_ALLOC(tables, arena, int32_t, table_words);
+  DGR_ALLOC(cnts, arena, int32_t, count_words);
+  DGR_HIP_CHECK(dgr_memset_async(tables, 0xff, table_words * sizeof(int32_t), stream));
+  DGR_HIP_CHECK(dgr_memset_async(cnts, 0, count_words * sizeof(int32_t), stream));
+  for (int l = 0; l < levels; ++l) {
+    const int64_t n = cm[l].n_cap;
+    j.coords[l] = cm[l].coords; j.n_dev[l] = cm[l].n_dev; j.n_cap[l] = n;
+    j.table[l] = tables; tables += (size_t)j.mask[l] + 1;
+    j.counts[l] = cnts; j.cursor[l] = cnts + (n + 1); cnts += 2 * (n + 1);
+    DGR_ALLOC(j.flag[l], arena, int32_t, n);
+    DGR_ALLOC(j.rank[l], arena, int32_t, n);
+    DGR_ALLOC(nb_dev[l], arena, int32_t, 1);
+    DGR_ALLOC(j.row_bucket[l], arena, int32_t, n);
+    DGR_ALLOC(j.bkeys[l], arena, int32_t, n * 4);
+    DGR_ALLOC(j.start[l], arena, int32_t, n + 1);
+    DGR_ALLOC(j.second[l], arena, int4, n);
+    if (l >= renumber_from) {
+      DGR_ALLOC(j.members[l], arena, int32_t, n);
+      DGR_ALLOC(j.coords_new[l], arena, int32_t, n * 7);
+      DGR_ALLOC(j.canon[l], arena, int32_t, n);
+      DGR_ALLOC(j.inv[l], arena, int32_t, n);
+      j.cm_table[l] = cm[l].table; j.cm_cap[l] = cm[l].table_mask + 1;
+      max_slots = std::max<int64_t>(max_slots, j.cm_cap[l]);
+    }
+    hb[l].table = j.table[l]; hb[l].mask = j.mask[l];
+    hb[l].bkeys = j.bkeys[l]; hb[l].start = j.start[l]; hb[l].second = j.second[l];
+  }
+  const dim3 rows((unsigned)dgr_ceil_div(max_n, 256), (unsigned)levels);
+  hb_insert_kernel<<<rows, 256, 0, stream>>>(j);
+  hb_flag_kernel<<<rows, 256, 0, stream>>>(j);
+  DGR_LAUNCH_CHECK(2);
+  const int32_t *ins[4];
+  int32_t *outs[4], *tots[4];
+  int64_t ns[4];
+  for (int l = 0; l < levels; ++l) { ins[l] = j.flag[l]; outs[l] = j.rank[l]; tots[l] = nb_dev[l]; ns[l] = cm[l].n_cap; }
+  DGR_CHECK(dgr_exclusive_scan_multi(arena, levels, ins, outs, ns, tots, stream));
+  hb_count_kernel<<<rows, 256, 0, stream>>>(j);
+  DGR_LAUNCH_CHECK();
+  for (int l = 0; l < levels; ++l) { ins[l] = j.counts[l]; outs[l] = j.start[l]; tots[l] = nullptr; ns[l] = cm[l].n_cap + 1; }
+  DGR_CHECK(dgr_exclusive_scan_multi(arena, levels, ins, outs, ns, tots, stream));
+  if (levels > renumber_from) {
+    hb_members_kernel<<<dim3(rows.x, (unsigned)(levels - renumber_from)), 256, 0, stream>>>(j, renumber_from);
+    DGR_LAUNCH_CHECK();
+  }
+  hb_fill_kernel<<<rows, 256, 0, stream>>>(j);
+  hb_tables_kernel<<<dim3((unsigned)dgr_ceil_div(max_slots, 256), (unsigned)levels), 256, 0, stream>>>(j);
+  DGR_LAUNCH_CHECK(2);
+  for (int l = 0; l < levels; ++l) {
+    if (j.coords_new[l]) { cm[l].coords = j.coords_new[l]; cm[l].canon = j.canon[l]; }
+    hb[l].built = true;
+  }
+  return DGR_OK;
+}
+
 int dgr_build_half_buckets(DgrArena &arena, DgrCoordMap *cm, DgrHalfBuckets *hb, int levels, int renumber_from,
                            hipStream_t stream) {
   DGR_REQUIRE(levels >= 1 && levels <= 4 && renumber_from >= 1, "half buckets: %d levels", levels);
+  if (!dgr_maps_unfused()) return build_half_buckets_levels(arena, cm, hb, levels, renumber_from, stream);
   int32_t *keys[4], *flag[4], *rank[4], *nb_dev[4], *row_bucket[4], *counts[4], *cursor[4];
   uint32_t cap[4];
   size_t table_words = 0, count_words = 0;
@@ -397,8 +733,8 @@
   int32_t *tables, *cnts;
   DGR_ALLOC(tables, arena, int32_t, table_words);
   DGR_ALLOC(cnts, arena, int32_t, count_words);
-  DGR_HIP_CHECK(hipMemsetAsync(tables, 0xff, table_words * sizeof(int32_t), stream));
-  DGR_HIP_CHECK(hipMemsetAsync(cnts, 0, count_words * sizeof(int32_t), stream));
+  DGR_HIP_CHECK(dgr_memset_async(tables, 0xff, table_words * sizeof(int32_t), stream));
+  DGR_HIP_CHECK(dgr_memset_async(cnts, 0, count_words * sizeof(int32_t), stream));
   for (int l = 0; l < levels; ++l) {
     const int64_t n = cm[l].n_cap;
     hb[l].table = tables; tables += cap[l];
@@ -419,7 +755,7 @@
     unique_insert<4><<<grid_for(n), 256, 0, stream>>>(keys[l], cm[l].n_dev, n, hb[l].table, hb[l].mask);
     unique_flag<4><<<grid_for(n), 256, 0, stream>>>(keys[l], cm[l].n_dev, n, hb[l].table, hb[l].mask, flag[l], nullptr);
   }
-  DGR_LAUNCH_CHECK();
+  DGR_LAUNCH_CHECK(3 * levels);
   {
     const int32_t *ins[4];
     int32_t *outs[4], *tots[4];
@@ -434,7 +770,7 @@
     bucket_count_kernel<<<grid_for(n), 256, 0, stream>>>(keys[l], cm[l].n_dev, hb[l].table, hb[l].mask, hb[l].bkeys, row_bucket[l],
                                                          counts[l]);
   }
-  DGR_LAUNCH_CHECK();
+  DGR_LAUNCH_CHECK(3 * levels);
   {
     const int32_t *ins[4];
     int32_t *outs[4], *tots[4];
@@ -467,7 +803,7 @@
     hb[l].built = true;
   }
   if (nrj) renumber_table_kernel<<<dim3((unsigned)grid_for(max_cap), nrj), 256, 0, stream>>>(rj);
-  DGR_LAUNCH_CHECK();
+  DGR_LAUNCH_CHECK(levels + nrj + (nrj ? 1 : 0));
   return DGR_OK;
 }
 
@@ -533,7 +869,7 @@
   }
   DGR_LAUNCH_CHECK();
   int32_t n32 = 0;
-  DGR_HIP_CHECK(hipMemcpyAsync(&n32, n_dev, sizeof(int32_t), hipMemcpyDeviceToHost, stream));
+  DGR_HIP_CHECK(dgr_memcpy_async(&n32, n_dev, sizeof(int32_t), hipMemcpyDeviceToHost, stream));
   DGR_HIP_CHECK(hipStreamSynchronize(stream));
   *n_out = n32;
   return DGR_OK;
diff --git a/deepglobalregistration_amd/csrc/ctx.hip b/deepglobalregistration_amd/csrc/ctx.hip
--- a/deepglobalregistration_amd/csrc/ctx.hip
+++ b/deepglobalregistration_amd/csrc/ctx.hip
@@ -259,6 +259,10 @@
   return DGR_OK;
 }
 
+thread_local int64_t *dgr_tls_launches = nullptr;
+
+extern "C" int64_t dgr_ctx_launches(dgr_ctx *ctx) { return ctx ? ctx->launches : 0; }
+
 extern "C" int dgr_ctx_conv_launch_kinds(dgr_ctx *ctx, char *buf, int64_t capacity, int64_t *n) {
   DGR_REQUIRE(ctx != nullptr && buf != nullptr && n != nullptr && capacity > 0, "bad argument");
   std::string all;
diff --git a/deepglobalregistration_amd/csrc/dgr_internal.h b/deepglobalregistration_amd/csrc/dgr_internal.h
--- a/deepglobalregistration_amd/csrc/dgr_internal.h
+++ b/deepglobalregistration_amd/csrc/dgr_internal.h
@@ -33,7 +33,29 @@
     }                              \
   } while (0)
 
-#define DGR_LAUNCH_CHECK() DGR_HIP_CHECK(hipGetLastError())
+extern thread_local int64_t *dgr_tls_launches;
+inline void dgr_count_launches(int n) {
+  if (dgr_tls_launches) *dgr_tls_launches += n;
+}
+#define DGR_LAUNCH_COUNT_ARG(_0, n, ...) n
+#define DGR_LAUNCH_CHECK(...)                                               \
+  do {                                                                      \
+    dgr_count_launches(DGR_LAUNCH_COUNT_ARG(0, ##__VA_ARGS__, 1, 0));       \
+    DGR_HIP_CHECK(hipGetLastError());                                       \
+  } while (0)
+inline hipError_t dgr_memset_async(void *dst, int value, size_t bytes, hipStream_t stream) {
+  dgr_count_launches(1);
+  return hipMemsetAsync(dst, value, bytes, stream);
+}
+inline hipError_t dgr_memcpy_async(void *dst, const void *src, size_t bytes, hipMemcpyKind kind, hipStream_t stream) {
+  dgr_count_launches(1);
+  return hipMemcpyAsync(dst, src, bytes, kind, stream);
+}
+
+inline bool dgr_maps_unfused() {
+  static const bool on = getenv("DGR_MAPS_UNFUSED") != nullptr;
+  return on;
+}
 
 inline bool dgr_exact_f32() {
   static const bool on = getenv("DGR_EXACT_F32") != nullptr;
@@ -251,6 +273,15 @@
   size_t pin_bytes = 0;
   hipStream_t part_stream = nullptr;
   int all_cus = 256;
+  int64_t launches = 0;
+};
+
+struct DgrLaunchScope {
+  int64_t *prev;
+  explicit DgrLaunchScope(dgr_ctx *ctx) : prev(dgr_tls_launches) { if (ctx) dgr_tls_launches = &ctx->launches; }
+  ~DgrLaunchScope() { dgr_tls_launches = prev; }
+  DgrLaunchScope(const DgrLaunchScope &) = delete;
+  DgrLaunchScope &operator=(const DgrLaunchScope &) = delete;
 };
 
 int dgr_ctx_pinned(dgr_ctx *ctx, size_t bytes, unsigned char **out);
diff --git a/deepglobalregistration_amd/csrc/kmap.hip b/deepglobalregistration_amd/csrc/kmap.hip
--- a/deepglobalregistration_amd/csrc/kmap.hip
+++ b/deepglobalregistration_amd/csrc/kmap.hip
@@ -498,7 +498,7 @@
     const size_t w_out = (size_t)(n_cap + 1) * KW, w_in = need_in_csr ? (size_t)(n_in_cap + 1) * KW : 0;
     DGR_ALLOC(mask_out, arena, uint32_t, w_out + w_in);
     if (need_in_csr) mask_in = mask_out + w_out;
-    DGR_HIP_CHECK(hipMemsetAsync(mask_out, 0, (w_out + w_in) * sizeof(uint32_t), stream));
+    DGR_HIP_CHECK(dgr_memset_async(mask_out, 0, (w_out + w_in) * sizeof(uint32_t), stream));
   }
   DGR_ALLOC(cnt_out, arena, int32_t, n_cap + 1);
   if (need_in_csr) DGR_ALLOC(cnt_in, arena, int32_t, n_in_cap + 1);
@@ -523,7 +523,7 @@
   kmap_fill<<<dim3(RB, (K + KM_KGROUP - 1) / KM_KGROUP), KM_THREADS, 0, stream>>>(
       out.n_dev, RB, K, n_cap, hits, counts, base, km->pair_in, km->pair_out, km->pair_cap, overflow, KW, mask_out,
       km->out_ptr, km->out_pos, mask_in, km->in_ptr, km->in_pos, km->pair_k);
-  DGR_LAUNCH_CHECK();
+  DGR_LAUNCH_CHECK(need_in_csr ? 5 : 4);
   arena.rewind(mk);
   km->built = true;
   return DGR_OK;
@@ -563,7 +563,7 @@
       words += (size_t)(t[m].n_cap + 1) * KW + (jobs[m].need_in_csr ? (size_t)(t[m].n_in_cap + 1) * KW : 0) + (size_t)(t[m].n_cap + 1);
     uint32_t *pool;
     DGR_ALLOC(pool, arena, uint32_t, words);
-    DGR_HIP_CHECK(hipMemsetAsync(pool, 0, words * sizeof(uint32_t), stream));
+    DGR_HIP_CHECK(dgr_memset_async(pool, 0, words * sizeof(uint32_t), stream));
     for (int m = 0; m < nj; ++m) {
       t[m].mask_out = pool; pool += (size_t)(t[m].n_cap + 1) * KW;
       t[m].mask_in = nullptr;
@@ -626,7 +626,7 @@
       if (nm) mask_count_multi<KW><<<dim3((unsigned)dgr_ceil_div(max_rows, 256), (unsigned)nm), 256, 0, stream>>>(mj);
     }
   }
-  DGR_LAUNCH_CHECK();
+  DGR_LAUNCH_CHECK(3);
   {
     const int32_t *ins[DGR_SCAN_MAX];
     int32_t *outs[DGR_SCAN_MAX], *tots[DGR_SCAN_MAX];
@@ -665,7 +665,7 @@
     }
     kmap_place_hits<<<dim3((unsigned)max_pb, (unsigned)nj), KM_THREADS, 0, stream>>>(pj);
   }
-  DGR_LAUNCH_CHECK();
+  DGR_LAUNCH_CHECK(3);
   arena.rewind(mk);
   return DGR_OK;
 }
@@ -844,7 +844,7 @@
   ms->conv1_ks = conv1_ks;
   if (!ms->overflow) {
     DGR_ALLOC(ms->overflow, arena, int32_t, 1);
-    DGR_HIP_CHECK(hipMemsetAsync(ms->overflow, 0, sizeof(int32_t), stream));
+    DGR_HIP_CHECK(dgr_memset_async(ms->overflow, 0, sizeof(int32_t), stream));
   }
   DGR_CHECK(dgr_build_coord_maps(arena, coords, N, ms, stream));
   if (nbr_tables) {
@@ -872,7 +872,7 @@
       }
       cls_count_kernel<<<dim3((unsigned)max_nb, 3), KM_THREADS, 0, stream>>>(cj);
       cls_fill_kernel<<<dim3((unsigned)max_nb, 3), KM_THREADS, 0, stream>>>(cj);
-      DGR_LAUNCH_CHECK();
+      DGR_LAUNCH_CHECK(2);
     }
     if (lean) {
       if (conv1_ks != 3 && !skip_conv1_map)
@@ -916,6 +916,7 @@
 extern "C" int dgr_maps_create(dgr_ctx *ctx, const int32_t *coords, int64_t N, int D,
                                int conv1_kernel_size, dgr_maps **out, dgr_stream stream_) {
   DGR_REQUIRE(ctx && coords && out, "dgr_maps_create: NULL argument");
+  DgrLaunchScope launch_scope(ctx);
   hipStream_t stream = (hipStream_t)stream_;
   DGR_HIP_CHECK(hipSetDevice(ctx->device));
   dgr_maps *m = new dgr_maps();
diff --git a/deepglobalregistration_amd/csrc/knn.hip b/deepglobalregistration_amd/csrc/knn.hip
--- a/deepglobalregistration_amd/csrc/knn.hip
+++ b/deepglobalregistration_amd/csrc/knn.hip
@@ -195,7 +195,7 @@
   dim3 grid(KNN_SCAN_SPLITS, B.np);
   knn_query_scan_kernel<<<grid, 256, 0, stream>>>(F0, F1, B, P.q_begin, P.qlist, P.qcount, best);
   knn_long_list_flags<<<1, 64, 0, stream>>>(P.qcount, B.np, P.flags);
-  DGR_LAUNCH_CHECK();
+  DGR_LAUNCH_CHECK(2);
   DGR_CHECK(knn_launch<32>(ctx, F0, F1, B, best, P.flags, stream, P.qlist, P.qcount, P.q_begin));
   return knn_launch<32>(ctx, F0, F1, B, best, P.fallback, stream);
 }
diff --git a/deepglobalregistration_amd/csrc/knn_common.h b/deepglobalregistration_amd/csrc/knn_common.h
--- a/deepglobalregistration_amd/csrc/knn_common.h
+++ b/deepglobalregistration_amd/csrc/knn_common.h
@@ -90,7 +90,7 @@
   DGR_REQUIRE(off1[npairs] < (1ll << 31) && n0 < (1ll << 31), "find_knn: N0 / N1 too large");
   u64 *keys;
   DGR_ALLOC(keys, ctx->arena, u64, n0 * k);
-  if (clear) DGR_HIP_CHECK(hipMemsetAsync(keys, 0xff, (size_t)(n0 * k) * sizeof(u64), stream));
+  if (clear) DGR_HIP_CHECK(dgr_memset_async(keys, 0xff, (size_t)(n0 * k) * sizeof(u64), stream));
   for (int p0 = 0; p0 < npairs; p0 += KNN_MAXP) {
     KnnBatch B;
     B.np = std::min(KNN_MAXP, npairs - p0);
diff --git a/deepglobalregistration_amd/csrc/knn_prefilter.h b/deepglobalregistration_amd/csrc/knn_prefilter.h
--- a/deepglobalregistration_amd/csrc/knn_prefilter.h
+++ b/deepglobalregistration_amd/csrc/knn_prefilter.h
@@ -280,8 +280,8 @@
   P.fallback = pair_words + KNN_MAXP;
   P.qcount = pair_words + 2 * KNN_MAXP;
   P.flags = pair_words + 3 * KNN_MAXP;
-  DGR_HIP_CHECK(hipMemsetAsync(P.cand_cnt, 0, (size_t)(P.span + 4 * KNN_MAXP) * sizeof(int32_t), stream));
-  DGR_HIP_CHECK(hipMemsetAsync(P.mt, 0xff, (size_t)n_mt * sizeof(uint32_t), stream));
+  DGR_HIP_CHECK(dgr_memset_async(P.cand_cnt, 0, (size_t)(P.span + 4 * KNN_MAXP) * sizeof(int32_t), stream));
+  DGR_HIP_CHECK(dgr_memset_async(P.mt, 0xff, (size_t)n_mt * sizeof(uint32_t), stream));
   dim3 grid((unsigned)dgr_ceil_div((int64_t)std::max(P.qb_max, P.rt_max) * 32 * 4, 256), 2 * B.np);
   knn_pack_kernel<TOPK><<<grid, 256, 0, stream>>>(F0, F1, B, P.Qp, P.Rp, P.na, P.nb, P.nb_max, P.fallback);
   DGR_LAUNCH_CHECK();
diff --git a/deepglobalregistration_amd/csrc/net.hip b/deepglobalregistration_amd/csrc/net.hip
--- a/deepglobalregistration_amd/csrc/net.hip
+++ b/deepglobalregistration_amd/csrc/net.hip
@@ -196,21 +196,21 @@
       DGR_HIP_CHECK(hipMalloc((void **)&P.staging, n * sizeof(float)));
       P.staging_n = n;
     }
-    DGR_HIP_CHECK(hipMemcpyAsync(P.staging, kd->data, n * sizeof(float), hipMemcpyHostToDevice, s));
+    DGR_HIP_CHECK(dgr_memcpy_async(P.staging, kd->data, n * sizeof(float), hipMemcpyHostToDevice, s));
     src = P.staging;
   }
   const float *sc = P.sc;
-  DGR_HIP_CHECK(hipMemcpyAsync(P.sc, scale.data(), (size_t)cout * sizeof(float), hipMemcpyHostToDevice, s));
+  DGR_HIP_CHECK(dgr_memcpy_async(P.sc, scale.data(), (size_t)cout * sizeof(float), hipMemcpyHostToDevice, s));
   if (has_shift) {
     DGR_CHECK(W.alloc(&L.shift, cout));
-    DGR_HIP_CHECK(hipMemcpyAsync(L.shift, shift.data(), (size_t)cout * sizeof(float), hipMemcpyHostToDevice, s));
+    DGR_HIP_CHECK(dgr_memcpy_async(L.shift, shift.data(), (size_t)cout * sizeof(float), hipMemcpyHostToDevice, s));
   }
   const int64_t nw = (int64_t)K * cin * cout;
-  DGR_HIP_CHECK(hipMemsetAsync(P.mxb, 0, sizeof(uint32_t), s));
+  DGR_HIP_CHECK(dgr_memset_async(P.mxb, 0, sizeof(uint32_t), s));
   dgr_absmax_scaled_kernel<<<(int)std::min<int64_t>((nw + 255) / 256, 4096), 256, 0, s>>>(src, sc, nw, cout, P.mxb);
   DGR_LAUNCH_CHECK();
   uint32_t bits = 0;
-  DGR_HIP_CHECK(hipMemcpyAsync(&bits, P.mxb, sizeof(bits), hipMemcpyDeviceToHost, s));
+  DGR_HIP_CHECK(dgr_memcpy_async(&bits, P.mxb, sizeof(bits), hipMemcpyDeviceToHost, s));
   DGR_HIP_CHECK(hipStreamSynchronize(s));
   float mx;
   memcpy(&mx, &bits, 4);
@@ -550,8 +550,8 @@
       DGR_REQUIRE(in.split.planes, "layer %s: the wide-layer kernel needs its input as split rows", L.name.c_str());
       if (prof) {
         DGR_ALLOC(a.clk, ctx->arena, unsigned long long, 2);
-        DGR_HIP_CHECK(hipMemsetAsync(a.clk, 0xff, sizeof(unsigned long long), stream));
-        DGR_HIP_CHECK(hipMemsetAsync(a.clk + 1, 0, sizeof(unsigned long long), stream));
+        DGR_HIP_CHECK(dgr_memset_async(a.clk, 0xff, sizeof(unsigned long long), stream));
+        DGR_HIP_CHECK(dgr_memset_async(a.clk + 1, 0, sizeof(unsigned long long), stream));
         clk = a.clk;
       }
       DGR_CHECK(dgr_conv_wide_launch(a, in.split, L.wb, L.wb_piece, L.w_unscale, ctx->num_cus, stream, &kname));
@@ -670,7 +670,7 @@
     const int64_t words = 5 * n1 + 6 * n2 + 6 * n4 + 3 * n8;
     uint32_t *pool;
     DGR_ALLOC(pool, A, uint32_t, words);
-    DGR_HIP_CHECK(hipMemsetAsync(pool, 0, (size_t)words * sizeof(uint32_t), stream));
+    DGR_HIP_CHECK(dgr_memset_async(pool, 0, (size_t)words * sizeof(uint32_t), stream));
     auto take = [&](int64_t n) { uint32_t *p = pool; pool += n; return p; };
     for (Tensor *t : {&T1, &Y1, &S1, &U1, &V1}) t->amax = take(n1);
     for (Tensor *t : {&T2, &Y2, &S2, &CAT2, &U2, &V2}) t->amax = take(n2);
@@ -826,14 +826,14 @@
 static int check_flag(dgr_ctx *ctx, const int32_t *flag_dev, hipStream_t stream) {
   unsigned char *pin;
   DGR_CHECK(dgr_ctx_pinned(ctx, 64, &pin));
-  DGR_HIP_CHECK(hipMemcpyAsync(pin, flag_dev, sizeof(int32_t), hipMemcpyDeviceToHost, stream));
+  DGR_HIP_CHECK(dgr_memcpy_async(pin, flag_dev, sizeof(int32_t), hipMemcpyDeviceToHost, stream));
   DGR_CHECK(dgr_ctx_wait(ctx, stream));
   return dgr_flag_error(*reinterpret_cast<volatile int32_t *>(pin));
 }
 
 int dgr_ctx_new_flag(dgr_ctx *ctx, hipStream_t stream) {
   DGR_ALLOC(ctx->flag_dev, ctx->arena, int32_t, 1);
-  DGR_HIP_CHECK(hipMemsetAsync(ctx->flag_dev, 0, sizeof(int32_t), stream));
+  DGR_HIP_CHECK(dgr_memset_async(ctx->flag_dev, 0, sizeof(int32_t), stream));
   return DGR_OK;
 }
 
@@ -854,6 +854,7 @@
   DGR_REQUIRE(net->ctx == ctx, "dgr_resunet_forward: the net object belongs to another context (one dgr_net per context: "
                                "dgr_net_share gives a second context its own over the same weights)");
   DGR_REQUIRE(N > 0, "dgr_resunet_forward: empty sparse tensor (N=%lld)", (long long)N);
+  DgrLaunchScope launch_scope(ctx);
   hipStream_t stream = (hipStream_t)stream_;
   DGR_HIP_CHECK(hipSetDevice(ctx->device));
   DGR_CHECK(ctx->arena.reset());
diff --git a/deepglobalregistration_amd/csrc/pipeline.hip b/deepglobalregistration_amd/csrc/pipeline.hip
--- a/deepglobalregistration_amd/csrc/pipeline.hip
+++ b/deepglobalregistration_amd/csrc/pipeline.hip
@@ -87,12 +87,12 @@
   DGR_CHECK(ctx->arena.reset());
   double *sum;
   DGR_ALLOC(sum, ctx->arena, double, 1);
-  DGR_HIP_CHECK(hipMemsetAsync(sum, 0, sizeof(double), stream));
+  DGR_HIP_CHECK(dgr_memset_async(sum, 0, sizeof(double), stream));
   int blocks = (int)dgr_ceil_div(N, 256);
   if (blocks > 1024) blocks = 1024;
   sigmoid_clip_sum_kernel<<<blocks, 256, 0, stream>>>(logit, N, clip, weights_out, sum);
   DGR_LAUNCH_CHECK();
-  DGR_HIP_CHECK(hipMemcpyAsync(wsum, sum, sizeof(double), hipMemcpyDeviceToHost, stream));
+  DGR_HIP_CHECK(dgr_memcpy_async(wsum, sum, sizeof(double), hipMemcpyDeviceToHost, stream));
   DGR_HIP_CHECK(hipStreamSynchronize(stream));
   return DGR_OK;
 }
@@ -124,12 +124,13 @@
 }
 
 __global__ void concat_coords_kernel(const int32_t *__restrict__ c0, int64_t n0, const int32_t *__restrict__ c1,
-                                     int64_t n1, int32_t *__restrict__ out) {
+                                     int64_t n1, int32_t *__restrict__ out, float *__restrict__ ones) {
   const int64_t i = (int64_t)blockIdx.x * blockDim.x + threadIdx.x;
   if (i >= n0 + n1) return;
   const int32_t *src = i < n0 ? c0 + i * 4 : c1 + (i - n0) * 4;
   out[i * 4] = src[0] * 2 + (i < n0 ? 0 : 1);
   out[i * 4 + 1] = src[1]; out[i * 4 + 2] = src[2]; out[i * 4 + 3] = src[3];
+  if (ones) ones[i] = 1.f;
 }
 
 struct StageTimer {
@@ -162,7 +163,7 @@
   DGR_ALLOC(B->weights, A, float, n0);
   DGR_ALLOC(B->off0_dev, A, int64_t, npairs + 1);
   DGR_ALLOC(B->res_dev, A, DgrRegResult, npairs);
-  DGR_HIP_CHECK(hipMemcpyAsync(B->off0_dev, off0, (size_t)(npairs + 1) * sizeof(int64_t), hipMemcpyHostToDevice, stream));
+  DGR_HIP_CHECK(dgr_memcpy_async(B->off0_dev, off0, (size_t)(npairs + 1) * sizeof(int64_t), hipMemcpyHostToDevice, stream));
   return DGR_OK;
 }
 
@@ -193,6 +194,7 @@
     DGR_REQUIRE(off0[p + 1] > off0[p] && off1[p + 1] > off1[p], "pair %d is empty", p);
   DGR_REQUIRE(dgr_net_ctx(fcgf) == ctx && dgr_net_ctx(inlier) == ctx,
               "dgr_register_batch: a net object belongs to another context (one dgr_net per context: dgr_net_share)");
+  DgrLaunchScope launch_scope(ctx);
   hipStream_t stream = (hipStream_t)stream_;
   DGR_HIP_CHECK(hipSetDevice(ctx->device));
   ctx->last_T64.clear();
@@ -210,14 +212,20 @@
   F1 = F0 + n0 * C;
   DGR_ALLOC(ones, A, float, n0 + n1);
   DGR_CHECK(alloc_batch_buffers(A, n0, npairs, off0, stream, &B));
-  fill_kernel<<<256, 256, 0, stream>>>(ones, n0 + n1, 1.f);
+  const bool ones_apart = dgr_maps_unfused();
+  if (ones_apart) {
+    fill_kernel<<<256, 256, 0, stream>>>(ones, n0 + n1, 1.f);
+    DGR_LAUNCH_CHECK();
+  }
 
   DGR_CHECK(tm.rec(0, 0));
   {
     DgrArena::Mark mk = A.mark();
     int32_t *coords01;
     DGR_ALLOC(coords01, A, int32_t, (n0 + n1) * 4);
-    concat_coords_kernel<<<(int)dgr_ceil_div(n0 + n1, 256), 256, 0, stream>>>(coords0, n0, coords1, n1, coords01);
+    concat_coords_kernel<<<(int)dgr_ceil_div(n0 + n1, 256), 256, 0, stream>>>(coords0, n0, coords1, n1, coords01,
+                                                                                    ones_apart ? nullptr : ones);
+    DGR_LAUNCH_CHECK();
     DGR_CHECK(dgr_resunet_forward_impl(ctx, fcgf, coords01, ones, n0 + n1, F0, stream));
     A.rewind(mk);
     dgr_net_invalidate_runs(fcgf);
@@ -243,8 +251,10 @@
   DgrRegResult *const res_dev = B.res_dev;
   DGR_CHECK(tm.rec(1, 0));
   DGR_CHECK(dgr_knn1_batch_impl(ctx, F0, off0, F1, off1, npairs, C, 0, idx1, nullptr, stream));
-  if (override_idx1)
+  if (override_idx1) {
     override_idx_kernel<<<(int)dgr_ceil_div(n0, 256), 256, 0, stream>>>(idx1, override_idx1, n0);
+    DGR_LAUNCH_CHECK();
+  }
   DGR_CHECK(tm.rec(1, 1));
   DGR_CHECK(tm.rec(2, 0));
   DGR_CHECK(dgr_inlier_inputs_impl(coords0, xyz0, n0, coords1, xyz1, idx1, ftype, coords6, feats6, stream));
@@ -268,8 +278,8 @@
   unsigned char *pin;
   DGR_CHECK(dgr_ctx_pinned(ctx, 64 + (size_t)npairs * sizeof(DgrRegResult), &pin));
   const DgrRegResult *res = reinterpret_cast<const DgrRegResult *>(pin + 64);
-  DGR_HIP_CHECK(hipMemcpyAsync(pin + 64, res_dev, (size_t)npairs * sizeof(DgrRegResult), hipMemcpyDeviceToHost, stream));
-  DGR_HIP_CHECK(hipMemcpyAsync(pin, ctx->flag_dev, sizeof(int32_t), hipMemcpyDeviceToHost, stream));
+  DGR_HIP_CHECK(dgr_memcpy_async(pin + 64, res_dev, (size_t)npairs * sizeof(DgrRegResult), hipMemcpyDeviceToHost, stream));
+  DGR_HIP_CHECK(dgr_memcpy_async(pin, ctx->flag_dev, sizeof(int32_t), hipMemcpyDeviceToHost, stream));
   DGR_CHECK(dgr_ctx_wait(ctx, stream, (long)(*ns_per_row * (double)(n0 + n1))));
   *ns_per_row = (double)ctx->last_wait_ns / (double)(n0 + n1);
   DGR_CHECK(dgr_flag_error(*reinterpret_cast<volatile int32_t *>(pin)));
@@ -321,7 +331,7 @@
           DGR_CHECK(dgr_ransac_begin(ctx, xyz0 + off0[p] * 3, Y, m0, 2.0 * prm->voxel_size,
                                      prm->ransac_hypotheses > 0 ? prm->ransac_hypotheses : 4000000, prm->ransac_seed, &rs[p],
                                      stream));
-          DGR_HIP_CHECK(hipMemcpyAsync(&rsh[(size_t)p * DGR_RANSAC_RESULT_DOUBLES], rs[p],
+          DGR_HIP_CHECK(dgr_memcpy_async(&rsh[(size_t)p * DGR_RANSAC_RESULT_DOUBLES], rs[p],
                                        DGR_RANSAC_RESULT_DOUBLES * sizeof(double), hipMemcpyDeviceToHost, stream));
           status_out[p] = DGR_STATUS_SAFEGUARD;
         }
@@ -329,7 +339,7 @@
         double *Tinit;
         DGR_ALLOC(Tinit, A, double, (int64_t)npairs * 16);
         for (int i = 0; i < npairs * 16; ++i) Th[i] = T_out[i];
-        DGR_HIP_CHECK(hipMemcpyAsync(Tinit, Th.data(), Th.size() * sizeof(double), hipMemcpyHostToDevice, stream));
+        DGR_HIP_CHECK(dgr_memcpy_async(Tinit, Th.data(), Th.size() * sizeof(double), hipMemcpyHostToDevice, stream));
         for (int p = 0; p < npairs; ++p)
           DGR_CHECK(dgr_icp_begin(ctx, xyz0 + off0[p] * 3, off0[p + 1] - off0[p], xyz1 + off1[p] * 3, off1[p + 1] - off1[p],
                                   2.0 * prm->voxel_size, rs[p] ? rs[p] : Tinit + (int64_t)p * 16, &jobs[p], stream));
@@ -463,6 +473,7 @@
   }
   const int64_t n0 = off0[npairs], n1 = off1[npairs];
   for (int p = 0; p < npairs; ++p) segs[(size_t)npairs + p].dst += n0;
+  DgrLaunchScope launch_scope(ctx);
   hipStream_t stream = (hipStream_t)stream_;
   DGR_HIP_CHECK(hipSetDevice(ctx->device));
   ctx->last_T64.clear();
@@ -483,7 +494,7 @@
   auto run = [&]() -> int {
     DGR_CHECK(alloc_batch_buffers(A, n0, npairs, off0.data(), stream, &B));
     DGR_CHECK(tm.rec(0, 0));
-    DGR_HIP_CHECK(hipMemcpyAsync(segs_dev, segs.data(), segs.size() * sizeof(BankSegment), hipMemcpyHostToDevice, stream));
+    DGR_HIP_CHECK(dgr_memcpy_async(segs_dev, segs.data(), segs.size() * sizeof(BankSegment), hipMemcpyHostToDevice, stream));
     bank_gather_kernel<<<(int)dgr_ceil_div(n0 + n1, BANK_GATHER_ROWS), BANK_GATHER_ROWS, 0, stream>>>(
         reinterpret_cast<const int4 *>(bank_coords), bank_xyz, reinterpret_cast<const float4 *>(bank_F), segs_dev,
         2 * npairs, n0 + n1, C == 16 ? 2 : C == 32 ? 3 : 4, reinterpret_cast<int4 *>(coords), xyz,
@@ -522,7 +533,7 @@
   if (dst_dev) {
     const int64_t bytes = ctx->last.numel[which] * (which == 0 ? 8 : 4);
     DGR_REQUIRE(capacity_bytes >= bytes, "destination buffer too small");
-    DGR_HIP_CHECK(hipMemcpyAsync(dst_dev, ctx->last.ptr[which], (size_t)bytes, hipMemcpyDeviceToDevice,
+    DGR_HIP_CHECK(dgr_memcpy_async(dst_dev, ctx->last.ptr[which], (size_t)bytes, hipMemcpyDeviceToDevice,
                                  (hipStream_t)stream));
   }
   return DGR_OK;
diff --git a/deepglobalregistration_amd/csrc/reg.hip b/deepglobalregistration_amd/csrc/reg.hip
--- a/deepglobalregistration_amd/csrc/reg.hip
+++ b/deepglobalregistration_amd/csrc/reg.hip
@@ -509,7 +509,7 @@
   DGR_ALLOC(a.cA, ctx->arena, float4, crows);
   DGR_ALLOC(a.cB, ctx->arena, float4, crows);
   DGR_ALLOC(a.xbuf, ctx->arena, unsigned long long, (int64_t)npairs * 2 * REG_CLMAX * REG_XG);
-  DGR_HIP_CHECK(hipMemsetAsync(a.xbuf, 0, (size_t)npairs * 2 * REG_CLMAX * REG_XG * sizeof(unsigned long long), stream));
+  DGR_HIP_CHECK(dgr_memset_async(a.xbuf, 0, (size_t)npairs * 2 * REG_CLMAX * REG_XG * sizeof(unsigned long long), stream));
   a.clip = clip; a.q = q; a.eps = eps;
   a.is_logit = is_logit; a.gate = gate; a.skip_refine = skip_refine;
   a.max_iter = max_iter; a.max_break = max_break; a.ratio = ratio;
@@ -555,20 +555,20 @@
   DGR_ALLOC(off, ctx->arena, int64_t, 2);
   DGR_ALLOC(res, ctx->arena, DgrRegResult, 1);
   const int64_t h_off[2] = {0, N};
-  DGR_HIP_CHECK(hipMemcpyAsync(off, h_off, sizeof(h_off), hipMemcpyHostToDevice, stream));
+  DGR_HIP_CHECK(dgr_memcpy_async(off, h_off, sizeof(h_off), hipMemcpyHostToDevice, stream));
   double *st_in = nullptr, *st_out = nullptr;
   if (state_in_host) {
     DGR_ALLOC(st_in, ctx->arena, double, 30);
-    DGR_HIP_CHECK(hipMemcpyAsync(st_in, state_in_host, 30 * sizeof(double), hipMemcpyHostToDevice, stream));
+    DGR_HIP_CHECK(dgr_memcpy_async(st_in, state_in_host, 30 * sizeof(double), hipMemcpyHostToDevice, stream));
   }
   if (state_out_host) {
     DGR_ALLOC(st_out, ctx->arena, double, 30);
-    DGR_HIP_CHECK(hipMemsetAsync(st_out, 0, 30 * sizeof(double), stream));
+    DGR_HIP_CHECK(dgr_memset_async(st_out, 0, 30 * sizeof(double), stream));
   }
   DGR_CHECK(launch_registration(ctx, X, Y, nullptr, w, 0, 0.f, off, h_off, 1, N, q, max_iter, max_break, ratio,
                                 skip_refine, 0, eps, nullptr, res, stream, st_in, st_out));
-  DGR_HIP_CHECK(hipMemcpyAsync(host_res, res, sizeof(DgrRegResult), hipMemcpyDeviceToHost, stream));
-  if (state_out_host) DGR_HIP_CHECK(hipMemcpyAsync(state_out_host, st_out, 30 * sizeof(double), hipMemcpyDeviceToHost, stream));
+  DGR_HIP_CHECK(dgr_memcpy_async(host_res, res, sizeof(DgrRegResult), hipMemcpyDeviceToHost, stream));
+  if (state_out_host) DGR_HIP_CHECK(dgr_memcpy_async(state_out_host, st_out, 30 * sizeof(double), hipMemcpyDeviceToHost, stream));
   DGR_HIP_CHECK(hipStreamSynchronize(stream));
   if (host_res->status == DGR_STATUS_EXCHANGE_TIMEOUT) {
     dgr_set_error("registration: the workgroups sharing a pair lost each other (exchange timed out)");
diff --git a/deepglobalregistration_amd/ops.py b/deepglobalregistration_amd/ops.py
--- a/deepglobalregistration_amd/ops.py
+++ b/deepglobalregistration_amd/ops.py
@@ -894,6 +894,10 @@
     return names[:n.value]
 
 
+def launches(device):
+    return int(_lib.load().dgr_ctx_launches(get_ctx(device)))
+
+
 def debug_ortho2rotation(p6, grad_R=None):
     dev = _dev(p6)
     p6 = _as(p6, torch.float32, dev).reshape(-1, 6)
diff --git a/include/dgr_hip.h b/include/dgr_hip.h
--- a/include/dgr_hip.h
+++ b/include/dgr_hip.h
@@ -150,6 +150,7 @@
 int dgr_ctx_conv_launch_times(dgr_ctx *ctx, float *times_ms, float *gemm_ms, int64_t capacity, int64_t *n);
 int dgr_ctx_conv_launch_kernel_us(dgr_ctx *ctx, float *us, int64_t capacity, int64_t *n);
 int dgr_ctx_conv_launch_kinds(dgr_ctx *ctx, char *buf, int64_t capacity, int64_t *n);
+int64_t dgr_ctx_launches(dgr_ctx *ctx);
 
 int dgr_radius_pairs_batch(dgr_ctx *ctx, const float *xyz0, const int64_t *off0, const float *xyz1,
                            const int64_t *off1, int npairs, const double *T, double radius, int K,
```
